# georgesterpu/avsr-tf1

Measured on AMD Instinct MI355X. Metric: utterances/sec (train step) at B=64 T_a=500 T_v=75, higher is better.
Workload: dtype f32; 1 GPU; c4: AV dual-attention (bimodal) video 1x256 + audio 3x256 uni-LSTM, scaled_luong, B=64 T_a=500x80 T_v=75 L=40; utterances_per_gpu=64, global_batch=64, T_a=500, F_a=80, T_v=75, F_v=128, T_dec=40, parallelism=dp1, video_frontend=resnet_cnn, launch=hipgraph, dropout=True

## Files before the change

avsr-tf1_amd/_lib.py:

```python
import ctypes as C
import os

import torch

from . import build as _build

MAX_LAYERS = 4
MAX_MECH = 4
MAX_STACKS = 4

_fp = C.POINTER(C.c_float)
_ip = C.POINTER(C.c_int32)


class AvsrError(RuntimeError):
    pass


class Mat(C.Structure):
    _fields_ = [("ptr", C.c_void_p), ("ld", C.c_int64), ("T", C.c_int32), ("pad_", C.c_int32), ("ldo", C.c_int64)]


class GemmDesc(C.Structure):
    _fields_ = [("A", Mat), ("B", Mat), ("C", Mat), ("bias", C.c_void_p),
                ("M", C.c_int32), ("N", C.c_int32), ("K", C.c_int32),
                ("trans_a", C.c_int32), ("trans_b", C.c_int32),
                ("alpha", C.c_float), ("beta", C.c_float), ("batch", C.c_int32),
                ("stride_a", C.c_int64), ("stride_b", C.c_int64), ("stride_c", C.c_int64),
                ("alpha_dev", C.c_void_p),
                ("splitk", C.c_int32), ("pad_", C.c_int32),
                ("workspace", C.c_void_p), ("workspace_floats", C.c_int64),
                ("colsum", C.c_void_p), ("colsum_beta", C.c_float), ("pad2_", C.c_int32)]


class RnnLayer(C.Structure):
    _fields_ = [("units", C.c_int32), ("in_dim", C.c_int32), ("hoisted", C.c_int32), ("out_col", C.c_int32),
                ("wt", C.c_void_p), ("w", C.c_void_p), ("bias", C.c_void_p),
                ("gates", C.c_void_p), ("cs", C.c_void_p), ("out", C.c_void_p), ("ld_out", C.c_int64),
                ("state", C.c_void_p), ("h_final", C.c_void_p), ("c_final", C.c_void_p),
                ("dgates", C.c_void_p), ("dstate", C.c_void_p), ("dout", C.c_void_p), ("ld_dout", C.c_int64),
                ("dout_col", C.c_int32), ("residual", C.c_int32), ("hs_seq", C.c_void_p), ("xt_seq", C.c_void_p),
                ("wt2", C.c_void_p), ("w2", C.c_void_p), ("bias2", C.c_void_p), ("rh_seq", C.c_void_p), ("dgates2", C.c_void_p)]


class RnnStack(C.Structure):
    _fields_ = [("B", C.c_int32), ("T", C.c_int32), ("reverse", C.c_int32), ("n_layers", C.c_int32),
                ("cell", C.c_int32), ("pad_", C.c_int32),
                ("len", C.c_void_p), ("dh_final", C.c_void_p), ("dc_final", C.c_void_p),
                ("seed", C.c_void_p), ("keep_in", C.c_float), ("keep_state", C.c_float), ("keep_out", C.c_float),
                ("consumer_keep", C.c_float), ("cell_id_base", C.c_int32), ("consumer_stream", C.c_int32),
                ("consumer_width", C.c_int32), ("pad2_", C.c_int32),
                ("layer", RnnLayer * MAX_LAYERS)]


class AttnMech(C.Structure):
    _fields_ = [("type", C.c_int32), ("T", C.c_int32), ("D", C.c_int32), ("chunk", C.c_int32),
                ("len", C.c_void_p), ("keys", C.c_void_p), ("values", C.c_void_p),
                ("values_sb", C.c_int64), ("values_st", C.c_int64),
                ("g", C.c_void_p), ("v", C.c_void_p), ("bq", C.c_void_p),
                ("wq_t", C.c_void_p), ("wq", C.c_void_p), ("watt_t", C.c_void_p), ("watt", C.c_void_p),
                ("scores", C.c_void_p), ("ctx", C.c_void_p), ("pq", C.c_void_p), ("pstat", C.c_void_p),
                ("pctx", C.c_void_p), ("dscores", C.c_void_p), ("dctx", C.c_void_p), ("dpq", C.c_void_p),
                ("pdq", C.c_void_p)]


class DecLayer(C.Structure):
    _fields_ = [("wt", C.c_void_p), ("w", C.c_void_p), ("bias", C.c_void_p), ("gates", C.c_void_p), ("cs", C.c_void_p),
                ("out", C.c_void_p), ("state", C.c_void_p), ("hs_seq", C.c_void_p), ("xin_seq", C.c_void_p),
                ("dgates", C.c_void_p), ("dstate", C.c_void_p), ("cell_id", C.c_int32), ("pad_", C.c_int32),
                ("wt2", C.c_void_p), ("w2", C.c_void_p), ("bias2", C.c_void_p), ("rh_seq", C.c_void_p), ("dgates2", C.c_void_p)]


MAX_DEC_EXTRA = 3


class AttnRnn(C.Structure):
    _fields_ = [("B", C.c_int32), ("L", C.c_int32), ("H", C.c_int32), ("E", C.c_int32),
                ("n_mech", C.c_int32), ("output_attention", C.c_int32), ("V", C.c_int32), ("mode", C.c_int32),
                ("go_id", C.c_int32), ("eos_id", C.c_int32),
                ("steplen", C.c_void_p), ("wt", C.c_void_p), ("w", C.c_void_p), ("bias", C.c_void_p),
                ("gates", C.c_void_p), ("cs", C.c_void_p), ("cell_out", C.c_void_p), ("att", C.c_void_p),
                ("h0", C.c_void_p), ("c0", C.c_void_p), ("state", C.c_void_p),
                ("h_final", C.c_void_p), ("c_final", C.c_void_p),
                ("mech", AttnMech * MAX_MECH),
                ("embedding", C.c_void_p), ("wout_t", C.c_void_p), ("bout", C.c_void_p),
                ("logits", C.c_void_p), ("ids", C.c_void_p), ("tok", C.c_void_p), ("n_unfinished", C.c_void_p),
                ("dgates", C.c_void_p), ("dstate", C.c_void_p), ("datt", C.c_void_p), ("dq", C.c_void_p),
                ("datt_ext", C.c_void_p), ("dcell_ext", C.c_void_p), ("dh0", C.c_void_p), ("dc0", C.c_void_p),
                ("dh_final", C.c_void_p), ("dc_final", C.c_void_p),
                ("seed", C.c_void_p), ("keep_in", C.c_float), ("keep_state", C.c_float), ("keep_out", C.c_float),
                ("sampling_prob", C.c_float), ("cell_id", C.c_int32), ("pad3_", C.c_int32),
                ("hs_seq", C.c_void_p), ("attd", C.c_void_p), ("xs", C.c_void_p), ("labels", C.c_void_p), ("fed", C.c_void_p),
                ("cell", C.c_int32), ("pad4_", C.c_int32), ("wt2", C.c_void_p), ("w2", C.c_void_p), ("bias2", C.c_void_p),
                ("rh_seq", C.c_void_p), ("dgates2", C.c_void_p),
                ("beam_width", C.c_int32), ("mem_shared", C.c_int32), ("length_penalty", C.c_float), ("pad6_", C.c_float),
                ("beam_logp", C.c_void_p), ("beam_fin", C.c_void_p), ("beam_len", C.c_void_p), ("step_ids", C.c_void_p),
                ("parent_ids", C.c_void_p), ("parent_rows", C.c_void_p),
                ("n_extra", C.c_int32), ("prof_tag", C.c_int32), ("out0", C.c_void_p), ("extra", DecLayer * MAX_DEC_EXTRA),
                ("fused_ws", C.c_void_p), ("fused_ws_floats", C.c_int64)]


MAX_LM_LAYERS = 4


class BeamLm(C.Structure):
    _fields_ = [("n_layers", C.c_int32), ("H", C.c_int32), ("E", C.c_int32), ("V", C.c_int32),
                ("one_hot", C.c_int32), ("n_rows", C.c_int32), ("lm_weight", C.c_float), ("pad_", C.c_int32),
                ("embedding", C.c_void_p), ("wt", C.c_void_p * MAX_LM_LAYERS), ("bias", C.c_void_p * MAX_LM_LAYERS),
                ("wout_t", C.c_void_p), ("bout", C.c_void_p), ("state_c", C.c_void_p), ("state_h", C.c_void_p), ("lm_logp", C.c_void_p)]


BEAM_CTC_MAX_T, BEAM_CTC_MAX_V = 2048, 256


class BeamCtc(C.Structure):
    _fields_ = [("n_utt", C.c_int32), ("beam_width", C.c_int32), ("T", C.c_int32), ("V", C.c_int32), ("eos_id", C.c_int32),
                ("weight", C.c_float), ("ld", C.c_int64)] + \
               [(n, C.c_void_p) for n in ("z", "in_len", "y", "state", "psi", "last", "term", "extra", "lm_logp")] + \
               [("lm_weight", C.c_float), ("pad_", C.c_int32)]


class ConvDesc(C.Structure):
    _fields_ = [(n, C.c_int32) for n in ("N", "H", "W", "Ci", "Co", "k", "stride", "pad_t", "pad_l", "Ho", "Wo", "pad_")] + \
               [("bn_scale", C.c_void_p), ("bn_shift", C.c_void_p)]


class ConvLaunch(C.Structure):
    _fields_ = [(n, C.c_int32) for n in ("kernel", "m", "ntc", "ch4", "rs", "fold", "ep", "nsp", "ntap", "t0", "F", "grid", "CsP", "lds_bytes",
                                         "slab", "pad_")]


class Conv3dDesc(C.Structure):
    _fields_ = [(n, C.c_int32) for n in ("B", "T", "H", "W", "Ci", "Co", "kt", "kh", "kw", "stride", "pad_f", "pad_t", "pad_l", "Ho", "Wo",
                                         "relu")] + [("scale", C.c_void_p), ("shift", C.c_void_p)]


class LogmelArgs(C.Structure):
    _fields_ = [(n, C.c_int32) for n in ("B", "N", "T_out", "F", "frame_length", "frame_step", "fft_length", "num_mel_bins", "window", "stride",
                                         "mel_nnz", "pad_")] + \
               [(n, C.c_void_p) for n in ("wav", "wav_len", "hann", "twiddle", "mel_lo", "mel_cnt", "mel_ptr", "mel_w", "out", "out_len")]


class CtcArgs(C.Structure):
    _fields_ = [("B", C.c_int32), ("T", C.c_int32), ("L", C.c_int32), ("C", C.c_int32), ("ld", C.c_int64)] + \
               [(n, C.c_void_p) for n in ("z", "labels", "labels_len", "in_len", "denom")] + [("weight", C.c_float), ("pad_", C.c_int32)] + \
               [(n, C.c_void_p) for n in ("nll", "status", "utt_loss", "dz", "ws")] + [("ws_floats", C.c_int64)]


class ColsumJob(C.Structure):
    _fields_ = [("a", Mat), ("b", Mat), ("out", C.c_void_p), ("rows", C.c_int32), ("F", C.c_int32), ("alpha", C.c_float), ("beta", C.c_float)]


class TransposeJob(C.Structure):
    _fields_ = [("src", C.c_void_p), ("dst", C.c_void_p), ("rows", C.c_int32), ("cols", C.c_int32)]


_STRUCTS = {"avsr_dec_layer": DecLayer, "avsr_mat": Mat, "avsr_gemm_desc": GemmDesc, "avsr_rnn_layer": RnnLayer, "avsr_rnn_stack": RnnStack,
            "avsr_conv_desc": ConvDesc, "avsr_conv_launch": ConvLaunch, "avsr_conv3d_desc": Conv3dDesc, "avsr_logmel_args": LogmelArgs, "avsr_ctc_args": CtcArgs, "avsr_attn_mech": AttnMech, "avsr_attn_rnn": AttnRnn, "avsr_transpose_job": TransposeJob,
            "avsr_colsum_job": ColsumJob, "avsr_beam_lm": BeamLm, "avsr_beam_ctc": BeamCtc}

_vp, _i32, _i64, _f32 = C.c_void_p, C.c_int32, C.c_int64, C.c_float
_SIGS = {
    "avsr_gemm": [C.POINTER(GemmDesc), _vp],
    "avsr_gemm_batch": [C.POINTER(GemmDesc), _i32, _vp],
    "avsr_rnn_fwd": [C.POINTER(RnnStack), _i32, _vp],
    "avsr_rnn_bwd": [C.POINTER(RnnStack), _i32, _vp],
    "avsr_rnn_set_persistent": [_vp, _i64],
    "avsr_rnn_set_persistent_mode": [_i32],
    "avsr_rnn_set_persistent_scratch": [_vp, _i64],
    "avsr_attn_rnn_fwd": [C.POINTER(AttnRnn), _i32, _i32, _vp],
    "avsr_attn_rnn_fused_eligible": [C.POINTER(AttnRnn)],
    "avsr_attn_rnn_fused_fwd_active": [C.POINTER(AttnRnn)],
    "avsr_attn_rnn_set_fused": [_i32],
    "avsr_attn_rnn_set_beam_kernel": [_i32],
    "avsr_conv_set_mfma": [_i32],
    "avsr_conv_supported": [C.POINTER(ConvDesc)],
    "avsr_conv_fwd": [C.POINTER(ConvDesc), _vp, _vp, _vp, _vp, _vp, _vp, _vp, _vp, C.POINTER(_i32), _vp],
    "avsr_conv_bwd_data": [C.POINTER(ConvDesc), _vp, _vp, _vp, _f32, _vp],
    "avsr_conv_bwd_weight": [C.POINTER(ConvDesc), _vp, _vp, _vp, _vp, _f32, _vp, _i64, _vp],
    "avsr_conv_bwd_data_bn": [C.POINTER(ConvDesc), _vp, _vp, _vp, _f32, _vp, _vp, _vp, _vp, _vp, C.POINTER(_i32), _vp],
    "avsr_conv_bwd_data_bn_supported": [C.POINTER(ConvDesc)],
    "avsr_conv_bwd_weight_bn": [C.POINTER(ConvDesc), _vp, _vp, _vp, _vp, _vp, _vp, _vp, _f32, _vp, _i64, _vp],
    "avsr_conv_bwd_weight_bn_supported": [C.POINTER(ConvDesc)],
    "avsr_conv_plan": [C.POINTER(ConvDesc), _i32, _i32, _i64, C.POINTER(ConvLaunch), _i32],
    "avsr_bn_bwd_finalize": [_vp, _i32, _i32, _i64, _vp, _vp, _vp, _vp, _vp, _f32, _vp, _vp],
    "avsr_bn_bwd_apply": [_vp, _vp, _vp, _vp, _i64, _i32, _f32, _vp],
    "avsr_bn_bwd_stage1": [_vp, _vp, _vp, _vp, _vp, _vp, _i64, _i32, _vp, C.POINTER(_i32), _vp],
    "avsr_bn_partials_f64": [_vp, _i32, _i32, _vp, _vp],
    "avsr_bn_finalize_f64": [_vp, _i32, _f32, _f32, _vp, _vp, _vp, _vp, _vp, _vp, _vp, _vp, _vp],
    "avsr_bn_bwd_finalize_f64": [_vp, _vp, _i32, _vp, _vp, _vp, _vp, _vp, _f32, _vp, _vp],
    "avsr_bn_eval_affine": [_vp, _vp, _vp, _vp, _f32, _vp, _vp, _i32, _vp],
    "avsr_bn_finalize": [_vp, _i32, _i32, _i64, _f32, _f32, _vp, _vp, _vp, _vp, _vp, _vp, _vp, _vp, _vp],
    "avsr_conv3d_supported": [C.POINTER(Conv3dDesc)],
    "avsr_conv3d_fwd": [C.POINTER(Conv3dDesc), _vp, _vp, _vp, _vp, _vp, _vp, _vp, C.POINTER(_i32), _vp],
    "avsr_conv3d_bwd_data": [C.POINTER(Conv3dDesc), _vp, _vp, _vp, _f32, _vp],
    "avsr_conv3d_bwd_weight": [C.POINTER(Conv3dDesc), _vp, _vp, _vp, _f32, _vp, _i64, _vp],
    "avsr_conv3d_bn_finalize": [_vp, _i32, _i32, _i64, _f32, _f32, _vp, _vp, _vp, _vp, _vp, _vp, _vp, _vp, _vp],
    "avsr_logmel_supported": [_i32, _i32, _i32, _i32, _i32],
    "avsr_logmel_fwd": [C.POINTER(LogmelArgs), _vp],
    "avsr_ctc_loss": [C.POINTER(CtcArgs), _vp],
    "avsr_ctc_best_path": [_vp, _i64, _vp, _i32, _i32, _i32, _vp, _vp],
    "avsr_batchnorm_apply": [_vp, _vp, _i32, _i32, _vp, _vp, _vp, _vp, _i32, _vp],
    "avsr_attn_rnn_bwd": [C.POINTER(AttnRnn), _vp],
    "avsr_beam_gather_tree": [_vp, _vp, _vp, _vp, _i32, _i32, _i32, _i32, _vp],
    "avsr_beam_search_step": [_vp, _i32, _i32, _i32, _i32, _i32, _f32, _vp, _vp, _vp, _vp, _vp, _vp, _vp, _vp, _vp, _vp, _vp, _vp, _i64, _i32, _vp, _vp, _vp],
    "avsr_beam_lm_supported": [C.POINTER(BeamLm)],
    "avsr_beam_lm_step": [C.POINTER(BeamLm), _vp, _vp, _i32, _i32, _vp],
    "avsr_beam_search_step_lm": [_vp, _i32, _i32, _i32, _i32, _i32, _f32, _vp, _vp, _vp, _vp, _vp, _vp, _vp, _vp, _vp, _vp, _vp, _vp, _i64, _i32, _vp, _vp,
                                 _vp, _f32, _vp],
    "avsr_attn_rnn_fwd_lm": [C.POINTER(AttnRnn), C.POINTER(BeamLm), _i32, _i32, _vp],
    "avsr_beam_ctc_supported": [C.POINTER(BeamCtc)],
    "avsr_beam_ctc_begin": [C.POINTER(BeamCtc), _vp],
    "avsr_beam_ctc_step": [C.POINTER(BeamCtc), _vp, _vp, _vp, _i32, _vp],
    "avsr_beam_search_step_ctc": [_vp, _i32, _i32, _i32, _i32, _i32, _f32, _vp, _vp, _vp, _vp, _vp, _vp, _vp, _vp, _vp, _vp, _vp, _vp, _i64, _i32, _vp, _vp,
                                  _vp, _f32, _vp, _f32, _vp, _vp],
    "avsr_attn_rnn_fwd_ctc": [C.POINTER(AttnRnn), C.POINTER(BeamLm), C.POINTER(BeamCtc), _i32, _i32, _vp],
    "avsr_attn_alpha_rows": [_vp, _vp, _vp, _vp, _vp, _vp, _i32, _i32, _i32, _vp],
    "avsr_bahdanau_dkeys": [_vp, _vp, _i64, _i64, _vp, _vp, _vp, _vp, _vp, _vp, _i32, _i32, _i32, _i32, _vp],
    "avsr_transpose": [C.POINTER(TransposeJob), _i32, _vp],
    "avsr_colsum": [C.POINTER(Mat), C.POINTER(Mat), _i32, _i32, _f32, _f32, _vp, _vp, _i64, _vp],
    "avsr_batchnorm_fwd": [_vp, _vp, _i32, _i32, _vp, _vp, _vp, _vp, _vp, _vp, _i32, _vp, _i64, _vp],
    "avsr_batchnorm_xhat": [_vp, _vp, _vp, _vp, _i32, _i32, _vp],
    "avsr_batchnorm_fwd_ex": [_vp, _vp, _i32, _i32, _vp, _vp, _vp, _vp, _vp, _vp, _i32, _f32, _f32, _i32, _i32, _vp, _i64, _vp],
    "avsr_batchnorm_bwd": [_vp, _vp, _vp, _vp, _vp, _vp, _vp, _vp, _vp, _i32, _i32, _i32, _f32, _vp, _i64, _vp],
    "avsr_im2col": [_vp, _vp, _i32, _i32, _i32, _i32, _i32, _i32, _i32, _i32, _i32, _i32, _i32, _vp],
    "avsr_col2im": [_vp, _vp, _i32, _i32, _i32, _i32, _i32, _i32, _i32, _i32, _i32, _i32, _i32, _f32, _vp],
    "avsr_relu": [_vp, _vp, _i64, _vp],
    "avsr_relu_bwd": [_vp, _vp, _vp, _i64, _vp],
    "avsr_add": [_vp, _vp, _vp, _i64, _vp],
    "avsr_selu": [_vp, _vp, _i64, _vp],
    "avsr_selu_bwd": [_vp, _vp, _vp, _i64, _vp],
    "avsr_conv3x3_supported": [_i32, _i32, _i32, _i32],
    "avsr_conv3x3": [_vp, _vp, _vp, _vp, _i32, _i32, _i32, _i32, _i32, _i32, _i32, _i32, _i32, _i32, _i32, _f32, _vp],
    "avsr_conv3x3_bwd_data_s2": [_vp, _vp, _vp, _i32, _i32, _i32, _i32, _i32, _i32, _i32, _i32, _i32, _f32, _vp],
    "avsr_conv3x3_bwd_weight": [_vp, _vp, _vp, _i32, _i32, _i32, _i32, _i32, _i32, _i32, _i32, _i32, _i32, _f32, _vp, _i64, _vp],
    "avsr_embed_labels": [_vp, _vp, _i32, _vp, _vp, _i32, _i32, _i32, _i32, _vp],
    "avsr_embed_grad": [_vp, _vp, _vp, _i32, _i32, _i32, _i32, _vp, _i64, _vp],
    "avsr_dropout_rows": [C.POINTER(Mat), C.POINTER(Mat), _i32, _i32, _vp, _i32, _f32, _i32, _i32, _i32, _vp],
    "avsr_seq_loss": [_vp, _vp, _vp, _vp, _i32, _vp, _vp, _i32, _i32, _i32, _vp],
    "avsr_seq_loss_fun": [_vp, _vp, _vp, _vp, _i32, _vp, _vp, _i32, _i32, _i32, _i32, _f32, _vp],
    "avsr_au_loss": [_vp, _vp, _vp, _vp, _vp, _i32, _i32, _f32, _vp],
    "avsr_au_loss_dp": [_vp, _vp, _vp, _vp, _vp, _i32, _i32, _f32, _vp, _vp],
    "avsr_normed_v": [_vp, _vp, _vp, _i32, _vp],
    "avsr_normed_v_bwd": [_vp, _vp, _vp, _vp, _vp, _i32, _vp],
    "avsr_reduce_scalar": [_vp, _i32, _vp, _i32, _i32, _f32, _vp],
    "avsr_l2_regularise": [C.POINTER(_i64), C.POINTER(_i64), _i32, _vp, _vp, _f32, _vp, _vp, _vp],
    "avsr_global_norm": [_vp, _i64, _f32, _vp, _vp, _vp],
    "avsr_adam_step": [_vp, _vp, _vp, _vp, _i64, _vp, _vp, _f32, _i32, _f32, _f32, _vp],
    "avsr_batchnorm_sync_sum": [_vp, _i32, _i32, _vp, _vp, _i64, _vp],
    "avsr_batchnorm_sync_sqsum": [_vp, _i32, _i32, _vp, _vp, _vp, _vp, _vp, _i64, _vp],
    "avsr_batchnorm_sync_apply": [_vp, _vp, _i32, _i32, _vp, _vp, _vp, _vp, _vp, _vp, _vp, _vp, _f32, _f32, _i32, _vp],
    "avsr_batchnorm_sync_moments": [_vp, _i32, _i32, _vp, _vp, _i64, _vp],
    "avsr_dp_sync_unpack": [_vp, _vp, _i32, C.POINTER(_i32), C.POINTER(_i32), C.POINTER(_vp), C.POINTER(_vp), C.POINTER(_vp), _vp],
    "avsr_seq_loss_per_utterance": [_vp, _vp, _vp, _vp, _i32, _i32, _vp],
    "avsr_instnorm_fwd": [_vp, _vp, _i32, _i32, _i32, _vp, _vp, _vp, _vp, _f32, _vp],
    "avsr_instnorm_bwd": [_vp, _vp, _vp, _vp, _vp, _vp, _vp, _vp, _i32, _i32, _i32, _vp],
    "avsr_optimiser_step": [_vp, _vp, _vp, _vp, _i64, _vp, _vp, _f32, _i32, _i32, _f32, _f32, _i32, _f32, _vp],
    "avsr_highway_fwd": [_vp, _vp, _vp, _vp, _vp, _i32, _i32, _i32, _vp],
    "avsr_highway_bwd": [_vp, _vp, _vp, _vp, _vp, _vp, _vp, _vp, _i32, _i32, _i32, _i32, _vp],
    "avsr_copy_words": [_vp, _vp, _i64, _vp],
    "avsr_zero_words": [_vp, _i64, _vp],
    "avsr_zero_multi": [C.POINTER(_vp), C.POINTER(_i64), _i32, _vp],
    "avsr_add_int": [_vp, _i32, _vp, _vp],
    "avsr_colsum_multi": [C.POINTER(ColsumJob), _i32, _vp, _i64, _vp],
    "avsr_slab_defer_begin": [], "avsr_slab_defer_end": [_vp],
    "avsr_adam_step_decay": [_vp, _vp, _vp, _vp, _i64, _vp, _vp, _f32, _i32, _i32, _f32, _f32, _vp],
    "avsr_prof_begin": [_i32],
    "avsr_prof_end": [C.POINTER(_i32), C.POINTER(_f32), C.POINTER(C.c_double)],
}
EXPORTS = ["avsr_abi_version", "avsr_sizeof", "avsr_attn_rnn_fused_ws_floats", "avsr_conv3d_wgrad_scratch_floats", "avsr_ctc_ws_floats"] + list(_SIGS)

_lib = None


def lib_path():
    return _build.LIB


def load():
    global _lib
    if _lib is not None:
        return _lib
    path = os.environ.get("AVSR_LIB") or _build.LIB
    if path == _build.LIB and _build.needs_build():
        try:
            _build.build()
        except Exception as e:
            if not os.path.exists(path):
                raise AvsrError("libavsr_hip.so is missing and could not be built: %s" % e)
    lib = C.CDLL(path)
    lib.avsr_abi_version.restype = C.c_int
    lib.avsr_sizeof.restype = C.c_int64
    lib.avsr_sizeof.argtypes = [C.c_char_p]
    for sym in EXPORTS:
        if not hasattr(lib, sym):
            raise AvsrError("libavsr_hip.so does not export %s" % sym)
    for name, at in _SIGS.items():
        fn = getattr(lib, name)
        fn.argtypes = at
        fn.restype = C.c_int
    lib.avsr_attn_rnn_fused_ws_floats.argtypes = [_i32, _i32, _i32]
    lib.avsr_attn_rnn_fused_ws_floats.restype = C.c_int64
    lib.avsr_conv3d_wgrad_scratch_floats.argtypes = [C.POINTER(Conv3dDesc)]
    lib.avsr_conv3d_wgrad_scratch_floats.restype = C.c_int64
    lib.avsr_ctc_ws_floats.argtypes = [_i32, _i32, _i32]
    lib.avsr_ctc_ws_floats.restype = C.c_int64
    for name, st in _STRUCTS.items():
        n = lib.avsr_sizeof(name.encode())
        if n != C.sizeof(st):
            raise AvsrError("ABI mismatch for %s: C %d vs ctypes %d" % (name, n, C.sizeof(st)))
    _lib = lib
    return lib


def check(rc, what):
    if rc != 0:
        raise AvsrError("%s failed with code %d" % (what, rc))


def ptr(t):
    return None if t is None else t.data_ptr()


def stream_ptr():
    return torch.cuda.current_stream().cuda_stream
```

avsr-tf1_amd/csrc/batchnorm.hip:

```cpp
#include "reduce.h"
#include "avsr_hip.h"

using namespace avsr;
#define S_(x) ((hipStream_t)(x))

namespace {

__global__ void bn_partial_sum_kernel(const float* x, float* part, int rows, int F, int rows_per_blk) {
  __shared__ float red[256];
  const int G = F < 256 ? 256 / F : 1;
  const int r0 = blockIdx.x * rows_per_blk, r1 = min(rows, r0 + rows_per_blk);
  for (int base = 0; base < (G > 1 ? 1 : F); base += blockDim.x) {
    const int idx = base + threadIdx.x;
    const int f = G > 1 ? idx % F : idx, g = G > 1 ? idx / F : 0;
    float s0 = 0.f, s1 = 0.f;
    if (G > 1 ? idx < G * F : idx < F) {
      int r = r0 + g;
      for (; r + G < r1; r += 2 * G) { s0 += x[(long)r * F + f]; s1 += x[(long)(r + G) * F + f]; }
      if (r < r1) s0 += x[(long)r * F + f];
    }
    if (G > 1) block_group_reduce(s0 + s1, idx, F, G, red, part + (long)blockIdx.x * F);
    else if (idx < F) part[(long)blockIdx.x * F + idx] = s0 + s1;
  }
}

__global__ __launch_bounds__(1024) void bn_mean_kernel(const float* part, int npart, float* mean, int rows, int F,
                                                       const float* total = nullptr) {
  if (total) rows = (int)total[0];
  __shared__ double red[32][33];
  const int fl = threadIdx.x & 31, g = threadIdx.x >> 5;
  const int f = blockIdx.x * 32 + fl;
  double s = 0.0;
  if (f < F)
    for (int i = g; i < npart; i += 32) s += (double)part[(long)i * F + f];
  red[g][fl] = s;
  __syncthreads();
  if (g == 0 && f < F) {
    double t = 0.0;
#pragma unroll
    for (int j = 0; j < 32; ++j) t += red[j][fl];
    mean[f] = (float)(t / rows);
  }
}

__global__ void bn_partial_sq_kernel(const float* x, const float* mean_v, float* part, int rows, int F, int rows_per_blk) {
  __shared__ float red[256];
  const int G = F < 256 ? 256 / F : 1;
  const int r0 = blockIdx.x * rows_per_blk, r1 = min(rows, r0 + rows_per_blk);
  for (int base = 0; base < (G > 1 ? 1 : F); base += blockDim.x) {
    const int idx = base + threadIdx.x;
    const int f = G > 1 ? idx % F : idx, g = G > 1 ? idx / F : 0;
    float s0 = 0.f, s1 = 0.f;
    if (G > 1 ? idx < G * F : idx < F) {
      const float mean = mean_v[f];
      int r = r0 + g;
      for (; r + G < r1; r += 2 * G) {
        const float d0 = x[(long)r * F + f] - mean, d1 = x[(long)(r + G) * F + f] - mean;
        s0 += d0 * d0; s1 += d1 * d1;
      }
      if (r < r1) { const float d0 = x[(long)r * F + f] - mean; s0 += d0 * d0; }
    }
    if (G > 1) block_group_reduce(s0 + s1, idx, F, G, red, part + (long)blockIdx.x * F);
    else if (idx < F) part[(long)blockIdx.x * F + idx] = s0 + s1;
  }
}

__global__ __launch_bounds__(1024) void bn_var_kernel(const float* part, int npart, const float* mean_v, float* invstd_v, float* mov_mean,
                                                      float* mov_var, int rows, int F, float eps, float momentum,
                                                      int bessel, const float* total = nullptr) {
  if (total) rows = (int)total[0];
  __shared__ double red[32][33];
  const int fl = threadIdx.x & 31, g = threadIdx.x >> 5;
  const int f = blockIdx.x * 32 + fl;
  double s = 0.0;
  if (f < F)
    for (int i = g; i < npart; i += 32) s += (double)part[(long)i * F + f];
  red[g][fl] = s;
  __syncthreads();
  if (g == 0 && f < F) {
    double t = 0.0;
#pragma unroll
    for (int j = 0; j < 32; ++j) t += red[j][fl];
    const float var = (float)(t / rows), mean = mean_v[f];
    invstd_v[f] = rsqrtf(var + eps);
    if (mov_mean) {
      const float unbiased = bessel ? var * ((float)rows / (float)max(1, rows - 1)) : var;
      mov_mean[f] = momentum * mov_mean[f] + (1.f - momentum) * mean;
      mov_var[f] = momentum * mov_var[f] + (1.f - momentum) * unbiased;
    }
  }
}

__global__ void bn_apply_kernel(const float* x, const float* mean_v, const float* invstd_v, const float* mov_mean, const float* mov_var,
                                const float* gamma, const float* beta, float* y, long n4, int F, int training, float eps, int relu) {
  for (long i = (long)blockIdx.x * blockDim.x + threadIdx.x; i < n4; i += (long)gridDim.x * blockDim.x) {
    const int f = (int)((i * 4) % F);
    const f32x4 xv = ld4(x + i * 4);
    f32x4 yv;
#pragma unroll
    for (int e = 0; e < 4; ++e) {
      const float mean = training ? mean_v[f + e] : mov_mean[f + e];
      const float istd = training ? invstd_v[f + e] : rsqrtf(mov_var[f + e] + eps);
      yv[e] = (xv[e] - mean) * (gamma[f + e] * istd) + beta[f + e];
      if (relu) yv[e] = fmaxf(yv[e], 0.f);
    }
    st4(y + i * 4, yv);
  }
}

__global__ void bn_xhat_kernel(const float* x, const float* mean, const float* invstd, float* xhat, long n, int F) {
  for (long i = (long)blockIdx.x * blockDim.x + threadIdx.x; i < n; i += (long)gridDim.x * blockDim.x) {
    const int f = (int)(i % F);
    xhat[i] = (x[i] - mean[f]) * invstd[f];
  }
}

int bn_blocks(int rows, int F, int64_t scratch_floats, int* rpb_out) {
  const int maxblk = 2048;
  int rpb = rows > 64 * maxblk ? (rows + maxblk - 1) / maxblk : 64;
  int nblk = (rows + rpb - 1) / rpb;
  if ((long)nblk * F > scratch_floats) {
    nblk = (int)(scratch_floats / F);
    if (nblk < 1) return 0;
    rpb = (rows + nblk - 1) / nblk;
    nblk = (rows + rpb - 1) / rpb;
  }
  *rpb_out = rpb;
  return nblk;
}

}

extern "C" int avsr_batchnorm_fwd_ex(const float* x, float* y, int32_t rows, int32_t F, const float* gamma, const float* beta,
                                     float* moving_mean, float* moving_var, float* save_mean, float* save_invstd, int32_t training,
                                     float eps, float momentum, int32_t relu, int32_t bessel, float* scratch, int64_t scratch_floats, void* stream) {
  if (!x || !y || !gamma || !beta || rows <= 0 || F <= 0 || !scratch) return AVSR_ERR_ARG;
  if (F % 4) return AVSR_ERR_ARG;
  int rpb;
  const int nblk = bn_blocks(rows, F, scratch_floats - 2 * F, &rpb);
  if (!nblk) return AVSR_ERR_ARG;
  float* part = scratch;
  float* mean_v = save_mean ? save_mean : scratch + (long)nblk * F;
  float* invstd_v = save_invstd ? save_invstd : scratch + (long)nblk * F + F;
  if (training) {
    hipLaunchKernelGGL(bn_partial_sum_kernel, dim3(nblk), dim3(256), 0, S_(stream), x, part, rows, F, rpb);
    AVSR_CHECK_LAUNCH();
    hipLaunchKernelGGL(bn_mean_kernel, dim3((F + 31) / 32), dim3(1024), 0, S_(stream), part, nblk, mean_v, rows, F);
    AVSR_CHECK_LAUNCH();
    hipLaunchKernelGGL(bn_partial_sq_kernel, dim3(nblk), dim3(256), 0, S_(stream), x, mean_v, part, rows, F, rpb);
    AVSR_CHECK_LAUNCH();
    hipLaunchKernelGGL(bn_var_kernel, dim3((F + 31) / 32), dim3(1024), 0, S_(stream), part, nblk, mean_v, invstd_v, moving_mean,
                       moving_var, rows, F, eps, momentum, bessel);
    AVSR_CHECK_LAUNCH();
  } else if (!moving_mean || !moving_var) {
    return AVSR_ERR_ARG;
  }
  const long n4 = (long)rows * F / 4;
  int blocks = (int)((n4 + 255) / 256);
  if (blocks > 4096) blocks = 4096;
  hipLaunchKernelGGL(bn_apply_kernel, dim3(blocks), dim3(256), 0, S_(stream), x, mean_v, invstd_v, moving_mean, moving_var, gamma, beta, y,
                     n4, F, training, eps, relu);
  AVSR_CHECK_LAUNCH();
  return AVSR_OK;
}

extern "C" int avsr_batchnorm_fwd(const float* x, float* y, int32_t rows, int32_t F, const float* gamma,
                                  const float* beta, float* moving_mean, float* moving_var, float* save_mean,
                                  float* save_invstd, int32_t training, float* scratch, int64_t scratch_floats,
                                  void* stream) {
  return avsr_batchnorm_fwd_ex(x, y, rows, F, gamma, beta, moving_mean, moving_var, save_mean, save_invstd, training, 1e-3f, 0.99f, 0,
                               0 , scratch, scratch_floats, stream);
}

extern "C" int avsr_batchnorm_apply(const float* x, float* y, int32_t rows, int32_t F, const float* gamma, const float* beta, const float* mean,
                                    const float* invstd, int32_t relu, void* stream) {
  if (!x || !y || !gamma || !beta || !mean || !invstd || rows <= 0 || F <= 0 || F % 4) return AVSR_ERR_ARG;
  const long n4 = (long)rows * F / 4;
  int blocks = (int)((n4 + 255) / 256);
  if (blocks > 4096) blocks = 4096;
  hipLaunchKernelGGL(bn_apply_kernel, dim3(blocks), dim3(256), 0, S_(stream), x, mean, invstd, nullptr, nullptr, gamma, beta, y, n4, F, 1, 0.f, relu);
  AVSR_CHECK_LAUNCH();
  return AVSR_OK;
}

extern "C" int avsr_batchnorm_xhat(const float* x, const float* mean, const float* invstd, float* xhat, int32_t rows,
                                   int32_t F, void* stream) {
  if (!x || !mean || !invstd || !xhat) return AVSR_ERR_ARG;
  const long n = (long)rows * F;
  hipLaunchKernelGGL(bn_xhat_kernel, dim3(blocks_for(n)), dim3(256), 0, S_(stream), x, mean, invstd, xhat, n, F);
  AVSR_CHECK_LAUNCH();
  return AVSR_OK;
}

namespace {

__global__ void bn_bwd_partial_kernel(const float* x, const float* dy, const float* gamma, const float* beta, const float* mean,
                                      const float* invstd, float* part, int rows, int F, int rows_per_blk, int relu) {
  __shared__ float red[512];
  const int G = F < 256 ? 256 / F : 1;
  const int r0 = blockIdx.x * rows_per_blk, r1 = min(rows, r0 + rows_per_blk);
  float* prow = part + (long)blockIdx.x * 2 * F;
  for (int base = 0; base < (G > 1 ? 1 : F); base += blockDim.x) {
    const int idx = base + threadIdx.x;
    const bool on = G > 1 ? idx < G * F : idx < F;
    const int f = G > 1 ? idx % F : idx, g = G > 1 ? idx / F : 0;
    float s1 = 0.f, s2 = 0.f;
    if (on) {
      const float m = mean[f], is = invstd[f], ga = gamma[f], be = beta[f];
      for (int r = r0 + g; r < r1; r += G) {
        const float xh = (x[(long)r * F + f] - m) * is;
        float d = dy[(long)r * F + f];
        if (relu && !(xh * ga + be > 0.f)) d = 0.f;
        s1 += d;
        s2 += d * xh;
      }
    }
    if (G > 1) {
      if (on) { red[idx] = s1; red[256 + idx] = s2; }
      __syncthreads();
      if (idx < F) {
        float t1 = 0.f, t2 = 0.f;
        for (int gg = 0; gg < G; ++gg) { t1 += red[gg * F + idx]; t2 += red[256 + gg * F + idx]; }
        prow[idx] = t1; prow[F + idx] = t2;
      }
    } else if (on) { prow[f] = s1; prow[F + f] = s2; }
  }
}

__global__ void bn_bwd_apply_kernel(const float* x, const float* dy, const float* gamma, const float* beta, const float* mean,
                                    const float* invstd, const float* sum1, const float* sum2, float* dx, long n, int rows, int F, int relu,
                                    float dx_beta) {
  const float inv_rows = 1.0f / (float)rows;
  for (long i = (long)blockIdx.x * blockDim.x + threadIdx.x; i < n; i += (long)gridDim.x * blockDim.x) {
    const int f = (int)(i % F);
    const float is = invstd[f], ga = gamma[f];
    const float xh = (x[i] - mean[f]) * is;
    float d = dy[i];
    if (relu && !(xh * ga + beta[f] > 0.f)) d = 0.f;
    const float v = ga * is * (d - (sum1[f] + xh * sum2[f]) * inv_rows);
    dx[i] = dx_beta != 0.f ? v + dx_beta * dx[i] : v;
  }
}

__global__ __launch_bounds__(256) void bn_bwd_partial4_kernel(const float* x, const float* dy, const float* gamma, const float* beta,
                                                               const float* mean, const float* invstd, float* part, long n4, int F, int relu) {
  __shared__ f32x4 red[2][256];
  const int f = (int)((threadIdx.x * 4) % F);
  const f32x4 m = ld4(mean + f), is = ld4(invstd + f), ga = ld4(gamma + f), be = ld4(beta + f);
  f32x4 s1 = {0.f, 0.f, 0.f, 0.f}, s2 = s1;
  for (long i = (long)blockIdx.x * 256 + threadIdx.x; i < n4; i += (long)gridDim.x * 256) {
    const f32x4 xv = ld4(x + i * 4), dv = ld4(dy + i * 4);
#pragma unroll
    for (int e = 0; e < 4; ++e) {
      const float xh = (xv[e] - m[e]) * is[e];
      float d = dv[e];
      if (relu && !(xh * ga[e] + be[e] > 0.f)) d = 0.f;
      s1[e] += d;
      s2[e] += d * xh;
    }
  }
  red[0][threadIdx.x] = s1; red[1][threadIdx.x] = s2;
  __syncthreads();
  const int tpf = F >> 2;
  if ((int)threadIdx.x < tpf) {
    f32x4 t1 = {0.f, 0.f, 0.f, 0.f}, t2 = t1;
    for (int k = threadIdx.x; k < 256; k += tpf) { t1 += red[0][k]; t2 += red[1][k]; }
    st4(part + (long)blockIdx.x * 2 * F + 4 * threadIdx.x, t1);
    st4(part + (long)blockIdx.x * 2 * F + F + 4 * threadIdx.x, t2);
  }
}

__global__ __launch_bounds__(256) void bn_bwd_apply4_kernel(const float* x, const float* dy, const float* gamma, const float* beta,
                                                             const float* mean, const float* invstd, const float* sum1, const float* sum2, float* dx,
                                                             long n4, int rows, int F, int relu, float dx_beta) {
  const int f = (int)((threadIdx.x * 4) % F);
  const float inv_rows = 1.0f / (float)rows;
  const f32x4 m = ld4(mean + f), is = ld4(invstd + f), ga = ld4(gamma + f), be = ld4(beta + f);
  f32x4 c1 = ld4(sum1 + f), c2 = ld4(sum2 + f);
#pragma unroll
  for (int e = 0; e < 4; ++e) { c1[e] *= inv_rows; c2[e] *= inv_rows; }
  for (long i = (long)blockIdx.x * 256 + threadIdx.x; i < n4; i += (long)gridDim.x * 256) {
    const f32x4 xv = ld4(x + i * 4), dv = ld4(dy + i * 4);
    f32x4 o;
    if (dx_beta != 0.f) o = ld4(dx + i * 4);
#pragma unroll
    for (int e = 0; e < 4; ++e) {
      const float xh = (xv[e] - m[e]) * is[e];
      float d = dv[e];
      if (relu && !(xh * ga[e] + be[e] > 0.f)) d = 0.f;
      const float v = ga[e] * is[e] * (d - (c1[e] + xh * c2[e]));
      o[e] = dx_beta != 0.f ? v + dx_beta * o[e] : v;
    }
    st4(dx + i * 4, o);
  }
}

}

extern "C" int avsr_batchnorm_bwd(const float* x, const float* dy, const float* gamma, const float* beta, const float* mean,
                                  const float* invstd, float* dx, float* dgamma, float* dbeta, int32_t rows, int32_t F, int32_t relu,
                                  float dx_beta, float* scratch, int64_t scratch_floats, void* stream) {
  if (!x || !dy || !gamma || !beta || !mean || !invstd || !scratch || rows <= 0 || F <= 0) return AVSR_ERR_ARG;
  const int maxblk = 2048;
  int rpb = rows > 64 * maxblk ? (rows + maxblk - 1) / maxblk : 64;
  int nblk = (rows + rpb - 1) / rpb;
  if ((long)nblk * 2 * F + 2 * F > scratch_floats) {
    nblk = (int)((scratch_floats - 2 * F) / (2L * F));
    if (nblk < 1) return AVSR_ERR_ARG;
    rpb = (rows + nblk - 1) / nblk;
    nblk = (rows + rpb - 1) / rpb;
  }
  float* part = scratch;
  const long n = (long)rows * F;
  auto al16 = [](const void* p) { return ((uintptr_t)p & 15) == 0; };
  const bool vec = F >= 4 && 1024 % F == 0 && al16(x) && al16(dy) && (!dx || al16(dx)) && al16(gamma) && al16(beta) && al16(mean) && al16(invstd) &&
                   al16(scratch) && rows >= 4096;
  if (vec) {
    int vb = (int)((n / 4 + 255) / 256);
    if (vb > 1024) vb = 1024;
    if ((long)vb * 2 * F + 2 * F > scratch_floats) vb = (int)((scratch_floats - 2 * F) / (2L * F));
    if (vb < 1) return AVSR_ERR_ARG;
    nblk = vb;
  }
  float* sums = scratch + (long)nblk * 2 * F;
  if (vec) hipLaunchKernelGGL(bn_bwd_partial4_kernel, dim3(nblk), dim3(256), 0, S_(stream), x, dy, gamma, beta, mean, invstd, part, n / 4, F, relu);
  else hipLaunchKernelGGL(bn_bwd_partial_kernel, dim3(nblk), dim3(256), 0, S_(stream), x, dy, gamma, beta, mean, invstd, part, rows, F, rpb, relu);
// ... 345 lines not shown
```

avsr-tf1_amd/csrc/capi.hip:

```cpp
#include <string.h>
#include "avsr_hip.h"

extern "C" int avsr_abi_version(void) { return 2; }

extern "C" int64_t avsr_sizeof(const char* name) {
  if (!name) return -1;
#define SZ(T) if (!strcmp(name, #T)) return (int64_t)sizeof(T);
  SZ(avsr_mat) SZ(avsr_gemm_desc) SZ(avsr_conv_desc) SZ(avsr_conv_launch) SZ(avsr_conv3d_desc) SZ(avsr_logmel_args) SZ(avsr_ctc_args) SZ(avsr_rnn_layer) SZ(avsr_rnn_stack) SZ(avsr_colsum_job)
#ifdef AVSR_HAVE_ATTN
  SZ(avsr_attn_mech) SZ(avsr_attn_rnn) SZ(avsr_transpose_job) SZ(avsr_dec_layer) SZ(avsr_beam_lm) SZ(avsr_beam_ctc)
#endif
#undef SZ
  return -1;
}

#include <vector>
#include "prof.h"
namespace avsr {
bool g_prof_enabled = false;
static std::vector<hipEvent_t> g_ev;
static std::vector<int> g_kind;
static size_t g_used = 0;
static double g_work[PROF_NKIND];
void prof_record(int kind, hipStream_t s, bool begin, double work) {
  if (begin) {
    if (g_used >= g_kind.size()) { g_prof_enabled = false; return; }
    g_kind[g_used] = kind;
    g_work[kind] += work;
    hipEventRecord(g_ev[2 * g_used], s);
  } else {
    hipEventRecord(g_ev[2 * g_used + 1], s);
    ++g_used;
  }
}
}

extern "C" int avsr_prof_begin(int32_t max_launches) {
  using namespace avsr;
  if (max_launches <= 0) return AVSR_ERR_ARG;
  while (g_ev.size() < (size_t)2 * max_launches) {
    hipEvent_t e;
    if (hipEventCreate(&e) != hipSuccess) return AVSR_ERR_HIP;
    g_ev.push_back(e);
  }
  g_kind.assign(max_launches, 0);
  g_used = 0;
  for (int k = 0; k < PROF_NKIND; ++k) g_work[k] = 0.0;
  g_prof_enabled = true;
  return AVSR_OK;
}

extern "C" int avsr_prof_end(int32_t* out_count, float* out_ms, double* out_flops) {
  using namespace avsr;
  g_prof_enabled = false;
  if (!out_count || !out_ms) return AVSR_ERR_ARG;
  if (hipDeviceSynchronize() != hipSuccess) return AVSR_ERR_HIP;
  for (int k = 0; k < PROF_NKIND; ++k) { out_count[k] = 0; out_ms[k] = 0.f; if (out_flops) out_flops[k] = g_work[k]; }
  for (size_t i = 0; i < g_used; ++i) {
    float ms = 0.f;
    if (hipEventElapsedTime(&ms, g_ev[2 * i], g_ev[2 * i + 1]) != hipSuccess) return AVSR_ERR_HIP;
    out_count[g_kind[i]] += 1;
    out_ms[g_kind[i]] += ms;
  }
  return AVSR_OK;
}
```

avsr-tf1_amd/csrc/elementwise.hip:

```cpp
#include "reduce.h"
#include "avsr_hip.h"

namespace avsr {

struct TJob { const float* src; float* dst; int rows, cols; };
struct TLaunch { int njob; TJob job[AVSR_MAX_TRANSPOSE]; };

__global__ void transpose_kernel(const TLaunch L) {
  __shared__ float tile[32][33];
  const TJob& J = L.job[blockIdx.z];
  const int tx = threadIdx.x & 31, ty = threadIdx.x >> 5;
  const int tiles_c = (J.cols + 31) / 32, tiles_r = (J.rows + 31) / 32;
  for (int tIdx = blockIdx.x; tIdx < tiles_c * tiles_r; tIdx += gridDim.x) {
    const int r0 = (tIdx / tiles_c) * 32, c0 = (tIdx % tiles_c) * 32;
    for (int j = ty; j < 32; j += 8) {
      const int r = r0 + j, c = c0 + tx;
      tile[j][tx] = (r < J.rows && c < J.cols) ? J.src[(long)r * J.cols + c] : 0.f;
    }
    __syncthreads();
    for (int j = ty; j < 32; j += 8) {
      const int c = c0 + j, r = r0 + tx;
      if (r < J.rows && c < J.cols) J.dst[(long)c * J.rows + r] = tile[tx][j];
    }
    __syncthreads();
  }
}

__global__ void embed_labels_kernel(const float* emb, const int32_t* labels, int go, float* out, int32_t* fed, int B, int L,
                                    int E, int nsteps) {
  const int b = blockIdx.x / nsteps, l = blockIdx.x % nsteps;
  const int tok = (l == 0) ? go : labels[(long)b * L + l - 1];
  if (fed && threadIdx.x == 0) fed[(long)b * L + l] = tok;
  for (int e = threadIdx.x; e < E; e += blockDim.x) out[((long)b * L + l) * E + e] = emb[(long)tok * E + e];
}

__global__ void dropout_rows_kernel(const float* x, long ldx, int Tx, long ldox, float* y, long ldy, int Ty, long ldoy,
                                    int rows, int cols, const int32_t* seed, uint32_t stream, float keep, int idx_w,
                                    int idx_coff, int accumulate) {
  const long total = (long)rows * cols;
  const bool on = seed && keep < 1.0f;
  const uint32_t sd = on ? (uint32_t)seed[0] : 0u;
  const float inv = 1.0f / keep;
  for (long i = (long)blockIdx.x * blockDim.x + threadIdx.x; i < total; i += (long)gridDim.x * blockDim.x) {
    const int r = (int)(i / cols), c = (int)(i % cols);
    float v = x[rowoff(r, ldx, Tx, ldox) + c];
    if (on) v = uniform01(sd, stream, (uint32_t)((long)r * idx_w + idx_coff + c)) < keep ? v * inv : 0.f;
    float* d = y + rowoff(r, ldy, Ty, ldoy) + c;
    *d = accumulate ? *d + v : v;
  }
}

#define EG_ROWS 256
__global__ void embed_grad_partial_kernel(const float* dx, const int32_t* fed, float* part, int rows, int E, int V) {
  __shared__ int toks[EG_ROWS];
  const int v = blockIdx.x, base = blockIdx.y * EG_ROWS;
  const int n = min(EG_ROWS, rows - base);
  for (int j = threadIdx.x; j < EG_ROWS; j += blockDim.x) toks[j] = j < n ? fed[base + j] : -1;
  __syncthreads();
  for (int e = threadIdx.x; e < E; e += blockDim.x) {
    float a = 0.f;
    for (int j = 0; j < n; j += 8) {
      float x[8];
#pragma unroll
      for (int k = 0; k < 8; ++k) x[k] = dx[(long)(base + min(j + k, n - 1)) * E + e];
#pragma unroll
      for (int k = 0; k < 8; ++k) a += (j + k < n && toks[j + k] == v) ? x[k] : 0.f;
    }
    part[((long)blockIdx.y * V + v) * E + e] = a;
  }
}

__global__ void seqlen_sum_kernel(const int32_t* len, int B, int L, float* denom) {
  __shared__ float red[4];
  float s = 0.f;
  for (int b = threadIdx.x; b < B; b += 256) s += (float)min(max(len[b], 0), L);
  s = block_sum_256(s, red);
  if (threadIdx.x == 0) denom[0] = s;
}

__global__ void set_scalar_kernel(float* p, float v) { p[0] = v; }

__global__ void seq_loss_kernel(float* logits, const int32_t* labels, const int32_t* len, const float* denom,
                                float* row_loss, float* dlogits, int B, int L, int V, int mode, float smooth) {
  const int row = blockIdx.x * blockDim.x + threadIdx.x;
  if (row >= B * L) return;
  const int b = row / L, l = row % L;
  float* lg = logits + (long)row * V;
  float* dl = dlogits ? dlogits + (long)row * V : nullptr;
  const bool valid = l < len[b];
  const float inv = 1.f / (denom[0] + 1e-12f);
  if (!valid) {
    row_loss[row] = mode == 1 ? logf((float)V) * inv : 0.f;
    for (int v = 0; v < V; ++v) lg[v] = 0.f;
    if (dl) for (int v = 0; v < V; ++v) dl[v] = 0.f;
    return;
  }
  float mx = lg[0];
  for (int v = 1; v < V; ++v) mx = fmaxf(mx, lg[v]);
  float s = 0.f;
  for (int v = 0; v < V; ++v) s += expf(lg[v] - mx);
  const float lse = mx + logf(s);
  const int y = labels[row];
  if (mode == 0) {
    row_loss[row] = (lse - lg[y]) * inv;
    if (dl) for (int v = 0; v < V; ++v) dl[v] = (expf(lg[v] - lse) - (v == y ? 1.f : 0.f)) * inv;
    return;
  }
  if (mode == 1) {
    const float off = smooth / (float)V, on = 1.f - smooth + off;
    float ce = 0.f;
    for (int v = 0; v < V; ++v) ce += (v == y ? on : off) * (lse - lg[v]);
    row_loss[row] = ce * inv;
    if (dl) for (int v = 0; v < V; ++v) dl[v] = (expf(lg[v] - lse) - (v == y ? on : off)) * inv;
    return;
  }
  float loss = 0.f, dot = 0.f;
  for (int v = 0; v < V; ++v) {
    const float p = expf(lg[v] - lse);
    const float q = fminf(fmaxf(p, 1e-7f), 1.f - 1e-7f);
    const bool inside = (p >= 1e-7f) && (p <= 1.f - 1e-7f);
    float f, a;
    if (mode == 3) {
      f = (v == y) ? -logf(q) : -logf(1.f - q);
      a = (v == y) ? -1.f / q : 1.f / (1.f - q);
    } else {
      if (v == y) { f = -(1.f - q) * (1.f - q) * logf(q); a = 2.f * (1.f - q) * logf(q) - (1.f - q) * (1.f - q) / q; }
      else        { f = -q * q * logf(1.f - q);           a = -2.f * q * logf(1.f - q) + q * q / (1.f - q); }
    }
    loss += f;
    dot += inside ? a * p : 0.f;
  }
  row_loss[row] = loss * inv;
  if (dl)
    for (int v = 0; v < V; ++v) {
      const float p = expf(lg[v] - lse);
      const float q = fminf(fmaxf(p, 1e-7f), 1.f - 1e-7f);
      const bool inside = (p >= 1e-7f) && (p <= 1.f - 1e-7f);
      float a;
      if (mode == 3) a = (v == y) ? -1.f / q : 1.f / (1.f - q);
      else a = (v == y) ? 2.f * (1.f - q) * logf(q) - (1.f - q) * (1.f - q) / q : -2.f * q * logf(1.f - q) + q * q / (1.f - q);
      dl[v] = p * ((inside ? a : 0.f) - dot) * inv;
    }
}

__global__ void seq_avg_kernel(const float* row_loss, const int32_t* len, const float* denom, float* out, int B, int L) {
  const int b = blockIdx.x * blockDim.x + threadIdx.x;
  if (b >= B) return;
  float s = 0.f;
  for (int l = 0; l < L; ++l) s += row_loss[(long)b * L + l];
  out[b] = s * (denom[0] + 1e-12f) / ((float)min(max(len[b], 0), L) + 1e-12f);
}

__global__ void au_loss_kernel(const float* z, const float* aus, const int32_t* len, float* row_loss, float* dz,
                               int B, int T, float weight, const float* total) {
  __shared__ float red[4];
  float cnt = 0.f;
  for (int b = threadIdx.x; b < B; b += 256) cnt += 2.f * (float)min(max(len[b], 0), T);
  cnt = block_sum_256(cnt, red);
  if (total) cnt = total[0];
  const float inv = cnt > 0.f ? 1.f / cnt : 0.f;
  for (int row = blockIdx.x * 256 + threadIdx.x; row < B * T; row += gridDim.x * 256) {
    const int b = row / T, t = row % T;
    float l = 0.f;
    for (int k = 0; k < 2; ++k) {
      float d = 0.f;
      if (t < len[b]) {
        const float p = sigmoidf_(z[(long)row * 2 + k]);
        const float tg = fminf(fmaxf(aus[(long)row * 2 + k], 0.f), 3.f) / 3.f;
        l += (p - tg) * (p - tg) * inv;
        d = weight * 2.f * (p - tg) * p * (1.f - p) * inv;
      }
      if (dz) dz[(long)row * 2 + k] = d;
    }
    row_loss[row] = l * weight;
  }
}

__global__ void normed_v_kernel(const float* v, const float* g, float* vn, int H) {
  __shared__ float red[4];
  float s = 0.f;
  for (int h = threadIdx.x; h < H; h += 256) s += v[h] * v[h];
  s = block_sum_256(s, red);
  const float sc = g[0] * rsqrtf(s);
  for (int h = threadIdx.x; h < H; h += 256) vn[h] = v[h] * sc;
}
__global__ void normed_v_bwd_kernel(const float* v, const float* g, const float* dvn, float* dv, float* dg, int H) {
  __shared__ float red[4];
  float s = 0.f, d = 0.f;
  for (int h = threadIdx.x; h < H; h += 256) { s += v[h] * v[h]; d += v[h] * dvn[h]; }
  s = block_sum_256(s, red);
  d = block_sum_256(d, red);
  const float nrm = sqrtf(s);
  for (int h = threadIdx.x; h < H; h += 256) dv[h] = g[0] / nrm * (dvn[h] - d * v[h] / s);
  if (threadIdx.x == 0) dg[0] = d / nrm;
}

struct Seg { long off, n; };
struct SegLaunch { int nseg; Seg seg[AVSR_MAX_SEGMENTS]; };

__global__ void l2_grad_kernel(const SegLaunch S, const float* w, float* g, float l2, float* part) {
  __shared__ float red[4];
  const Seg sg = S.seg[blockIdx.y];
  float s = 0.f;
  for (long i = (long)blockIdx.x * 256 + threadIdx.x; i < sg.n; i += (long)gridDim.x * 256) {
    const float x = w[sg.off + i];
    g[sg.off + i] += l2 * x;
    s += x * x;
  }
  s = block_sum_256(s, red);
  if (threadIdx.x == 0) part[blockIdx.y * gridDim.x + blockIdx.x] = 0.5f * l2 * s;
}

__global__ void sumsq_partial_kernel(const float* g, long n, float* part) {
  __shared__ float red[4];
  float s = 0.f;
  for (long i = (long)blockIdx.x * 256 + threadIdx.x; i < n; i += (long)gridDim.x * 256) s += g[i] * g[i];
  s = block_sum_256(s, red);
  if (threadIdx.x == 0) part[blockIdx.x] = s;
}

__global__ void reduce_scalar_kernel(const float* part, int n, float* out, int do_sqrt, int accumulate, float scale) {
  __shared__ double dred[256];
  double s = 0.0;
  for (int i = threadIdx.x; i < n; i += 256) s += (double)part[i];
  dred[threadIdx.x] = s;
  __syncthreads();
  for (int o = 128; o > 0; o >>= 1) {
    if (threadIdx.x < o) dred[threadIdx.x] += dred[threadIdx.x + o];
    __syncthreads();
  }
  if (threadIdx.x == 0) {
    double v = dred[0];
    if (do_sqrt) v = sqrt(v);
    v *= scale;
    out[0] = accumulate ? out[0] + (float)v : (float)v;
  }
}

__global__ void adam_kernel(float* p, float* g, float* m, float* v, long n, const float* gnorm, int32_t* step,
                            float lr, int warmup, float clip, float b1, float b2, float eps, float grad_scale,
                            int decay_steps, int opt, float weight_decay) {
  const int t = step[0] + 1;
  float lr_now = lr;
  if (decay_steps > 0) {
    const float frac = (float)(t - 1) / (float)decay_steps;
    const float i_restart = floorf(logf(1.0f + frac) / logf(2.0f));
    const float pw = exp2f(i_restart);
    const float within = (frac - (pw - 1.0f)) / pw;
    lr_now *= 0.5f * (1.0f + cosf(3.14159265358979323846f * within));
  }
  if (warmup > 0) lr_now *= fminf(1.0f, (float)t / (float)warmup);
  const double c1 = 1.0 - exp((double)t * log((double)b1));
  const double c2 = 1.0 - exp((double)t * log((double)b2));
  const float lr_t = (float)((double)lr_now * sqrt(c2) / c1);
  float scale = grad_scale;
  if (clip > 0.f) scale *= clip / fmaxf(gnorm[0], clip);
  for (long i = (long)blockIdx.x * blockDim.x + threadIdx.x; i < n; i += (long)gridDim.x * blockDim.x) {
    const float gi = g[i] * scale;
    if (opt == 3) {
      const float acc = 0.9f * m[i] + gi;
      m[i] = acc;
      p[i] -= lr_now * acc;
      continue;
    }
    const float mi = b1 * m[i] + (1.f - b1) * gi;
    const float vi = b2 * v[i] + (1.f - b2) * gi * gi;
    m[i] = mi;
    v[i] = vi;
    float pi = p[i];
    if (opt == 2) pi -= weight_decay * pi;
    const float num = opt == 1 ? b1 * mi + (1.f - b1) * gi : mi;
    p[i] = pi - lr_t * num / (sqrtf(vi) + eps);
  }
}
__global__ void step_inc_kernel(int32_t* step) { step[0] += 1; }

struct HwView { float* p; long ld; int T; long ldo; };
__device__ __forceinline__ long hw_off(const HwView& v, int r) { return rowoff(r, v.ld, v.T, v.ldo); }

__global__ void highway_fwd_kernel(HwView x, HwView h, HwView cpre, HwView y, const int32_t* len, int rows, int H, int T) {
  const long total = (long)rows * H;
  for (long i = (long)blockIdx.x * blockDim.x + threadIdx.x; i < total; i += (long)gridDim.x * blockDim.x) {
    const int r = (int)(i / H), c = (int)(i % H);
    float out = 0.f;
    if (!len || (r % T) < len[r / T]) {
      const float g = 1.f / (1.f + expf(-cpre.p[hw_off(cpre, r) + c]));
      out = x.p[hw_off(x, r) + c] * g + h.p[hw_off(h, r) + c] * (1.f - g);
    }
    y.p[hw_off(y, r) + c] = out;
  }
}

__global__ void highway_bwd_kernel(HwView x, HwView h, HwView cpre, HwView dy, HwView dh, HwView dcpre, HwView dx, const int32_t* len,
                                   int rows, int H, int T, int accumulate_dx) {
  const long total = (long)rows * H;
  for (long i = (long)blockIdx.x * blockDim.x + threadIdx.x; i < total; i += (long)gridDim.x * blockDim.x) {
    const int r = (int)(i / H), c = (int)(i % H);
    float vdh = 0.f, vdc = 0.f, vdx = 0.f;
    if (!len || (r % T) < len[r / T]) {
      const float g = 1.f / (1.f + expf(-cpre.p[hw_off(cpre, r) + c]));
      const float d = dy.p[hw_off(dy, r) + c];
      vdh = d * (1.f - g);
      vdc = d * (x.p[hw_off(x, r) + c] - h.p[hw_off(h, r) + c]) * g * (1.f - g);
      vdx = d * g;
    }
    dh.p[hw_off(dh, r) + c] = vdh;
    dcpre.p[hw_off(dcpre, r) + c] = vdc;
    float* px = dx.p + hw_off(dx, r) + c;
    *px = accumulate_dx ? *px + vdx : vdx;
  }
}

}

using namespace avsr;
#define S_(x) ((hipStream_t)(x))

extern "C" int avsr_transpose(const avsr_transpose_job* jobs, int32_t n, void* stream) {
  if (!jobs || n <= 0) return AVSR_ERR_ARG;
  for (int i0 = 0; i0 < n; i0 += AVSR_MAX_TRANSPOSE) {
    TLaunch L;
    L.njob = (n - i0) < AVSR_MAX_TRANSPOSE ? (n - i0) : AVSR_MAX_TRANSPOSE;
    int maxtiles = 1;
    for (int i = 0; i < L.njob; ++i) {
      const avsr_transpose_job& j = jobs[i0 + i];
      if (!j.src || !j.dst || j.rows <= 0 || j.cols <= 0) return AVSR_ERR_ARG;
      L.job[i] = TJob{j.src, j.dst, j.rows, j.cols};
      const int tiles = ((j.rows + 31) / 32) * ((j.cols + 31) / 32);
      if (tiles > maxtiles) maxtiles = tiles;
    }
    if (maxtiles > 1024) maxtiles = 1024;
    hipLaunchKernelGGL(transpose_kernel, dim3(maxtiles, 1, L.njob), dim3(256), 0, S_(stream), L);
    AVSR_CHECK_LAUNCH();
  }
  return AVSR_OK;
}

struct ZmLaunch { uint32_t* p[8]; long n[8]; int cnt; };
__global__ __launch_bounds__(256) void zero_multi_kernel(const ZmLaunch L) {
  const long stride = (long)gridDim.x * 256;
#pragma unroll 1
  for (int k = 0; k < L.cnt; ++k) {
    uint32_t* p = L.p[k];
    const long n = L.n[k], n4 = ((uintptr_t)p & 15) == 0 ? n >> 2 : 0;
    typedef unsigned int u32x4_ __attribute__((ext_vector_type(4)));
    for (long i = (long)blockIdx.x * 256 + threadIdx.x; i < n4; i += stride) reinterpret_cast<u32x4_*>(p)[i] = u32x4_{0u, 0u, 0u, 0u};
    for (long i = n4 * 4 + (long)blockIdx.x * 256 + threadIdx.x; i < n; i += stride) p[i] = 0u;
  }
}
extern "C" int avsr_zero_multi(void* const* ptrs, const int64_t* n_words, int32_t count, void* stream) {
  if (count <= 0) return AVSR_OK;
  if (!ptrs || !n_words) return AVSR_ERR_ARG;
  for (int c0 = 0; c0 < count; c0 += 8) {
    ZmLaunch L = {};
    long tot = 0;
    for (int k = 0; k < 8 && c0 + k < count; ++k) {
      if (!ptrs[c0 + k] || n_words[c0 + k] < 0) return AVSR_ERR_ARG;
      L.p[k] = (uint32_t*)ptrs[c0 + k]; L.n[k] = n_words[c0 + k]; L.cnt = k + 1; tot += n_words[c0 + k];
    }
    long blocks = (tot / 4 + 256 * 4 - 1) / (256 * 4);
    if (blocks > 2048) blocks = 2048;
    if (blocks < 1) blocks = 1;
    hipLaunchKernelGGL(zero_multi_kernel, dim3((int)blocks), dim3(256), 0, S_(stream), L);
    AVSR_CHECK_LAUNCH();
  }
  return AVSR_OK;
}
__global__ void add_int_kernel(const int32_t* a, int32_t b, int32_t* out) { out[0] = a[0] + b; }
extern "C" int avsr_add_int(const int32_t* a, int32_t b, int32_t* out, void* stream) {
  if (!a || !out) return AVSR_ERR_ARG;
  hipLaunchKernelGGL(add_int_kernel, dim3(1), dim3(1), 0, S_(stream), a, b, out);
  AVSR_CHECK_LAUNCH();
  return AVSR_OK;
}

struct DpUnpack { const double* buf; float* dp_norm; int nstream; int off[4]; int F[4]; float* mean[4]; float* sq[4]; float* rows[4]; };
__global__ void dp_sync_unpack_kernel(const DpUnpack U) {
  const int t = blockIdx.x * blockDim.x + threadIdx.x;
  if (t < 2 && U.dp_norm) U.dp_norm[t] = (float)U.buf[t];
  for (int s = 0; s < U.nstream; ++s) {
    const double* b = U.buf + U.off[s];
    const int F = U.F[s];
    const double n = b[2 * F];
    if (t == 0) U.rows[s][0] = (float)n;
    if (t < F) {
      const double m = n > 0.0 ? b[t] / n : 0.0;
      double c = b[F + t] - n * m * m;
      if (c < 0.0) c = 0.0;
      U.mean[s][t] = (float)m;
      U.sq[s][t] = (float)c;
    }
  }
}
extern "C" int avsr_dp_sync_unpack(const double* buf, float* dp_norm, int32_t nstream, const int32_t* off, const int32_t* F,
                                   float* const* mean, float* const* sq, float* const* rows, void* stream) {
  if (!buf || nstream < 0 || nstream > 4) return AVSR_ERR_ARG;
  DpUnpack U = {};
  U.buf = buf; U.dp_norm = dp_norm; U.nstream = nstream;
  int maxF = 2;
  for (int s = 0; s < nstream; ++s) {
    if (!off || !F || !mean || !sq || !rows || !mean[s] || !sq[s] || !rows[s] || F[s] <= 0) return AVSR_ERR_ARG;
    U.off[s] = off[s]; U.F[s] = F[s]; U.mean[s] = mean[s]; U.sq[s] = sq[s]; U.rows[s] = rows[s];
    if (F[s] > maxF) maxF = F[s];
  }
  hipLaunchKernelGGL(dp_sync_unpack_kernel, dim3((maxF + 255) / 256), dim3(256), 0, S_(stream), U);
  AVSR_CHECK_LAUNCH();
  return AVSR_OK;
}

extern "C" int avsr_embed_labels(const float* emb, const int32_t* labels, int32_t go_id, float* out, int32_t* fed,
                                 int32_t B, int32_t L, int32_t E, int32_t n_steps, void* stream) {
  if (!emb || !labels || !out || n_steps <= 0 || n_steps > L) return AVSR_ERR_ARG;
  hipLaunchKernelGGL(embed_labels_kernel, dim3(B * n_steps), dim3(E >= 256 ? 256 : ((E + 63) / 64) * 64), 0, S_(stream),
                     emb, labels, go_id, out, fed, B, L, E, n_steps);
  AVSR_CHECK_LAUNCH();
  return AVSR_OK;
}

extern "C" int avsr_embed_grad(const float* dx, const int32_t* fed, float* demb, int32_t B, int32_t L, int32_t E,
                               int32_t V, float* scratch, int64_t scratch_floats, void* stream) {
  if (!dx || !fed || !demb || !scratch || B <= 0 || L <= 0 || E <= 0 || V <= 0) return AVSR_ERR_ARG;
  const int rows = B * L;
  const int nchunk = (rows + EG_ROWS - 1) / EG_ROWS;
  if ((long)nchunk * V * E > scratch_floats || nchunk > 65535) return AVSR_ERR_ARG;
  hipLaunchKernelGGL(embed_grad_partial_kernel, dim3(V, nchunk), dim3(E >= 256 ? 256 : ((E + 63) / 64) * 64), 0, S_(stream), dx, fed,
                     scratch, rows, E, V);
  AVSR_CHECK_LAUNCH();
  return avsr_colsum_final_launch(scratch, nchunk, demb, V * E, 1.0f, 0.0f, stream);
}

extern "C" int avsr_dropout_rows(const avsr_mat* x, const avsr_mat* y, int32_t rows, int32_t cols, const int32_t* seed,
                                 int32_t stream_id, float keep, int32_t idx_width, int32_t idx_coff, int32_t accumulate,
                                 void* stream) {
  if (!x || !y || !x->ptr || !y->ptr || rows <= 0 || cols <= 0) return AVSR_ERR_ARG;
  hipLaunchKernelGGL(dropout_rows_kernel, dim3(blocks_for((long)rows * cols)), dim3(256), 0, S_(stream), x->ptr, (long)x->ld,
                     x->T, (long)x->ldo, y->ptr, (long)y->ld, y->T, (long)y->ldo, rows, cols, seed, (uint32_t)stream_id, keep,
                     idx_width, idx_coff, accumulate);
  AVSR_CHECK_LAUNCH();
  return AVSR_OK;
}

extern "C" int avsr_seq_loss(float* logits, const int32_t* labels, const int32_t* labels_len, float* denom,
                             int32_t compute_denom, float* row_loss, float* dlogits, int32_t B, int32_t L, int32_t V,
                             void* stream) {
  return avsr_seq_loss_fun(logits, labels, labels_len, denom, compute_denom, row_loss, dlogits, B, L, V, 0, 0.f, stream);
}

extern "C" int avsr_seq_loss_fun(float* logits, const int32_t* labels, const int32_t* labels_len, float* denom,
                                 int32_t compute_denom, float* row_loss, float* dlogits, int32_t B, int32_t L, int32_t V,
                                 int32_t loss_fun, float label_smoothing, void* stream) {
  if (!logits || !labels || !labels_len || !denom || !row_loss || loss_fun < 0 || loss_fun > 3) return AVSR_ERR_ARG;
  if (compute_denom) {
    if (loss_fun == 1) hipLaunchKernelGGL(set_scalar_kernel, dim3(1), dim3(1), 0, S_(stream), denom, (float)B * (float)L);
    else hipLaunchKernelGGL(seqlen_sum_kernel, dim3(1), dim3(256), 0, S_(stream), labels_len, B, L, denom);
    AVSR_CHECK_LAUNCH();
  }
  hipLaunchKernelGGL(seq_loss_kernel, dim3((B * L + 127) / 128), dim3(128), 0, S_(stream), logits, labels, labels_len,
                     denom, row_loss, dlogits, B, L, V, loss_fun, label_smoothing);
  AVSR_CHECK_LAUNCH();
  return AVSR_OK;
}

static inline avsr::HwView hwv(const avsr_mat* m) { return avsr::HwView{m->ptr, (long)m->ld, m->T, (long)m->ldo}; }

extern "C" int avsr_highway_fwd(const avsr_mat* x, const avsr_mat* h, const avsr_mat* carry_pre, const avsr_mat* y, const int32_t* len,
                                int32_t B, int32_t T, int32_t H, void* stream) {
  if (!x || !h || !carry_pre || !y || !x->ptr || !h->ptr || !carry_pre->ptr || !y->ptr || B <= 0 || T <= 0 || H <= 0) return AVSR_ERR_ARG;
  hipLaunchKernelGGL(highway_fwd_kernel, dim3(blocks_for((long)B * T * H)), dim3(256), 0, S_(stream), hwv(x), hwv(h), hwv(carry_pre), hwv(y),
                     len, B * T, H, T);
  AVSR_CHECK_LAUNCH();
  return AVSR_OK;
}

extern "C" int avsr_highway_bwd(const avsr_mat* x, const avsr_mat* h, const avsr_mat* carry_pre, const avsr_mat* dy, const avsr_mat* dh,
                                const avsr_mat* dcarry_pre, const avsr_mat* dx, const int32_t* len, int32_t B, int32_t T, int32_t H,
                                int32_t accumulate_dx, void* stream) {
  if (!x || !h || !carry_pre || !dy || !dh || !dcarry_pre || !dx || !x->ptr || !h->ptr || !carry_pre->ptr || !dy->ptr || !dh->ptr ||
      !dcarry_pre->ptr || !dx->ptr || B <= 0 || T <= 0 || H <= 0) return AVSR_ERR_ARG;
  hipLaunchKernelGGL(highway_bwd_kernel, dim3(blocks_for((long)B * T * H)), dim3(256), 0, S_(stream), hwv(x), hwv(h), hwv(carry_pre), hwv(dy),
                     hwv(dh), hwv(dcarry_pre), hwv(dx), len, B * T, H, T, accumulate_dx);
  AVSR_CHECK_LAUNCH();
  return AVSR_OK;
}

extern "C" int avsr_copy_words(void* dst, const void* src, int64_t n_words, void* stream) {
  if (!dst || !src || n_words < 0) return AVSR_ERR_ARG;
  return avsr::dev_copy(dst, src, (size_t)n_words * 4, S_(stream)) == hipSuccess ? AVSR_OK : AVSR_ERR_HIP;
}

extern "C" int avsr_zero_words(void* dst, int64_t n_words, void* stream) {
  if (!dst || n_words < 0) return AVSR_ERR_ARG;
  return avsr::dev_zero(dst, (size_t)n_words * 4, S_(stream)) == hipSuccess ? AVSR_OK : AVSR_ERR_HIP;
}

extern "C" int avsr_seq_loss_per_utterance(const float* row_loss, const int32_t* labels_len, const float* denom, float* out,
                                           int32_t B, int32_t L, void* stream) {
  if (!row_loss || !labels_len || !denom || !out || B <= 0 || L <= 0) return AVSR_ERR_ARG;
  hipLaunchKernelGGL(seq_avg_kernel, dim3((B + 63) / 64), dim3(64), 0, S_(stream), row_loss, labels_len, denom, out, B, L);
  AVSR_CHECK_LAUNCH();
  return AVSR_OK;
}

extern "C" int avsr_au_loss(const float* z, const float* aus, const int32_t* len, float* row_loss, float* dz, int32_t B,
                            int32_t T, float weight, void* stream) {
  return avsr_au_loss_dp(z, aus, len, row_loss, dz, B, T, weight, nullptr, stream);
}

extern "C" int avsr_au_loss_dp(const float* z, const float* aus, const int32_t* len, float* row_loss, float* dz, int32_t B,
                               int32_t T, float weight, const float* total_count, void* stream) {
  if (!z || !aus || !len || !row_loss) return AVSR_ERR_ARG;
  hipLaunchKernelGGL(au_loss_kernel, dim3(blocks_for((long)B * T, 256, 256)), dim3(256), 0, S_(stream), z, aus, len,
                     row_loss, dz, B, T, weight, total_count);
  AVSR_CHECK_LAUNCH();
  return AVSR_OK;
}

extern "C" int avsr_normed_v(const float* v, const float* g, float* vn, int32_t H, void* stream) {
  if (!v || !g || !vn) return AVSR_ERR_ARG;
  hipLaunchKernelGGL(normed_v_kernel, dim3(1), dim3(256), 0, S_(stream), v, g, vn, H);
  AVSR_CHECK_LAUNCH();
  return AVSR_OK;
}
extern "C" int avsr_normed_v_bwd(const float* v, const float* g, const float* dvn, float* dv, float* dg, int32_t H,
                                 void* stream) {
  if (!v || !g || !dvn || !dv || !dg) return AVSR_ERR_ARG;
  hipLaunchKernelGGL(normed_v_bwd_kernel, dim3(1), dim3(256), 0, S_(stream), v, g, dvn, dv, dg, H);
  AVSR_CHECK_LAUNCH();
  return AVSR_OK;
}

extern "C" int avsr_reduce_scalar(const float* part, int32_t n, float* out, int32_t do_sqrt, int32_t accumulate,
                                  float scale, void* stream) {
  if (!part || !out || n <= 0) return AVSR_ERR_ARG;
  hipLaunchKernelGGL(reduce_scalar_kernel, dim3(1), dim3(256), 0, S_(stream), part, n, out, do_sqrt, accumulate, scale);
  AVSR_CHECK_LAUNCH();
  return AVSR_OK;
}

extern "C" int avsr_l2_regularise(const int64_t* seg_off, const int64_t* seg_n, int32_t nseg, const float* params,
                                  float* grads, float l2, float* loss_accum, float* scratch, void* stream) {
  if (nseg <= 0) return AVSR_OK;
  if (!seg_off || !seg_n || !params || !grads || !scratch || nseg > AVSR_MAX_SEGMENTS) return AVSR_ERR_ARG;
  SegLaunch S;
  S.nseg = nseg;
  for (int i = 0; i < nseg; ++i) S.seg[i] = Seg{(long)seg_off[i], (long)seg_n[i]};
  const int gx = 64;
  hipLaunchKernelGGL(l2_grad_kernel, dim3(gx, nseg), dim3(256), 0, S_(stream), S, params, grads, l2, scratch);
  AVSR_CHECK_LAUNCH();
  if (loss_accum) {
    hipLaunchKernelGGL(reduce_scalar_kernel, dim3(1), dim3(256), 0, S_(stream), scratch, gx * nseg, loss_accum, 0, 1, 1.0f);
    AVSR_CHECK_LAUNCH();
  }
  return AVSR_OK;
}

extern "C" int avsr_global_norm(const float* grads, int64_t n, float grad_scale, float* norm_out, float* scratch,
                                void* stream) {
  if (!grads || !norm_out || !scratch || n <= 0) return AVSR_ERR_ARG;
  const int gx = blocks_for(n, 1024, 1024);
  hipLaunchKernelGGL(sumsq_partial_kernel, dim3(gx), dim3(256), 0, S_(stream), grads, (long)n, scratch);
  AVSR_CHECK_LAUNCH();
  hipLaunchKernelGGL(reduce_scalar_kernel, dim3(1), dim3(256), 0, S_(stream), scratch, gx, norm_out, 1, 0, grad_scale);
  AVSR_CHECK_LAUNCH();
  return AVSR_OK;
}

extern "C" int avsr_adam_step(float* params, float* grads, float* m, float* v, int64_t n, const float* global_norm,
                              int32_t* step, float lr, int32_t warmup_steps, float clip_norm, float grad_scale,
                              void* stream) {
  return avsr_adam_step_decay(params, grads, m, v, n, global_norm, step, lr, warmup_steps, 0, clip_norm, grad_scale, stream);
}

extern "C" int avsr_adam_step_decay(float* params, float* grads, float* m, float* v, int64_t n, const float* global_norm,
                                    int32_t* step, float lr, int32_t warmup_steps, int32_t first_decay_steps,
                                    float clip_norm, float grad_scale, void* stream) {
  return avsr_optimiser_step(params, grads, m, v, n, global_norm, step, lr, warmup_steps, first_decay_steps, clip_norm, grad_scale, 0, 0.f,
                             stream);
}

extern "C" int avsr_optimiser_step(float* params, float* grads, float* m, float* v, int64_t n, const float* global_norm,
                                   int32_t* step, float lr, int32_t warmup_steps, int32_t first_decay_steps, float clip_norm,
                                   float grad_scale, int32_t optimiser, float weight_decay, void* stream) {
  if (!params || !grads || !m || !v || !step || n <= 0 || first_decay_steps < 0 || optimiser < 0 || optimiser > 3) return AVSR_ERR_ARG;
  if (clip_norm > 0.f && !global_norm) return AVSR_ERR_ARG;
  hipLaunchKernelGGL(adam_kernel, dim3(blocks_for(n, 1024, 2048)), dim3(256), 0, S_(stream), params, grads, m, v, (long)n,
                     global_norm, step, lr, warmup_steps, clip_norm, 0.9f, 0.999f, 1e-8f, grad_scale, first_decay_steps, optimiser, weight_decay);
  AVSR_CHECK_LAUNCH();
  hipLaunchKernelGGL(step_inc_kernel, dim3(1), dim3(1), 0, S_(stream), step);
  AVSR_CHECK_LAUNCH();
  return AVSR_OK;
}
```

avsr-tf1_amd/model.py:

```python
from collections import OrderedDict
from dataclasses import dataclass
from typing import Dict, List, Optional

import os

import numpy as np
import torch

from . import ops, params as PR
from ._lib import AttnRnn, RnnStack
from .config import ATT_CODE, BAHDANAU_TYPES, CELL_ID_DECODER, LUONG_TYPES, ModelConfig, encoder_cell_id
from .model_base import Batch, Ref, SeqBuf, _FlagReader, _PtrView, _splitk, desc_steplen
from .model_decoder import DecoderMixin
from .model_encoder import EncoderMixin


class Seq2SeqModel(EncoderMixin, DecoderMixin):
    def __init__(self, cfg: ModelConfig, device="cuda", seed=0, weights: Optional[Dict[str, np.ndarray]] = None):
        cfg.validate()
        if not torch.cuda.is_available():
            raise RuntimeError("avsr_tf1_amd needs an MI355X GPU: the HIP engine has no CPU fallback")
        from . import _lib
        _lib.load()
        self.cfg_tf, self.dev = cfg, torch.device(device)
# ... 228 lines not shown
                                     ["dec/att%d" % i for i in range(len(cfg.decoder_memories()))], Tv=Tv, Ta=Ta, greedy=greedy)
        D = ws["dec"]
        V = cfg.vocab_size
        D["xemb"], D["dxemb"] = z(B * Ldec, cfg.embedding_size), z(B * Ldec, cfg.embedding_size)
        D["logits"], D["dlogits"], D["row_loss"] = z(B, Ldec, V), z(B, Ldec, V), z(B * Ldec)
        D["fed"] = torch.zeros(B, Ldec, dtype=torch.int32, device=dev)
        D["ids"] = torch.zeros(B, Ldec, dtype=torch.int32, device=dev)
        D["tok"] = torch.zeros(B, dtype=torch.int32, device=dev)
        D["nunf"] = torch.zeros(1, dtype=torch.int32, device=dev)
        D["nunf_prev"] = torch.zeros(1, dtype=torch.int32, device=dev)
        D["steplen"] = torch.zeros(B, dtype=torch.int32, device=dev)
        ws["B"], ws["L"] = B, L
        self._ws_cache[key] = ws
        return ws

    def prepare_workspace(self, batch):
        B, L = batch.labels.shape
        Ta = self._audio_rows(batch)
        Tv = batch.video.shape[1] if batch.video is not None else 0
        self._ensure_gemm_ws()
        return self._get_ws(B, Ta, Tv, L, False)

    def pin_workspace(self, ws):
        for k, v in self._ws_cache.items():
            if v is ws:
                self._ws_pinned.add(k)
                return k
        return None

    def unpin_workspace(self, key):
        self._ws_pinned.discard(key)

    def _make_block(self, ws, B, L, H, E, mems, cell_prefix, att_prefixes, Tv, Ta, greedy, mem_B=None):
        cfg, dev = self.cfg, self.dev
        z = lambda *s: torch.zeros(*s, device=dev)
        A = H * len(mems)
        mem_B = B if mem_B is None else mem_B
        blk = {"B": B, "L": L, "H": H, "E": E, "A": A, "cell": cell_prefix, "mems": [], "mem_B": mem_B}
        if cell_prefix.startswith("dec/"):
            blk["cell_id"], blk["keep"] = CELL_ID_DECODER, cfg.decoder_dropout
        else:
            blk["cell_id"], blk["keep"] = encoder_cell_id("audio", "fw", len(cfg.audio_units) - 1), cfg.audio_dropout
        if self.gru:
            blk["rh"], blk["dpc"] = z(B, L, H), z(B, L, H)
        if cfg.use_dropout:
            blk["hs_seq"] = SeqBuf(B, L, H, 1, 0, dev)
            if A:
                blk["attd"] = SeqBuf(B, L, A, 1, 0, dev)
        blk.update(gates=z(B, L, H, 4), cs=z(B, L, H), cell_out=SeqBuf(B, L, H, 1, 0, dev), state=z(4 * B * H),
                   dgates=z(B, L, H, 4), dstate=z(12 * B * H), dq=z(B, L, H), dh0=z(B, H), dc0=z(B, H),
                   hf=z(B, H), cf=z(B, H), dcell_ext=z(B, L, H))
        if A:
            blk.update(att=SeqBuf(B, L, A, 1, 0, dev), datt=z(B, L, A), datt_ext=z(B, L, A))
        if mems and len(mems) <= 2 and not self.gru:
            blk["fused_ws"] = z(ops.attn_rnn_fused_ws_floats(B, len(mems), 256))
        blk["extra"] = []
        if cell_prefix == "dec/l0":
            n_extra = len(cfg.decoder_units) - 1
            if n_extra:
                blk["out0"] = SeqBuf(B, L, H, 1, 0, dev)
            for j in range(1, n_extra + 1):
                X = dict(prefix="dec/l%d" % j, cell_id=CELL_ID_DECODER + j, gates=z(B, L, H, 4), cs=z(B, L, H), state=z(4 * B * H),
                         dgates=z(B, L, H, 4), dstate=z(12 * B * H), out=(blk["cell_out"] if j == n_extra else SeqBuf(B, L, H, 1, 0, dev)))
                if cfg.use_dropout:
                    X["hs_seq"], X["xin_seq"] = SeqBuf(B, L, H, 1, 0, dev), SeqBuf(B, L, H, 1, 0, dev)
                if self.gru:
                    X["rh"], X["dpc"] = z(B, L, H), z(B, L, H)
                blk["extra"].append(X)
        for (stream, att_type), pre in zip(mems, att_prefixes):
            T = Ta if stream == "audio" else Tv
            D = cfg.memory_depth(stream)
            chunk = 64 if T > 64 else max(16, (T + 1) // 2)
            while (T + chunk - 1) // chunk > 16:
                chunk *= 2
            nc = (T + chunk - 1) // chunk
            m = {"stream": stream, "type": att_type, "prefix": pre, "T": T, "D": D, "chunk": chunk, "nc": nc}
            m["proj"] = D > 256 and H <= 256
            Dv = H if m["proj"] else D
            m["Dv"] = Dv
            if m["proj"]:
                eye = torch.eye(H, device=dev)
                m.update(pvals=z(mem_B, T, H), dpvals=z(mem_B, T, H), eye=eye, watt_p=torch.cat([z(H, H), eye], 0).contiguous(),
                         watt_p_t=torch.cat([z(H, H), eye], 1).contiguous())
            m.update(keys=z(mem_B, T, H), dkeys=z(mem_B, T, H), scores=z(B, L, T), dscores=z(B, L, T), ctx=z(B, L, Dv), dctx=z(B, L, Dv),
                     pstat=z(L, 2, nc, B), pctx=z(nc, B, Dv), pdq=z(nc, B, H), rowdot=z(B * L))
            if att_type in BAHDANAU_TYPES:
                m.update(pq=z(B, L, H), dpq=z(B, L, H), vn=z(H), dvn=z(H), dv_part=z(((T + 15) // 16) * B, H))
            blk["mems"].append(m)
        return blk

    def _ensure_gemm_ws(self):
        if self.gemm_ws is None:
            self.gemm_ws = torch.empty(48 << 20, device=self.dev)
        ops.set_gemm_workspace(self.gemm_ws)

    def _gemm_tn(self, A, Bm, Cm, M, N, K, beta=1.0, colsum=None, group_tiles=None):
        sk = _splitk(M, N, K)
        if group_tiles and K >= 16384:
            sk = max(2, min(768 // int(group_tiles), K // 256))
        elif group_tiles and K >= 1024:
            sk = max(1, min(768 // int(group_tiles), K // 64))
        while sk > 1 and sk * (M * N + (N if colsum is not None else 0)) > self.gemm_ws.numel():
            sk //= 2
        ops.gemm(A, Bm, Cm, M, N, K, trans_a=1, beta=beta, splitk=sk, workspace=self.gemm_ws, colsum=colsum, colsum_beta=1.0)

    def forward_train(self, batch: Batch, compute_denom=True):
        cfg = self.cfg
        B, L = batch.labels.shape
        Ta = self._audio_rows(batch)
        Tv = batch.video.shape[1] if batch.video is not None else 0
        ws = self._get_ws(B, Ta, Tv, L, False)
        self._cur = (ws, batch)
        ops.colsum_batch_abort()
        self._refresh_derived()
        ops.add_int(self.step, int(self.seed_offset), self.seed)
        self._encode(ws, batch, True)
        D = ws["dec"]
        H, E, V = D["H"], D["E"], cfg.vocab_size
        self._decoder_init_state(ws)
        sampling = cfg.sampling_probability > 0
        A = D["A"]
        drop_in = self._dropping and cfg.decoder_dropout[0] < 1.0
        xm = ops.mat(D["xemb"], E)
        ops.embed_labels(self._emb_t(), batch.labels, cfg.go_id, D["xemb"], D["fed"], B, L, E, 1 if sampling else L)
        if drop_in:
            if sampling:
                ops.dropout_rows(ops.mat(D["xemb"], L * E), ops.mat(D["xemb"], L * E), B, E, self.seed, CELL_ID_DECODER * 4,
                                 cfg.decoder_dropout[0], L * (E + A))
            else:
                ops.dropout_rows(xm, xm, B * L, E, self.seed, CELL_ID_DECODER * 4, cfg.decoder_dropout[0], E + A)
        if not sampling:
            ops.gemm(xm, self.P[self._kn("dec/l0")[0]].mat(self.G * H), ops.mat(D["gates"], self.G * H), B * L, self.G * H, E)
            if self.gru:
                ops.gemm(xm, self.P["dec/l0/cand_kernel"].mat(H), ops.mat(D["cs"], H), B * L, H, E)
        self._block_prepare(ws, D)
        D["desc"] = d = self._block_desc(ws, D, batch.labels_len, 2 if sampling else 0, D["h0"], D["c0"], with_bwd=True)
        if sampling:
            d.output_attention = int(cfg.output_attention())
            d.seed = ops.fptr(self.seed)
            d.sampling_prob = cfg.sampling_probability
            if not self._bdrop(D):
                d.keep_in = d.keep_state = d.keep_out = 1.0
                d.cell_id = CELL_ID_DECODER
            d.embedding = ops.fptr(*self._emb())
            d.wout_t = ops.fptr(self.derived, self.Tr["dec/out/kernel"].off)
            d.bout = ops.fptr(self.params, self.P["dec/out/bias"].off)
            d.logits, d.xs, d.labels, d.fed = ops.fptr(D["logits"]), ops.fptr(D["xemb"]), ops.fptr(batch.labels), ops.fptr(D["fed"])
        ops.attn_rnn_fwd(d, 0, L)
        if not sampling:
            ov, O = self._out_vec(D)
            ops.gemm(ov, self.P["dec/out/kernel"].mat(V), ops.mat(D["logits"], V), B * L, V, O, bias=self._pp("dec/out/bias"))
        ops.seq_loss(D["logits"], batch.labels, batch.labels_len, self.denom, compute_denom, D["row_loss"], D["dlogits"], B, L, V,
                     loss_fun=cfg.loss_code(), label_smoothing=cfg.label_smoothing)
        ops.reduce_scalar(D["row_loss"], B * L, self.loss)
        if cfg.regress_aus and "video" in ws["enc"]:
            Ev = ws["enc"]["video"]
            ops.reduce_scalar(Ev["au_row"], B * Ev["T"], self.loss, accumulate=True)
        if cfg.use_ctc:
            self._ctc_forward(ws, batch)
        return D["logits"]

    def local_loss_denominator(self, batch: Batch):
        B, L = batch.labels.shape
        if self.cfg.loss_code() == 1:
            return torch.full((1,), float(B * L), device=self.dev)
        return batch.labels_len.clamp(0, L).sum().to(torch.float32).reshape(1)

    def local_au_count(self, batch: Batch):
        if not (self.cfg.regress_aus and batch.video is not None):
            return torch.zeros(1, device=self.dev)
        return (2.0 * batch.video_len.clamp(0, batch.video.shape[1]).sum()).to(torch.float32).reshape(1)

    def sequence_likelihoods(self, batch: Batch):
        self.forward_train(batch)
        ws, _ = self._cur
        D = ws["dec"]
        if "utt_loss" not in D:
            D["utt_loss"] = torch.zeros(ws["B"], device=self.dev)
        ops.seq_loss_per_utterance(D["row_loss"], batch.labels_len, self.denom, D["utt_loss"], ws["B"], ws["L"])
        return D["utt_loss"]

    def backward_decoder(self):
        cfg = self.cfg
        ws, batch = self._cur
        B, L = ws["B"], ws["L"]
        D = ws["dec"]
        H, E, A, V = D["H"], D["E"], D["A"], cfg.vocab_size
        self._ensure_gemm_ws()
        zs = [self.grads] + [ws["enc"][s]["dmem"].t for s in cfg.streams() if "dmem" in ws["enc"][s]]
        if cfg.architecture == "av_align":
            zs += [ws["enc"]["audio"]["blk"]["datt_ext"], ws["enc"]["audio"]["blk"]["dcell_ext"]]
        ops.zero_multi(zs)
        ops.colsum_batch_begin(self.grads)
        ov, O = self._out_vec(D)
        dl = ops.mat(D["dlogits"], V)
        oa = cfg.output_attention()
        dext = D["datt_ext"] if oa else D["dcell_ext"]
        with ops.gemm_group():
            self._gemm_tn(ov, dl, self.Gr["dec/out/kernel"].mat(V), O, V, B * L)
            ops.colsum(dl, B * L, V, self.grads, self.scratch, beta=1.0, out_offset=self.Gr["dec/out/bias"].off)
            ops.gemm(dl, self.P["dec/out/kernel"].mat(V), ops.mat(dext, O), B * L, O, V, trans_b=1)
        d = D["desc"]
        d.datt_ext = ops.fptr(dext) if oa else None
        d.dcell_ext = None if oa else ops.fptr(dext)
        self._block_backward(ws, D, d, ops.mat(D["xemb"], E), ops.mat(D["dxemb"], E), 0.0, oa)
        if self._dropping and cfg.decoder_dropout[0] < 1.0:
            dm = ops.mat(D["dxemb"], E)
            ops.dropout_rows(dm, dm, B * L, E, self.seed, CELL_ID_DECODER * 4, cfg.decoder_dropout[0], E + A)
        if self.onehot is None:
            ops.embed_grad(D["dxemb"], D["fed"], self._gp("dec/embedding"), B, L, E, V, self.scratch)
        self._decoder_init_state_bwd(ws)
        ops.colsum_batch_end(self.scratch)

    def backward_encoders(self):
        ws, batch = self._cur
        ops.colsum_batch_begin(self.grads)
        try:
            self._encode_backward(ws, batch)
        finally:
            ops.colsum_batch_end(self.scratch)
        self._dp_stats_pack()

    def backward(self):
        self.backward_decoder()
        self.backward_encoders()

    def _dp_stats_pack(self):
        if self.dp_world > 1 and self.n_stats > 0:
            ops.colsum(ops.mat(self.stats, self.n_stats), 1, self.n_stats, self.grads_and_loss, self.scratch, alpha=1.0 / self.dp_world,
                       out_offset=self._stats_mirror_off)

    def _dp_stats_unpack(self):
        if self.dp_world > 1 and self.n_stats > 0:
            ops.colsum(ops.mat(self.grads_and_loss, self.n_stats, offset=self._stats_mirror_off), 1, self.n_stats, self.stats, self.scratch)

    def decoder_grad_bucket(self):
        segs = [(g.off, g.off + g.n, n) for n, g in self.Gr.items()]
        dec = [(lo, hi) for lo, hi, n in segs if n.startswith("dec/")]
        if not dec:
            return None
        lo, hi = min(x[0] for x in dec), max(x[1] for x in dec)
        if any(lo <= a < hi and not n.startswith("dec/") for a, b, n in segs):
            return None
        return lo, hi

    def apply_update(self):
        cfg = self.cfg
        self._dp_stats_unpack()
        if cfg.recurrent_l2 is not None:
            ops.l2_regularise(self.l2_segments, self.params, self.grads, cfg.recurrent_l2, self.loss, self.scratch)
        if self.use_cnn:
            ops.l2_regularise(self.cnn_l2_segments, self.params, self.grads, 1e-3, self.loss, self.scratch)
            if self.dense_l2_segments:
                ops.l2_regularise(self.dense_l2_segments, self.params, self.grads, 1e-4, self.loss, self.scratch)
        ops.global_norm(self.grads, self.n_train, self.gnorm, self.scratch)
        ops.adam_step(self.params, self.grads, self.adam_m, self.adam_v, self.n_train, self.gnorm, self.step,
                      cfg.learning_rate, cfg.warmup_steps, cfg.max_gradient_norm if cfg.clip_gradients else 0.0,
                      first_decay_steps=cfg.lr_decay_steps, optimiser=cfg.optimiser, weight_decay=cfg.weight_decay)

    def train_step(self, batch: Batch):
        self.forward_train(batch)
        self.backward()
        self.apply_update()
        return self.loss, self.gnorm
```

avsr-tf1_amd/model_encoder.py:

```python
from collections import OrderedDict
from dataclasses import dataclass
from typing import Dict, List, Optional
import os
import numpy as np
import torch
from . import ops, params as PR
from ._lib import AttnRnn, RnnStack
from .config import ATT_CODE, BAHDANAU_TYPES, CELL_ID_DECODER, LUONG_TYPES, ModelConfig, encoder_cell_id
from .model_base import Batch, Ref, SeqBuf, _FlagReader, _PtrView, _splitk, desc_steplen


class EncoderMixin:
    def _kn(self, prefix):
        return (prefix + "/gates_kernel", prefix + "/gates_bias") if self.gru else (prefix + "/kernel", prefix + "/bias")

    def _keeps(self, s):
        return self.cfg.video_dropout if s == "video" else self.cfg.audio_dropout

    def _sdrop(self, s):
        return self._dropping and min(self._keeps(s)) < 1.0

    def _bdrop(self, blk):
        return self._dropping and min(blk["keep"]) < 1.0

# ... 140 lines not shown
                E = ws["enc"][s]
                if l >= E["nplain"]:
                    continue
                T, u = E["T"], E["units"][l]
                for d in cfg.directions():
                    Ld = E["layers"][(d, l)]
                    if l > 0:
                        Lo = E["layers"][(d, l - 1)]
                        x, pre = self._highway_x(E, d, l), f"{s}/enc/{d}/l{l}"
                        cp, dcp = ops.mat(Ld["cpre"], u, T=T, ldo=T * u), ops.mat(Ld["dcpre"], u, T=T, ldo=T * u)
                        dy_below = Lo["dy"].mat(0, Lo["col"])
                        ops.highway_bwd(x, Ld["hout"].mat(0), cp, Ld["dy"].mat(0, Ld["col"]), Ld["dhout"].mat(0), dcp, dy_below, E["len"], B, T, u,
                                        accumulate_dx=False)
                        self._gemm_tn(x, ops.mat(Ld["dcpre"], u), self.Gr[pre + "/carry_w"].mat(u), u, u, B * T)
                        ops.colsum(ops.mat(Ld["dcpre"], u), B * T, u, self.grads, self.scratch, beta=1.0, out_offset=self.Gr[pre + "/carry_b"].off)
                        ops.gemm(ops.mat(Ld["dcpre"], u), self.P[pre + "/carry_w"].mat(u), dy_below, B * T, u, u, trans_b=1, beta=1.0)
                    stacks.append(self._rnn_stack_single(ws, s, d, l, B, E["len"], backward=True))
            self._run_stacks(stacks, ops.rnn_bwd)
            for s in hw_streams:
                E = ws["enc"][s]
                if l >= E["nplain"]:
                    continue
                T, u, F0 = E["T"], E["units"][l], E["F0"]
                drop = self._sdrop(s)
                for d in cfg.directions():
                    Ld = E["layers"][(d, l)]
                    kname, bname = self._kn(f"{s}/enc/{d}/l{l}")
                    G = self.G
                    Gk, dg = self.Gr[kname], ops.mat(Ld["dgates"], G * u)
                    in_w = F0 if l == 0 else u
                    if l == 0:
                        a_x = ops.mat(E["xd"][d] if drop else E["xin0"], F0)
                    else:
                        a_x = ops.mat(Ld["xd"], u) if drop else self._highway_x(E, d, l)
                    self._gemm_tn(a_x, dg, Gk.mat(G * u), in_w, G * u, B * T)
                    sh = 1 if d == "bw" else -1
                    hrec = Ld["hs_seq"].mat(sh) if drop else (Ld["out"].mat(sh, Ld["col"]) if l == 0 else Ld["hout"].mat(sh))
                    self._gemm_tn(hrec, dg, Gk.mat(G * u, row0=in_w), u, G * u, B * T)
                    ops.colsum(dg, B * T, G * u, self.grads, self.scratch, beta=1.0, out_offset=self.Gr[bname].off)
                    if self.gru:
                        cpre = f"{s}/enc/{d}/l{l}"
                        Gc, dpc = self.Gr[cpre + "/cand_kernel"], ops.mat(Ld["dpc"], u)
                        self._gemm_tn(a_x, dpc, Gc.mat(u), in_w, u, B * T)
                        self._gemm_tn(ops.mat(Ld["rh"], u), dpc, Gc.mat(u, row0=in_w), u, u, B * T)
                        ops.colsum(dpc, B * T, u, self.grads, self.scratch, beta=1.0, out_offset=self.Gr[cpre + "/cand_bias"].off)
                    if l > 0:
                        Lo = E["layers"][(d, l - 1)]
                        dy_below = Lo["dy"].mat(0, Lo["col"])
                        tgt, beta = (ops.mat(Ld["dxtmp"], u), 0.0) if drop else (dy_below, 1.0)
                        ops.gemm(dg, self.P[kname].mat(G * u), tgt, B * T, u, G * u, trans_b=1, beta=beta)
                        if self.gru:
                            ops.gemm(ops.mat(Ld["dpc"], u), self.P[f"{s}/enc/{d}/l{l}/cand_kernel"].mat(u), tgt, B * T, u, u, trans_b=1, beta=1.0)
                        if drop:
                            ops.dropout_rows(ops.mat(Ld["dxtmp"], u), dy_below, B * T, u, self.seed, encoder_cell_id(s, d, l) * 4,
                                             self._keeps(s)[0], u, accumulate=True)

    def bn_sync_enable(self):
        cfg = self.cfg
        streams = [s for s in cfg.streams() if cfg.batch_normalisation and not (s == "video" and self.use_cnn)]
        if not streams:
            return None
        off, n = {}, 0
        for s in streams:
            off[s], n = n, n + cfg.feat(s)
        z = lambda k: torch.zeros(k, dtype=torch.float32, device=self.dev)
        buf = z(n + len(streams))
        self.bn_sync = dict(streams=streams, off=off, sum=buf, sq=z(n), mean=z(n), rows=[buf[n + i:n + i + 1] for i in range(len(streams))])
        return self.bn_sync

    def _fit_width(self, E, x, s):
        F = E["F"]
        if "xpad" in E and x.shape[-1] != F:
            Ft = self.cfg_tf.feat(s)
            assert x.shape == E["xpad"].shape[:2] + (Ft,) and x.is_contiguous() and x.dtype == torch.float32
            ops.dropout_rows(ops.mat(x, Ft), ops.mat(E["xpad"], F), x.shape[0] * x.shape[1], Ft, None, 0, 1.0, Ft)
            x = E["xpad"]
        return x

    def _audio_rows(self, batch):
        if batch.audio is None:
            return 0
        return batch.audio.shape[1] if self.audio_fe is None else self.audio_fe.spec.rows(batch.audio.shape[1])

    def _wav_features(self, E, batch):
        x = batch.audio
        assert x.dim() == 2 and x.shape[0] == E["wav_x"].shape[0] and self.audio_fe.spec.rows(x.shape[1]) == E["T"], \
            "audio_processing='wav' takes [B, N] waveforms"
        self.audio_fe.forward(x, batch.audio_len, E["wav_x"], E["wav_len"])
        return E["wav_x"], E["wav_len"]

    def _bn_sync_x(self, batch, s):
        x = batch.video if s == "video" else batch.audio
        F = self.cfg.feat(s)
        if (s == "audio" and self.audio_fe is not None) or x.shape[-1] != F:
            B, L = batch.labels.shape
            ws = self._get_ws(B, self._audio_rows(batch), batch.video.shape[1] if batch.video is not None else 0, L, False)
            if s == "audio" and self.audio_fe is not None:
                x, _ = self._wav_features(ws["enc"][s], batch)
            else:
                x = self._fit_width(ws["enc"][s], x, s)
        assert x.is_contiguous() and x.dtype == torch.float32 and x.shape[-1] == F
        return x, x.shape[0] * x.shape[1], F

    def dp_sync_pack(self, batch):
        bs = self.bn_sync
        streams = bs["streams"] if bs else []
        if getattr(self, "_dp_buf", None) is None:
            offs, n = [], 2
            for s in streams:
                offs.append(n)
                n += 2 * self.cfg.feat(s) + 1
            self._dp_buf, self._dp_offs = torch.zeros(n, dtype=torch.float64, device=self.dev), offs
        buf = self._dp_buf
        buf[0:1].copy_(self.local_loss_denominator(batch))
        buf[1:2].copy_(self.local_au_count(batch))
        for i, s in enumerate(streams):
            x, rows, F = self._bn_sync_x(batch, s)
            o = self._dp_offs[i]
            ops.batchnorm_sync_moments(x, rows, F, buf[o:o + 2 * F], self.scratch)
            buf[o + 2 * F:o + 2 * F + 1].fill_(float(rows))
        self.au_scale, self.au_external = 1.0, True
        return buf

    def dp_sync_unpack(self):
        bs = self.bn_sync
        streams = bs["streams"] if bs else []
        jobs = []
        for i, s in enumerate(streams):
            F, o = self.cfg.feat(s), bs["off"][s]
            jobs.append((self._dp_offs[i], F, bs["mean"][o:o + F], bs["sq"][o:o + F], bs["rows"][i]))
        ops.dp_sync_unpack(self._dp_buf, self.dp_norm, jobs)

    def bn_sync_sums(self, batch):
        bs = self.bn_sync
        for i, s in enumerate(bs["streams"]):
            x, rows, F = self._bn_sync_x(batch, s)
            o = bs["off"][s]
            ops.batchnorm_sync_sum(x, rows, F, bs["sum"][o:o + F], self.scratch)
            bs["rows"][i].fill_(float(rows))
        return bs["sum"]

    def bn_sync_squares(self, batch):
        bs = self.bn_sync
        for i, s in enumerate(bs["streams"]):
            x, rows, F = self._bn_sync_x(batch, s)
            o = bs["off"][s]
            ops.batchnorm_sync_sqsum(x, rows, F, bs["sum"][o:o + F], bs["rows"][i], bs["mean"][o:o + F], bs["sq"][o:o + F], self.scratch)
        return bs["sq"]

    def _encode(self, ws, batch: Batch, training: bool):
        cfg, B = self.cfg, ws["B"]
        self._dropping = bool(cfg.use_dropout and training)
        stacks = []
        for s in cfg.streams():
            E = ws["enc"][s]
            T, F = E["T"], E["F"]
            x = batch.video if s == "video" else batch.audio
            len_t = batch.video_len if s == "video" else batch.audio_len
            if s == "audio" and self.audio_fe is not None:
                x, len_t = self._wav_features(E, batch)
            if "cnn" in E:
                Hh, Ww, Cc = cfg.video_hw
                assert x.shape == (B, T, Hh, Ww, Cc) and x.is_contiguous() and x.dtype == torch.float32
                x = E["cnn"].forward(x.view(B * T, Hh, Ww, Cc), training).view(B, T, F)
            if "cnn" not in E:
                x = self._fit_width(E, x, s)
            assert x.shape == (B, T, F) and x.is_contiguous() and x.dtype == torch.float32
            E["x"], E["len"] = x, len_t
            if cfg.batch_normalisation:
                sync = getattr(self, "cnn_bn_sync", None) if (training and "cnn" in E) else None
                if sync is not None:
                    if "sync64" not in E:
                        E["sync64"] = torch.zeros(2 * F + 1, dtype=torch.float64, device=self.dev)
                        E["sync_mean"], E["sync_sq"], E["sync_rows"] = (torch.zeros(F, device=self.dev), torch.zeros(F, device=self.dev),
                                                                       torch.zeros(1, device=self.dev))
                    buf = E["sync64"]
                    ops.batchnorm_sync_moments(x, B * T, F, buf[:2 * F], self.scratch)
                    buf[2 * F:2 * F + 1].fill_(float(B * T))
                    sync(buf)
                    ops.dp_sync_unpack(buf, None, [(0, F, E["sync_mean"], E["sync_sq"], E["sync_rows"])])
                    ops.batchnorm_sync_apply(x, E["xn"], B * T, F, self._pp(f"{s}/bn/gamma"), self._pp(f"{s}/bn/beta"),
                                             self._sp(f"{s}/bn/moving_mean"), self._sp(f"{s}/bn/moving_variance"),
                                             E["sync_mean"], E["sync_sq"], E["sync_rows"], E["invstd"])
                    E["mean"] = E["sync_mean"]
                elif training and self.bn_sync is not None and s in self.bn_sync["streams"]:
                    o = self.bn_sync["off"][s]
                    ops.batchnorm_sync_apply(x, E["xn"], B * T, F, self._pp(f"{s}/bn/gamma"), self._pp(f"{s}/bn/beta"),
                                             self._sp(f"{s}/bn/moving_mean"), self._sp(f"{s}/bn/moving_variance"),
                                             self.bn_sync["mean"][o:o + F], self.bn_sync["sq"][o:o + F],
                                             self.bn_sync["rows"][self.bn_sync["streams"].index(s)], E["invstd"])
                    E["mean"] = self.bn_sync["mean"][o:o + F]
                else:
                    E["mean"] = E["mean_own"]
                    ops.batchnorm_fwd(x, E["xn"], B * T, F, self._pp(f"{s}/bn/gamma"), self._pp(f"{s}/bn/beta"),
                                      self._sp(f"{s}/bn/moving_mean"), self._sp(f"{s}/bn/moving_variance"),
                                      E["mean"], E["invstd"], training, self.scratch)
                E["xin"] = E["xn"]
            else:
                E["xin"] = x
            if cfg.instance_normalisation:
                E["in_x"] = E["xin"]
                ops.instnorm_fwd(E["xin"], E["xi"], B, T, F, self._pp(f"{s}/in/gamma"), self._pp(f"{s}/in/beta"), E["in_mean"], E["in_invstd"])
                E["xin"] = E["xi"]
            F0 = E["F0"]
            E["xin0"], E["dxin0"] = E["xin"], E["dxn"]
            if self.n_dense:
                a_prev, w_prev = E["xin"], F
                for k, Dn in enumerate(E["dense"]):
                    u = cfg.input_dense_layers[k]
                    ops.gemm(ops.mat(a_prev, w_prev), self.P[f"{s}/dense{k}/kernel"].mat(u), ops.mat(Dn["z"], u), B * T, u, w_prev)
                    ops.selu(Dn["z"], Dn["a"], B * T * u)
                    a_prev, w_prev = Dn["a"], u
                E["xin0"], E["dxin0"] = a_prev, E["dense"][-1]["da"]
            if E["nplain"] == 0 or cfg.highway(s):
                continue
            for d in cfg.directions():
                u0 = E["units"][0]
                W0 = self.P[self._kn(f"{s}/enc/{d}/l0")[0]]
                xin = E["xin0"]
                if self._sdrop(s):
                    xin = E["xd"][d]
                    ops.dropout_rows(ops.mat(E["xin0"], F0), ops.mat(xin, F0), B * T, F0, self.seed, encoder_cell_id(s, d, 0) * 4,
                                     self._keeps(s)[0], F0)
                G = self.G
                ops.gemm(ops.mat(xin, F0), W0.mat(G * u0), ops.mat(E["layers"][(d, 0)]["gates"], G * u0), B * T, G * u0, F0)
                if self.gru:
                    ops.gemm(ops.mat(xin, F0), self.P[f"{s}/enc/{d}/l0/cand_kernel"].mat(u0), ops.mat(E["layers"][(d, 0)]["cs"], u0), B * T, u0, F0)
                stacks.append(self._rnn_stack(ws, s, d, B, len_t))
        self._run_stacks(stacks, ops.rnn_fwd)
        if any(cfg.highway(s) for s in cfg.streams()):
            self._encode_highway(ws, B)
        for s in cfg.streams():
            E = ws["enc"][s]
            if E["attentive"]:
                self._av_align_forward(ws, batch, training)
                continue
            self._final_state_fwd(ws, s)
            if s == "video" and cfg.regress_aus and training:
                Wau = self.P["video/au/kernel"]
                ops.gemm(E["mem"].mat(), Wau.mat(2), ops.mat(E["au_z"], 2), B * E["T"], 2, E["mem"].D, bias=self._pp("video/au/bias"))
                ops.au_loss(E["au_z"], batch.aus, E["len"], E["au_row"], E["au_dz"], B, E["T"], cfg.au_loss_weight * self.au_scale,
                            total_count=self.au_total if self.au_external else None)

    def _ctc_head(self, ws):
        cfg, B = self.cfg, ws["B"]
        s = cfg.ctc_stream()
        E, Cc = ws["enc"][s], cfg.vocab_size + 1
        ops.gemm(self._mem_desc(ws, s)["vmat"], self.P[f"{s}/ctc/kernel"].mat(Cc), ops.mat(E["ctc_z"], Cc), B * E["T"], Cc,
                 cfg.memory_depth(s), bias=self._pp(f"{s}/ctc/bias"))
        return E, Cc

    def _ctc_forward(self, ws, batch):
        cfg, B = self.cfg, ws["B"]
        E, Cc = self._ctc_head(ws)
        ops.ctc_loss(E["ctc_z"], Cc, batch.labels, batch.labels_len, E["len"], self.denom, cfg.ctc_weight, E["ctc_nll"], E["ctc_status"],
                     E["ctc_utt"], E["ctc_dz"], E["ctc_ws"], B, E["T"], ws["L"], Cc)
        ops.reduce_scalar(E["ctc_utt"], B, self.loss, accumulate=True)

    def ctc_best_path(self, batch):
        out = self._ctc_best_path(batch)
        if self.check_persistent():
            out = self._ctc_best_path(batch)
        return out

    def _ctc_best_path(self, batch):
        cfg = self.cfg
        if not cfg.use_ctc:
            raise ValueError("ctc_best_path needs a model built with use_ctc=True")
        B = (batch.audio if batch.audio is not None else batch.video).shape[0]
        Ta = self._audio_rows(batch)
        Tv = batch.video.shape[1] if batch.video is not None else 0
        ws = self._get_ws(B, Ta, Tv, 1, True)
        self._refresh_derived()
        self._encode(ws, batch, False)
        E, Cc = self._ctc_head(ws)
        ops.ctc_best_path(E["ctc_z"], Cc, E["len"], B, E["T"], Cc, E["ctc_ids"])
        ids = E["ctc_ids"].view(B, E["T"]).cpu().numpy()
        out = []
        for row in ids:
            seq, prev = [], -1
            for k in row:
                k = int(k)
                if k < 0:
                    break
                if k != prev and k != Cc - 1:
                    seq.append(k)
                prev = k
            out.append(seq)
        return out

    def persistent_flagged(self):
        return bool(self.persistent_rnn and ops.rnn_persistent_error())

    def check_persistent(self, disable=True, force=False):
        if not self.persistent_rnn:
            return False
        if not force and not ops.rnn_persistent_error():
            return False
        if disable:
            import warnings
            warnings.warn("avsr_tf1_amd: persistent RNN kernel timed out; falling back to per-step launches")
            self.persistent_rnn = False
            self.fused_decode = False
            ops.rnn_set_persistent(False)
            ops.rnn_persistent_clear()
        return True

    @staticmethod
    def _run_stacks(stacks, fn):
        if not stacks:
            return
        if sum(s.n_layers for s in stacks) <= 8 and len(stacks) <= 4:
            fn(stacks)
            return
        for s in stacks:
            fn([s])

    def _pp(self, name):
        r = self.P[name]
        return r.t[r.off:r.off + r.n]

    def _gp(self, name):
        r = self.Gr[name]
        return r.t[r.off:r.off + r.n]

    def _sp(self, name):
        r = self.S[name]
        if self._redo_pass:
            if self._stats_sink is None:
                self._stats_sink = torch.empty_like(self.stats)
            ops.copy_(self._stats_sink[r.off:r.off + r.n], r.t[r.off:r.off + r.n])
            return self._stats_sink[r.off:r.off + r.n]
        return r.t[r.off:r.off + r.n]

    def redoing(self):
        import contextlib

        @contextlib.contextmanager
        def ctx():
            self._redo_pass = True
            try:
                yield
            finally:
                self._redo_pass = False
        return ctx()

    def _final_state_fwd(self, ws, s):
        cfg, B = self.cfg, ws["B"]
        E = ws["enc"][s]
        top = len(E["units"]) - 1
        u, H = E["units"][-1], cfg.decoder_units[0]
        if cfg.encoder_type == "unidirectional":
            Lt = E["layers"][("fw", top)]
            E["c_fin"], E["h_fin"] = (None if self.gru else Lt["cf"]), Lt["hf"]
            return
        for nm, key, dst in ((("proj", "hf", "h_dec"),) if self.gru else (("proj_c", "cf", "c_dec"), ("proj_h", "hf", "h_dec"))):
            Pm = self.P[f"{s}/enc/{nm}"]
            for di, d in enumerate(cfg.directions()):
                ops.gemm(ops.mat(E["layers"][(d, top)][key], u), Pm.mat(H, row0=di * u), ops.mat(E[dst], H), B, H, u,
                         beta=0.0 if di == 0 else 1.0)
        E["c_fin"], E["h_fin"] = (None if self.gru else E["c_dec"]), E["h_dec"]

    def _final_state_bwd(self, ws, s, dc, dh):
        cfg, B = self.cfg, ws["B"]
        E = ws["enc"][s]
        top = len(E["units"]) - 1
        u, H = E["units"][-1], cfg.decoder_units[0]
        if E["attentive"]:
            E["blk"]["dcf_in"], E["blk"]["dhf_in"] = dc, dh
            return
        if cfg.encoder_type == "unidirectional":
            Lt = E["layers"][("fw", top)]
            if not self.gru and dc.data_ptr() != Lt["dcf"].data_ptr():
                ops.copy_(Lt["dcf"], dc)
            if dh.data_ptr() != Lt["dhf"].data_ptr():
                ops.copy_(Lt["dhf"], dh)
# ... 124 lines not shown
```

avsr-tf1_amd/ops.py:

```python
import ctypes as C
import os

import torch

from . import _lib
from ._lib import (AttnMech, AttnRnn, GemmDesc, Mat, RnnLayer, RnnStack, TransposeJob, check, stream_ptr)


def fptr(t, offset=0):
    if t is None:
        return None
    assert t.is_cuda, "HIP engine buffers must live on the GPU"
    return t.data_ptr() + t.element_size() * int(offset)


def mat(t, ld, T=0, ldo=0, offset=0):
    assert t.dtype == torch.float32
    return Mat(fptr(t, offset), int(ld), int(T), 0, int(ldo))


def _L():
    return _lib.load()


# ... 102 lines not shown
        check(_L().avsr_gemm_batch(arr, n, _s()), "avsr_gemm_batch")
    grp["descs"], grp["cursor"], grp["keep"] = [], 0, []


def rnn_fwd(stacks):
    arr = (RnnStack * len(stacks))(*stacks)
    check(_L().avsr_rnn_fwd(arr, len(stacks), _s()), "avsr_rnn_fwd")


def rnn_bwd(stacks):
    arr = (RnnStack * len(stacks))(*stacks)
    check(_L().avsr_rnn_bwd(arr, len(stacks), _s()), "avsr_rnn_bwd")


def attn_rnn_fwd(desc, l_begin, l_end):
    check(_L().avsr_attn_rnn_fwd(C.byref(desc), int(l_begin), int(l_end), _s()), "avsr_attn_rnn_fwd")


def attn_rnn_bwd(desc):
    check(_L().avsr_attn_rnn_bwd(C.byref(desc), _s()), "avsr_attn_rnn_bwd")


def beam_search_step(logits, n_utt, beam_width, V, step, eos_id, length_penalty_weight, logp_in, fin_in, len_in, logp_out, fin_out, len_out,
                     tok, parent_rows, step_ids, parent_ids, n_unfinished, x=None, x_stride=0, O=0, wout_t=None, bout=None):
    check(_L().avsr_beam_search_step(fptr(logits), n_utt, beam_width, V, step, eos_id, float(length_penalty_weight), fptr(logp_in), fptr(fin_in),
                                     fptr(len_in), fptr(logp_out), fptr(fin_out), fptr(len_out), fptr(tok), fptr(parent_rows), fptr(step_ids),
                                     fptr(parent_ids), fptr(n_unfinished), fptr(x), x_stride, O, fptr(wout_t), fptr(bout), _s()),
          "avsr_beam_search_step")


def beam_search_step_lm(logits, n_utt, beam_width, V, step, eos_id, length_penalty_weight, logp_in, fin_in, len_in, logp_out, fin_out, len_out,
                        tok, parent_rows, step_ids, parent_ids, n_unfinished, lm_logp, lm_weight, x=None, x_stride=0, O=0, wout_t=None, bout=None):
    check(_L().avsr_beam_search_step_lm(fptr(logits), n_utt, beam_width, V, step, eos_id, float(length_penalty_weight), fptr(logp_in), fptr(fin_in),
                                        fptr(len_in), fptr(logp_out), fptr(fin_out), fptr(len_out), fptr(tok), fptr(parent_rows), fptr(step_ids),
                                        fptr(parent_ids), fptr(n_unfinished), fptr(x), x_stride, O, fptr(wout_t), fptr(bout), fptr(lm_logp),
                                        float(lm_weight), _s()), "avsr_beam_search_step_lm")


def beam_lm_supported(desc):
    return bool(_L().avsr_beam_lm_supported(C.byref(desc)))


def beam_lm_step(desc, tok, parent_rows, n_rows, step):
    check(_L().avsr_beam_lm_step(C.byref(desc), fptr(tok), fptr(parent_rows), int(n_rows), int(step), _s()), "avsr_beam_lm_step")


def beam_ctc_supported(desc):
    return bool(_L().avsr_beam_ctc_supported(C.byref(desc)))


def beam_ctc_begin(desc):
    check(_L().avsr_beam_ctc_begin(C.byref(desc), _s()), "avsr_beam_ctc_begin")


def beam_ctc_step(desc, tok, parent_rows, fin, step):
    check(_L().avsr_beam_ctc_step(C.byref(desc), fptr(tok), fptr(parent_rows), fptr(fin), int(step), _s()), "avsr_beam_ctc_step")


def beam_search_step_ctc(logits, n_utt, beam_width, V, step, eos_id, length_penalty_weight, logp_in, fin_in, len_in, logp_out, fin_out, len_out,
                         tok, parent_rows, step_ids, parent_ids, n_unfinished, lm_logp, lm_weight, ctc_term, ctc_weight, extra,
                         x=None, x_stride=0, O=0, wout_t=None, bout=None):
    check(_L().avsr_beam_search_step_ctc(fptr(logits), n_utt, beam_width, V, step, eos_id, float(length_penalty_weight), fptr(logp_in),
                                         fptr(fin_in), fptr(len_in), fptr(logp_out), fptr(fin_out), fptr(len_out), fptr(tok), fptr(parent_rows),
                                         fptr(step_ids), fptr(parent_ids), fptr(n_unfinished), fptr(x), x_stride, O, fptr(wout_t), fptr(bout),
                                         fptr(lm_logp), float(lm_weight), fptr(ctc_term), float(ctc_weight), fptr(extra), _s()),
          "avsr_beam_search_step_ctc")


def attn_rnn_fwd_ctc(desc, lm_desc, ctc_desc, l_begin, l_end):
    check(_L().avsr_attn_rnn_fwd_ctc(C.byref(desc), C.byref(lm_desc) if lm_desc is not None else None, C.byref(ctc_desc), int(l_begin),
                                     int(l_end), _s()), "avsr_attn_rnn_fwd_ctc")


def attn_rnn_fwd_lm(desc, lm_desc, l_begin, l_end):
    check(_L().avsr_attn_rnn_fwd_lm(C.byref(desc), C.byref(lm_desc), int(l_begin), int(l_end), _s()), "avsr_attn_rnn_fwd_lm")


def beam_gather_tree(step_ids, parent_ids, beam_len, out, n_utt, beam_width, T, eos_id):
    check(_L().avsr_beam_gather_tree(fptr(step_ids), fptr(parent_ids), fptr(beam_len), fptr(out), n_utt, beam_width, T, eos_id, _s()),
          "avsr_beam_gather_tree")


def attn_alpha_rows(scores, dscores, mem_len, steplen, g, rowdot, B, L, T):
    check(_L().avsr_attn_alpha_rows(fptr(scores), fptr(dscores), fptr(mem_len), fptr(steplen), fptr(g), fptr(rowdot),
                                    B, L, T, _s()), "avsr_attn_alpha_rows")


def bahdanau_dkeys(keys, pq, pq_sb, pq_sl, dscores, v, bq, mem_len, dkeys, dv_part, B, L, T, H):
    check(_L().avsr_bahdanau_dkeys(fptr(keys), fptr(pq), pq_sb, pq_sl, fptr(dscores), fptr(v), fptr(bq),
                                   fptr(mem_len), fptr(dkeys), fptr(dv_part), B, L, T, H, _s()), "avsr_bahdanau_dkeys")


def transpose(jobs):
    arr = (TransposeJob * len(jobs))()
    for i, (s, so, d, do, r, c) in enumerate(jobs):
        arr[i] = TransposeJob(fptr(s, so), fptr(d, do), int(r), int(c))
    check(_L().avsr_transpose(arr, len(jobs), _s()), "avsr_transpose")


_colsum_batch = None


def colsum_batch_begin(grads):
    global _colsum_batch
    _colsum_batch = (grads, [])


def colsum_batch_flush(scratch):
    global _colsum_batch
    if _colsum_batch is None:
        return
    grads, jobs = _colsum_batch
    _colsum_batch = (grads, [])
    if jobs:
        from ._lib import ColsumJob
        arr = (ColsumJob * len(jobs))(*jobs)
        check(_L().avsr_colsum_multi(arr, len(jobs), fptr(scratch), scratch.numel(), _s()), "avsr_colsum_multi")


def colsum_batch_abort():
    global _colsum_batch
    _colsum_batch = None


def colsum_batch_end(scratch):
    global _colsum_batch
    colsum_batch_flush(scratch)
    _colsum_batch = None


def colsum(a, rows, F, out, scratch, b=None, alpha=1.0, beta=0.0, out_offset=0):
    if _colsum_batch is not None and out is _colsum_batch[0]:
        from ._lib import ColsumJob, Mat
        dst = fptr(out, out_offset)
        dups = [j for j in _colsum_batch[1] if j.out == dst]
        dup = bool(dups)
        if dup and (beta != 1.0 or any(j.beta != 1.0 for j in dups)):
            colsum_batch_flush(scratch)
            dup = False
        if not dup:
            _colsum_batch[1].append(ColsumJob(a, b if b is not None else Mat(None, 0, 0, 0, 0), dst, int(rows), int(F),
                                              float(alpha), float(beta)))
            return
    check(_L().avsr_colsum(C.byref(a), C.byref(b) if b is not None else None, rows, F, alpha, beta,
                           fptr(out, out_offset), fptr(scratch), scratch.numel(), _s()), "avsr_colsum")


def batchnorm_fwd(x, y, rows, F, gamma, beta, mov_mean, mov_var, save_mean, save_invstd, training, scratch):
    check(_L().avsr_batchnorm_fwd(fptr(x), fptr(y), rows, F, fptr(gamma), fptr(beta), fptr(mov_mean), fptr(mov_var),
                                  fptr(save_mean), fptr(save_invstd), int(training), fptr(scratch), scratch.numel(),
                                  _s()), "avsr_batchnorm_fwd")


def batchnorm_sync_sum(x, rows, F, sum_out, scratch):
    check(_L().avsr_batchnorm_sync_sum(fptr(x), rows, F, fptr(sum_out), fptr(scratch), scratch.numel(), _s()), "avsr_batchnorm_sync_sum")


def batchnorm_sync_sqsum(x, rows, F, sum_global, total_rows, mean_out, sq_out, scratch):
    check(_L().avsr_batchnorm_sync_sqsum(fptr(x), rows, F, fptr(sum_global), fptr(total_rows), fptr(mean_out), fptr(sq_out),
                                         fptr(scratch), scratch.numel(), _s()), "avsr_batchnorm_sync_sqsum")


def batchnorm_sync_apply(x, y, rows, F, gamma, beta, mov_mean, mov_var, mean, sq_global, total_rows, invstd_out, eps=1e-3, momentum=0.99,
                         relu=0):
    check(_L().avsr_batchnorm_sync_apply(fptr(x), fptr(y), rows, F, fptr(gamma), fptr(beta), fptr(mov_mean), fptr(mov_var), fptr(mean),
                                         fptr(sq_global), fptr(total_rows), fptr(invstd_out), float(eps), float(momentum), int(relu), _s()),
          "avsr_batchnorm_sync_apply")


def batchnorm_sync_moments(x, rows, F, out64, scratch):
    assert out64.dtype == torch.float64
    check(_L().avsr_batchnorm_sync_moments(fptr(x), rows, F, out64.data_ptr(), fptr(scratch), scratch.numel(), _s()), "avsr_batchnorm_sync_moments")


def dp_sync_unpack(buf64, dp_norm, streams):
    n = len(streams)
    off = (C.c_int32 * max(n, 1))(*[int(s[0]) for s in streams])
    Fs = (C.c_int32 * max(n, 1))(*[int(s[1]) for s in streams])
    mk = lambda k: (C.c_void_p * max(n, 1))(*[s[k].data_ptr() for s in streams])
    check(_L().avsr_dp_sync_unpack(buf64.data_ptr(), fptr(dp_norm), n, off, Fs, mk(2), mk(3), mk(4), _s()), "avsr_dp_sync_unpack")


def batchnorm_xhat(x, mean, invstd, xhat, rows, F):
    check(_L().avsr_batchnorm_xhat(fptr(x), fptr(mean), fptr(invstd), fptr(xhat), rows, F, _s()), "avsr_batchnorm_xhat")


def embed_labels(emb, labels, go_id, out, fed, B, L, E, n_steps=None):
    check(_L().avsr_embed_labels(fptr(emb), fptr(labels), go_id, fptr(out), fptr(fed), B, L, E, L if n_steps is None else n_steps,
                                 _s()), "avsr_embed_labels")


def embed_grad(dx, fed, demb, B, L, E, V, scratch):
    check(_L().avsr_embed_grad(fptr(dx), fptr(fed), fptr(demb), B, L, E, V, fptr(scratch), scratch.numel(), _s()), "avsr_embed_grad")


def dropout_rows(x, y, rows, cols, seed, stream_id, keep, idx_width, idx_coff=0, accumulate=False):
    check(_L().avsr_dropout_rows(C.byref(x), C.byref(y), rows, cols, fptr(seed), int(stream_id), float(keep), int(idx_width),
                                 int(idx_coff), int(accumulate), _s()), "avsr_dropout_rows")


LOSS_FUN = {None: 0, "label_smoothing": 1, "focal_loss": 2, "mc_loss": 3}


def seq_loss(logits, labels, labels_len, denom, compute_denom, row_loss, dlogits, B, L, V, loss_fun=0, label_smoothing=0.0):
    check(_L().avsr_seq_loss_fun(fptr(logits), fptr(labels), fptr(labels_len), fptr(denom), int(compute_denom),
                                 fptr(row_loss), fptr(dlogits), B, L, V, int(loss_fun), float(label_smoothing), _s()), "avsr_seq_loss_fun")


def au_loss(z, aus, lens, row_loss, dz, B, T, weight, total_count=None):
    check(_L().avsr_au_loss_dp(fptr(z), fptr(aus), fptr(lens), fptr(row_loss), fptr(dz), B, T, float(weight), fptr(total_count), _s()),
          "avsr_au_loss_dp")


def ctc_ws_floats(B, T, L):
    return int(_L().avsr_ctc_ws_floats(int(B), int(T), int(L)))


def ctc_loss(z, ld, labels, labels_len, in_len, denom, weight, nll, status, utt_loss, dz, ws, B, T, L, n_classes):
    from ._lib import CtcArgs
    a = CtcArgs()
    a.B, a.T, a.L, a.C, a.ld = int(B), int(T), int(L), int(n_classes), int(ld)
    a.z, a.labels, a.labels_len, a.in_len, a.denom = fptr(z), fptr(labels), fptr(labels_len), fptr(in_len), fptr(denom)
    a.weight = float(weight)
    a.nll, a.status, a.utt_loss, a.dz, a.ws, a.ws_floats = fptr(nll), fptr(status), fptr(utt_loss), fptr(dz), fptr(ws), int(ws.numel())
    check(_L().avsr_ctc_loss(C.byref(a), _s()), "avsr_ctc_loss")


def ctc_best_path(z, ld, in_len, B, T, n_classes, ids):
    check(_L().avsr_ctc_best_path(fptr(z), int(ld), fptr(in_len), int(B), int(T), int(n_classes), fptr(ids), _s()), "avsr_ctc_best_path")


def normed_v(v, g, vn, H):
    check(_L().avsr_normed_v(fptr(v), fptr(g), fptr(vn), H, _s()), "avsr_normed_v")


def normed_v_bwd(v, g, dvn, dv, dg, H):
    check(_L().avsr_normed_v_bwd(fptr(v), fptr(g), fptr(dvn), fptr(dv), fptr(dg), H, _s()), "avsr_normed_v_bwd")


def reduce_scalar(part, n, out, do_sqrt=False, accumulate=False, scale=1.0, out_offset=0):
    check(_L().avsr_reduce_scalar(fptr(part), n, fptr(out, out_offset), int(do_sqrt), int(accumulate), float(scale),
                                  _s()), "avsr_reduce_scalar")


def l2_regularise(segments, params, grads, l2, loss_accum, scratch):
    n = len(segments)
    if n == 0:
        return
    off = (C.c_int64 * n)(*[int(o) for o, _ in segments])
    cnt = (C.c_int64 * n)(*[int(c) for _, c in segments])
    check(_L().avsr_l2_regularise(off, cnt, n, fptr(params), fptr(grads), float(l2), fptr(loss_accum), fptr(scratch),
                                  _s()), "avsr_l2_regularise")


def global_norm(grads, n, norm_out, scratch, grad_scale=1.0):
    check(_L().avsr_global_norm(fptr(grads), n, float(grad_scale), fptr(norm_out), fptr(scratch), _s()),
          "avsr_global_norm")


def seq_loss_per_utterance(row_loss, labels_len, denom, out, B, L):
    check(_L().avsr_seq_loss_per_utterance(fptr(row_loss), fptr(labels_len), fptr(denom), fptr(out), B, L, _s()),
          "avsr_seq_loss_per_utterance")


def highway_fwd(x, h, cpre, y, lens, B, T, H):
    check(_L().avsr_highway_fwd(C.byref(x), C.byref(h), C.byref(cpre), C.byref(y), fptr(lens), B, T, H, _s()), "avsr_highway_fwd")


def highway_bwd(x, h, cpre, dy, dh, dcpre, dx, lens, B, T, H, accumulate_dx=False):
    check(_L().avsr_highway_bwd(C.byref(x), C.byref(h), C.byref(cpre), C.byref(dy), C.byref(dh), C.byref(dcpre), C.byref(dx), fptr(lens),
                                B, T, H, int(accumulate_dx), _s()), "avsr_highway_bwd")


def copy_(dst, src):
    assert dst.is_cuda and src.is_cuda and dst.numel() == src.numel() and dst.element_size() == 4 and src.element_size() == 4
    assert dst.is_contiguous() and src.is_contiguous() and dst.dtype == src.dtype
    check(_L().avsr_copy_words(dst.data_ptr(), src.data_ptr(), dst.numel(), _s()), "avsr_copy_words")


def zero_(dst):
    assert dst.is_cuda and dst.element_size() == 4 and dst.is_contiguous()
    check(_L().avsr_zero_words(dst.data_ptr(), dst.numel(), _s()), "avsr_zero_words")


def zero_multi(tensors):
    ts = [t for t in tensors if t is not None and t.numel()]
    if not ts:
        return
    for t in ts:
        assert t.is_cuda and t.element_size() == 4 and t.is_contiguous()
    ptrs = (C.c_void_p * len(ts))(*[t.data_ptr() for t in ts])
    cnt = (C.c_int64 * len(ts))(*[t.numel() for t in ts])
    check(_L().avsr_zero_multi(ptrs, cnt, len(ts), _s()), "avsr_zero_multi")


def add_int(a, b, out):
    check(_L().avsr_add_int(fptr(a), int(b), fptr(out), _s()), "avsr_add_int")


def instnorm_fwd(x, y, B, T, F, gamma, beta, mean_out, invstd_out, eps=1e-6):
    check(_L().avsr_instnorm_fwd(fptr(x), fptr(y), B, T, F, fptr(gamma), fptr(beta), fptr(mean_out), fptr(invstd_out), float(eps), _s()),
          "avsr_instnorm_fwd")


def instnorm_bwd(x, dy, gamma, mean, invstd, dx, dgamma_part, dbeta_part, B, T, F):
    check(_L().avsr_instnorm_bwd(fptr(x), fptr(dy), fptr(gamma), fptr(mean), fptr(invstd), fptr(dx), fptr(dgamma_part), fptr(dbeta_part),
                                 B, T, F, _s()), "avsr_instnorm_bwd")


OPTIMISER = {"Adam": 0, "Nadam": 1, "AdamW": 2, "Momentum": 3}


def adam_step(params, grads, m, v, n, gnorm, step, lr, warmup_steps, clip_norm, grad_scale=1.0, first_decay_steps=0, optimiser="Adam",
              weight_decay=0.0):
    check(_L().avsr_optimiser_step(fptr(params), fptr(grads), fptr(m), fptr(v), n, fptr(gnorm), fptr(step), float(lr),
                                   int(warmup_steps), int(first_decay_steps), float(clip_norm), float(grad_scale), OPTIMISER[optimiser],
                                   float(weight_decay), _s()), "avsr_optimiser_step")


PROF_KINDS = ("gemm", "step_lstm_fwd", "step_lstm_bwd", "step_dense", "attn_fwd", "attn_bwd", "rnn_persist_fwd", "rnn_persist_bwd", "dec_persist_fwd", "dec_persist_bwd",
              "conv_fwd", "conv_bwd_data", "conv_bwd_weight", "align_persist_fwd", "align_persist_bwd")


def prof_begin(max_launches=65536):
    check(_L().avsr_prof_begin(int(max_launches)), "avsr_prof_begin")


def prof_end():
    cnt = (C.c_int32 * len(PROF_KINDS))()
    ms = (C.c_float * len(PROF_KINDS))()
    fl = (C.c_double * len(PROF_KINDS))()
    check(_L().avsr_prof_end(cnt, ms, fl), "avsr_prof_end")
    return {k: (int(cnt[i]), float(ms[i]), float(fl[i])) for i, k in enumerate(PROF_KINDS)}


_persist_sync = None
_persist_scratch = None


def rnn_set_persistent(on, device="cuda", ints=1 << 20, mode=3, scratch_floats=64 << 20):
    global _persist_sync, _persist_scratch
    check(_L().avsr_rnn_set_persistent_mode(int(mode)), "avsr_rnn_set_persistent_mode")
    if on:
        if _persist_sync is None:
            _persist_sync = torch.zeros(ints, dtype=torch.int32, device=device)
        if (mode & 6) == 2 and _persist_scratch is None:
            _persist_scratch = torch.zeros(scratch_floats, dtype=torch.float32, device=device)
        if _persist_scratch is not None:
            check(_L().avsr_rnn_set_persistent_scratch(_persist_scratch.data_ptr(), _persist_scratch.numel()), "avsr_rnn_set_persistent_scratch")
        _persist_sync[:1].zero_()
        check(_L().avsr_rnn_set_persistent(_persist_sync.data_ptr(), ints), "avsr_rnn_set_persistent")
    else:
        check(_L().avsr_rnn_set_persistent(None, 0), "avsr_rnn_set_persistent")


def rnn_persistent_clear():
    if _persist_sync is not None:
        _persist_sync[:1].zero_()


def attn_rnn_fused_ws_floats(B, n_mech, Dmax=256):
    return int(_L().avsr_attn_rnn_fused_ws_floats(int(B), int(n_mech), int(Dmax)))


def attn_rnn_fused_eligible(desc):
    return bool(_L().avsr_attn_rnn_fused_eligible(C.byref(desc)))


def attn_rnn_fused_fwd_active(desc):
    return bool(_L().avsr_attn_rnn_fused_fwd_active(C.byref(desc)))


def attn_rnn_set_fused(on):
    check(_L().avsr_attn_rnn_set_fused(int(on)), "avsr_attn_rnn_set_fused")


def attn_rnn_set_beam_kernel(on):
    check(_L().avsr_attn_rnn_set_beam_kernel(int(on)), "avsr_attn_rnn_set_beam_kernel")


def rnn_persistent_error():
    return bool(_persist_sync is not None and int(_persist_sync[:1].item()) != 0)


def batchnorm_fwd_ex(x, y, rows, F, gamma, beta, mov_mean, mov_var, save_mean, save_invstd, training, eps, momentum, relu, scratch, bessel=1):
    check(_L().avsr_batchnorm_fwd_ex(fptr(x), fptr(y), rows, F, fptr(gamma), fptr(beta), fptr(mov_mean), fptr(mov_var), fptr(save_mean),
                                     fptr(save_invstd), int(training), float(eps), float(momentum), int(relu), int(bessel), fptr(scratch),
                                     scratch.numel(), _s()), "avsr_batchnorm_fwd_ex")


def batchnorm_bwd(x, dy, gamma, beta, mean, invstd, dx, dgamma, dbeta, rows, F, relu, scratch, dx_beta=0.0):
    check(_L().avsr_batchnorm_bwd(fptr(x), fptr(dy), fptr(gamma), fptr(beta), fptr(mean), fptr(invstd), fptr(dx), fptr(dgamma), fptr(dbeta),
                                  rows, F, int(relu), float(dx_beta), fptr(scratch), scratch.numel(), _s()), "avsr_batchnorm_bwd")


def im2col(x, col, N, H, W, Cc, kh, kw, stride, pad_t, pad_l, Ho, Wo):
    check(_L().avsr_im2col(fptr(x), fptr(col), N, H, W, Cc, kh, kw, stride, pad_t, pad_l, Ho, Wo, _s()), "avsr_im2col")


def col2im(dcol, dx, N, H, W, Cc, kh, kw, stride, pad_t, pad_l, Ho, Wo, beta=0.0):
    check(_L().avsr_col2im(fptr(dcol), fptr(dx), N, H, W, Cc, kh, kw, stride, pad_t, pad_l, Ho, Wo, float(beta), _s()), "avsr_col2im")


def relu(x, y, n):
    check(_L().avsr_relu(fptr(x), fptr(y), int(n), _s()), "avsr_relu")


def relu_bwd(y, dy, dx, n):
    check(_L().avsr_relu_bwd(fptr(y), fptr(dy), fptr(dx), int(n), _s()), "avsr_relu_bwd")


def add(a, b, out, n):
    check(_L().avsr_add(fptr(a), fptr(b), fptr(out), int(n), _s()), "avsr_add")


def conv3x3_supported(Ci, Co, H, W):
    return bool(_L().avsr_conv3x3_supported(Ci, Co, H, W))


def conv3x3(x, w, bias, y, N, H, W, Ci, Co, stride, pad_t, pad_l, Ho, Wo, flip=0, beta=0.0):
    check(_L().avsr_conv3x3(fptr(x), fptr(w), fptr(bias), fptr(y), N, H, W, Ci, Co, stride, pad_t, pad_l, Ho, Wo, int(flip), float(beta), _s()),
          "avsr_conv3x3")


def conv_set_mfma(on):
    check(_L().avsr_conv_set_mfma(int(on)), "avsr_conv_set_mfma")


def conv_desc(N, H, W, Ci, Co, k, stride, pad_t, pad_l, Ho, Wo, bn=None):
    from ._lib import ConvDesc
    d = ConvDesc(N, H, W, Ci, Co, k, stride, pad_t, pad_l, Ho, Wo, 0, None, None)
    if bn is not None:
        d.bn_scale, d.bn_shift = fptr(bn[0]), fptr(bn[1])
    return d


def conv_supported(d):
    return bool(_L().avsr_conv_supported(C.byref(d)))


def conv_fwd(d, x, w, bias, y, res=None, res_bn=None, stats=None):
    n = C.c_int32(0)
    check(_L().avsr_conv_fwd(C.byref(d), fptr(x), fptr(w), fptr(bias), fptr(res), fptr(res_bn[0]) if res_bn else None,
                             fptr(res_bn[1]) if res_bn else None, fptr(y), fptr(stats), C.byref(n), _s()), "avsr_conv_fwd")
    return int(n.value)


def conv_bwd_data(d, dy, w, dx, beta=0.0):
    check(_L().avsr_conv_bwd_data(C.byref(d), fptr(dy), fptr(w), fptr(dx), float(beta), _s()), "avsr_conv_bwd_data")


def conv_bwd_data_bn_supported(d):
    return bool(_L().avsr_conv_bwd_data_bn_supported(C.byref(d)))


def conv_bwd_data_bn(d, dy, w, dx, beta=0.0, acc=None, bn_x=None, bn=None, stats=None):
    n = C.c_int32(0)
    check(_L().avsr_conv_bwd_data_bn(C.byref(d), fptr(dy), fptr(w), fptr(dx), float(beta), fptr(acc), fptr(bn_x),
                                     fptr(bn[0]) if bn else None, fptr(bn[1]) if bn else None, fptr(stats), C.byref(n), _s()), "avsr_conv_bwd_data_bn")
    return int(n.value)


def bn_bwd_finalize(part, nparts, Cn, count, mean, invstd, gamma, dgamma, dbeta, k, grad_beta=1.0):
    check(_L().avsr_bn_bwd_finalize(fptr(part), int(nparts), int(Cn), int(count), fptr(mean), fptr(invstd), fptr(gamma), fptr(dgamma), fptr(dbeta),
                                    float(grad_beta), fptr(k), _s()), "avsr_bn_bwd_finalize")


def bn_partials_f64(part, nparts, Cn, out64):
    check(_L().avsr_bn_partials_f64(fptr(part), int(nparts), int(Cn), out64.data_ptr(), _s()), "avsr_bn_partials_f64")

# ... 145 lines not shown
```

include/avsr_hip.h:

```cpp
#ifndef AVSR_HIP_H
#define AVSR_HIP_H
#include <stdint.h>

#ifdef __cplusplus
extern "C" {
#endif
#if defined(__GNUC__) || defined(__clang__)
#pragma GCC visibility push(default)
#endif

#define AVSR_OK 0
#define AVSR_ERR_ARG (-1)
#define AVSR_ERR_HIP (-2)
#define AVSR_ERR_UNSUPPORTED (-3)

#define AVSR_MAX_LAYERS 4
#define AVSR_MAX_MECH 4
#define AVSR_MAX_STACKS 4
#define AVSR_HAVE_ATTN 1
#define AVSR_MAX_TRANSPOSE 16
#define AVSR_MAX_SEGMENTS 32

int avsr_abi_version(void);
int64_t avsr_sizeof(const char* name);
// ... 120 lines not shown
#define AVSR_MAX_DEC_EXTRA 3

typedef struct avsr_attn_rnn {
  int32_t B, L, H, E, n_mech, output_attention, V, mode;
  int32_t go_id, eos_id;
  int32_t* steplen;
  const float* wt;
  const float* w;
  const float* bias;
  float* gates;
  float* cs;
  float* cell_out;
  float* att;
  const float* h0;
  const float* c0;
  float* state;
  float* h_final;
  float* c_final;
  avsr_attn_mech mech[AVSR_MAX_MECH];
  const float* embedding;
  const float* wout_t;
  const float* bout;
  float* logits;
  int32_t* ids;
  int32_t* tok;
  int32_t* n_unfinished;
  float* dgates;
  float* dstate;
  float* datt;
  float* dq;
  const float* datt_ext;
  const float* dcell_ext;
  float* dh0;
  float* dc0;
  const float* dh_final;
  const float* dc_final;
  const int32_t* seed;
  float keep_in, keep_state, keep_out, sampling_prob;
  int32_t cell_id, pad3_;
  float* hs_seq;
  float* attd;
  float* xs;
  const int32_t* labels;
  int32_t* fed;
  int32_t cell, pad4_;
  const float* wt2;
  const float* w2;
  const float* bias2;
  float* rh_seq;
  float* dgates2;
  int32_t beam_width, mem_shared;
  float length_penalty;
  float pad6_;
  float* beam_logp;
  int32_t* beam_fin;
  int32_t* beam_len;
  int32_t* step_ids;
  int32_t* parent_ids;
  int32_t* parent_rows;
  int32_t n_extra, prof_tag;
  float* out0;
  avsr_dec_layer extra[AVSR_MAX_DEC_EXTRA];
  float* fused_ws;
  int64_t fused_ws_floats;
} avsr_attn_rnn;
int64_t avsr_attn_rnn_fused_ws_floats(int32_t B, int32_t n_mech, int32_t Dmax);
int avsr_attn_rnn_fused_eligible(const avsr_attn_rnn* d);
int avsr_attn_rnn_fused_fwd_active(const avsr_attn_rnn* d);
int avsr_attn_rnn_set_fused(int32_t on);
int avsr_attn_rnn_set_beam_kernel(int32_t on);

int avsr_attn_rnn_fwd(const avsr_attn_rnn* d, int32_t l_begin, int32_t l_end, void* stream);
int avsr_attn_rnn_bwd(const avsr_attn_rnn* d, void* stream);
int avsr_beam_gather_tree(const int32_t* step_ids, const int32_t* parent_ids, const int32_t* beam_len, int32_t* out,
                          int32_t n_utt, int32_t beam_width, int32_t T, int32_t eos_id, void* stream);

int avsr_beam_search_step(float* logits, int32_t n_utt, int32_t beam_width, int32_t V, int32_t step, int32_t eos_id,
                          float length_penalty_weight, const float* logp_in, const int32_t* fin_in, const int32_t* len_in,
                          float* logp_out, int32_t* fin_out, int32_t* len_out, int32_t* tok, int32_t* parent_rows,
                          int32_t* step_ids, int32_t* parent_ids, int32_t* n_unfinished, const float* x, int64_t x_stride,
                          int32_t O, const float* wout_t, const float* bout, void* stream);

#define AVSR_MAX_LM_LAYERS 4
typedef struct avsr_beam_lm {
  int32_t n_layers, H, E, V;
  int32_t one_hot, n_rows;
  float lm_weight;
  int32_t pad_;
  const float* embedding;
  const float* wt[AVSR_MAX_LM_LAYERS];
  const float* bias[AVSR_MAX_LM_LAYERS];
  const float* wout_t;
  const float* bout;
  float* state_c;
  float* state_h;
  float* lm_logp;
} avsr_beam_lm;
int avsr_beam_lm_supported(const avsr_beam_lm* lm);
int avsr_beam_lm_step(const avsr_beam_lm* lm, const int32_t* tok, const int32_t* parent_rows, int32_t n_rows, int32_t step, void* stream);
int avsr_beam_search_step_lm(float* logits, int32_t n_utt, int32_t beam_width, int32_t V, int32_t step, int32_t eos_id,
                             float length_penalty_weight, const float* logp_in, const int32_t* fin_in, const int32_t* len_in,
                             float* logp_out, int32_t* fin_out, int32_t* len_out, int32_t* tok, int32_t* parent_rows,
                             int32_t* step_ids, int32_t* parent_ids, int32_t* n_unfinished, const float* x, int64_t x_stride,
                             int32_t O, const float* wout_t, const float* bout, const float* lm_logp, float lm_weight, void* stream);
int avsr_attn_rnn_fwd_lm(const avsr_attn_rnn* d, const avsr_beam_lm* lm, int32_t l_begin, int32_t l_end, void* stream);

#define AVSR_BEAM_CTC_MAX_T 2048
#define AVSR_BEAM_CTC_MAX_V 256
typedef struct avsr_beam_ctc {
  int32_t n_utt, beam_width, T, V;
  int32_t eos_id;
  float weight;
  int64_t ld;
  const float* z;
  const int32_t* in_len;
  float* y;
  float* state;
  float* psi;
  int32_t* last;
  float* term;
  float* extra;
  const float* lm_logp;
  float lm_weight;
  int32_t pad_;
} avsr_beam_ctc;
int avsr_beam_ctc_supported(const avsr_beam_ctc* ctc);
int avsr_beam_ctc_begin(const avsr_beam_ctc* ctc, void* stream);
int avsr_beam_ctc_step(const avsr_beam_ctc* ctc, const int32_t* tok, const int32_t* parent_rows, const int32_t* fin, int32_t step,
                       void* stream);
int avsr_beam_search_step_ctc(float* logits, int32_t n_utt, int32_t beam_width, int32_t V, int32_t step, int32_t eos_id,
                              float length_penalty_weight, const float* logp_in, const int32_t* fin_in, const int32_t* len_in,
                              float* logp_out, int32_t* fin_out, int32_t* len_out, int32_t* tok, int32_t* parent_rows,
                              int32_t* step_ids, int32_t* parent_ids, int32_t* n_unfinished, const float* x, int64_t x_stride,
                              int32_t O, const float* wout_t, const float* bout, const float* lm_logp, float lm_weight,
                              const float* ctc_term, float ctc_weight, float* extra, void* stream);
int avsr_attn_rnn_fwd_ctc(const avsr_attn_rnn* d, const avsr_beam_lm* lm, const avsr_beam_ctc* ctc, int32_t l_begin, int32_t l_end,
                          void* stream);

int avsr_attn_alpha_rows(float* scores, const float* dscores, const int32_t* len, const int32_t* steplen,
                         const float* g, float* rowdot, int32_t B, int32_t L, int32_t T, void* stream);
int avsr_bahdanau_dkeys(const float* keys, const float* pq, int64_t pq_sb, int64_t pq_sl, const float* dscores,
                        const float* v, const float* bq, const int32_t* len, float* dkeys, float* dv_part,
                        int32_t B, int32_t L, int32_t T, int32_t H, void* stream);

typedef struct avsr_transpose_job {
  const float* src;
  float* dst;
  int32_t rows, cols;
} avsr_transpose_job;
int avsr_transpose(const avsr_transpose_job* jobs, int32_t n, void* stream);

int avsr_colsum(const avsr_mat* a, const avsr_mat* b, int32_t rows, int32_t F, float alpha, float beta, float* out,
                float* scratch, int64_t scratch_floats, void* stream);

int avsr_batchnorm_fwd(const float* x, float* y, int32_t rows, int32_t F, const float* gamma, const float* beta,
                       float* moving_mean, float* moving_var, float* save_mean, float* save_invstd, int32_t training,
                       float* scratch, int64_t scratch_floats, void* stream);
int avsr_batchnorm_fwd_ex(const float* x, float* y, int32_t rows, int32_t F, const float* gamma, const float* beta,
                          float* moving_mean, float* moving_var, float* save_mean, float* save_invstd, int32_t training,
                          float eps, float momentum, int32_t relu, int32_t bessel, float* scratch, int64_t scratch_floats,
                          void* stream);
int avsr_batchnorm_sync_sum(const float* x, int32_t rows, int32_t F, float* sum_out, float* scratch, int64_t scratch_floats,
                            void* stream);
int avsr_batchnorm_sync_sqsum(const float* x, int32_t rows, int32_t F, const float* sum_global, const float* total_rows,
                              float* mean_out, float* sq_out, float* scratch, int64_t scratch_floats, void* stream);
int avsr_batchnorm_sync_moments(const float* x, int32_t rows, int32_t F, double* out64, float* scratch, int64_t scratch_floats, void* stream);
int avsr_dp_sync_unpack(const double* buf, float* dp_norm, int32_t nstream, const int32_t* off, const int32_t* F, float* const* mean,
                        float* const* sq, float* const* rows, void* stream);
int avsr_batchnorm_sync_apply(const float* x, float* y, int32_t rows, int32_t F, const float* gamma, const float* beta,
                              float* moving_mean, float* moving_var, const float* mean, const float* sq_global,
                              const float* total_rows, float* invstd_out, float eps, float momentum, int32_t relu, void* stream);
int avsr_batchnorm_bwd(const float* x, const float* dy, const float* gamma, const float* beta, const float* mean,
                       const float* invstd, float* dx, float* dgamma, float* dbeta, int32_t rows, int32_t F, int32_t relu,
                       float dx_beta, float* scratch, int64_t scratch_floats, void* stream);

int avsr_im2col(const float* x, float* col, int32_t N, int32_t H, int32_t W, int32_t C, int32_t kh, int32_t kw, int32_t stride,
                int32_t pad_t, int32_t pad_l, int32_t Ho, int32_t Wo, void* stream);
int avsr_col2im(const float* dcol, float* dx, int32_t N, int32_t H, int32_t W, int32_t C, int32_t kh, int32_t kw, int32_t stride,
                int32_t pad_t, int32_t pad_l, int32_t Ho, int32_t Wo, float beta, void* stream);
int avsr_conv3x3_supported(int32_t Ci, int32_t Co, int32_t H, int32_t W);
int avsr_conv_set_mfma(int32_t on);
typedef struct avsr_conv_desc {
  int32_t N, H, W, Ci, Co, k, stride, pad_t, pad_l, Ho, Wo, pad_;
  const float* bn_scale;
  const float* bn_shift;
} avsr_conv_desc;
int avsr_conv_supported(const avsr_conv_desc* c);
int avsr_conv_fwd(const avsr_conv_desc* c, const float* x, const float* w, const float* bias, const float* res, const float* res_scale,
                  const float* res_shift, float* y, float* stats, int32_t* nparts, void* stream);
int avsr_conv_bwd_data(const avsr_conv_desc* c, const float* dy, const float* w, float* dx, float beta, void* stream);
int avsr_conv_bwd_weight(const avsr_conv_desc* c, const float* x, const float* dy, float* dw, float* dbias, float beta, float* scratch,
                         int64_t scratch_floats, void* stream);
int avsr_conv_bwd_data_bn(const avsr_conv_desc* c, const float* dy, const float* w, float* dx, float beta, const float* acc,
                          const float* bn_x, const float* bn_scale, const float* bn_shift, float* stats, int32_t* nparts, void* stream);
int avsr_conv_bwd_data_bn_supported(const avsr_conv_desc* c);
int avsr_conv_bwd_weight_bn(const avsr_conv_desc* c, const float* x, const float* dz, const float* y, const float* k, float* dx_out,
                            float* dw, float* dbias, float beta, float* scratch, int64_t scratch_floats, void* stream);
int avsr_conv_bwd_weight_bn_supported(const avsr_conv_desc* c);
#define AVSR_CONV_PLAN_BIAS 1
#define AVSR_CONV_PLAN_RES 2
#define AVSR_CONV_PLAN_STATS 4
#define AVSR_CONV_PLAN_BETA 8
#define AVSR_CONV_PLAN_ACC 16
#define AVSR_CONV_PLAN_BNB 32
#define AVSR_CONV_PLAN_FOLD 64
#define AVSR_CONV_PLAN_FOLD_DX 128
#define AVSR_CONV_PLAN_DBIAS 256
typedef struct avsr_conv_launch {
  int32_t kernel, m, ntc, ch4, rs, fold, ep, nsp;
  int32_t ntap, t0, F, grid, CsP, lds_bytes, slab, pad_;
} avsr_conv_launch;
int avsr_conv_plan(const avsr_conv_desc* c, int32_t op, int32_t flags, int64_t scratch_floats, avsr_conv_launch* out, int32_t cap);
int avsr_bn_bwd_finalize(const float* part, int32_t nparts, int32_t C, int64_t count, const float* mean, const float* invstd,
                         const float* gamma, float* dgamma, float* dbeta, float grad_beta, float* k, void* stream);
int avsr_bn_bwd_apply(const float* dz, const float* x, const float* k, float* dx, int64_t rows, int32_t C, float beta, void* stream);
int avsr_bn_bwd_stage1(const float* dy, const float* x, const float* scale, const float* shift, const float* y, float* dz, int64_t rows,
                       int32_t C, float* part, int32_t* nparts, void* stream);
int avsr_bn_finalize(const float* part, int32_t nparts, int32_t C, int64_t count, float eps, float momentum, float* mean, float* invstd,
                     float* mov_mean, float* mov_var, const float* gamma, const float* beta, float* scale, float* shift, void* stream);
int avsr_bn_partials_f64(const float* part, int32_t nparts, int32_t C, double* out64, void* stream);
int avsr_bn_finalize_f64(const double* sums, int32_t C, float eps, float momentum, float* mean, float* invstd, float* mov_mean,
                         float* mov_var, const float* gamma, const float* beta, float* scale, float* shift, void* stream);
int avsr_bn_bwd_finalize_f64(const double* local, const double* global, int32_t C, const float* mean, const float* invstd,
                             const float* gamma, float* dgamma, float* dbeta, float grad_beta, float* k, void* stream);
int avsr_bn_eval_affine(const float* gamma, const float* beta, const float* mov_mean, const float* mov_var, float eps, float* scale,
                        float* shift, int32_t C, void* stream);
int avsr_batchnorm_apply(const float* x, float* y, int32_t rows, int32_t F, const float* gamma, const float* beta, const float* mean,
                         const float* invstd, int32_t relu, void* stream);
int avsr_conv3x3(const float* x, const float* w, const float* bias, float* y, int32_t N, int32_t H, int32_t W, int32_t Ci, int32_t Co,
                 int32_t stride, int32_t pad_t, int32_t pad_l, int32_t Ho, int32_t Wo, int32_t flip, float beta, void* stream);
int avsr_conv3x3_bwd_data_s2(const float* dy, const float* w, float* dx, int32_t N, int32_t H, int32_t W, int32_t Ci, int32_t Co,
                             int32_t pad_t, int32_t pad_l, int32_t Ho, int32_t Wo, float beta, void* stream);
int avsr_conv3x3_bwd_weight(const float* x, const float* dy, float* dw, int32_t N, int32_t H, int32_t W, int32_t Ci, int32_t Co,
                            int32_t stride, int32_t pad_t, int32_t pad_l, int32_t Ho, int32_t Wo, float beta, float* scratch,
                            int64_t scratch_floats, void* stream);
typedef struct avsr_conv3d_desc {
  int32_t B, T, H, W, Ci, Co;
  int32_t kt, kh, kw, stride;
  int32_t pad_f, pad_t, pad_l, Ho, Wo, relu;
  const float* scale;
  const float* shift;
} avsr_conv3d_desc;
int avsr_conv3d_supported(const avsr_conv3d_desc* c);
int64_t avsr_conv3d_wgrad_scratch_floats(const avsr_conv3d_desc* c);
int avsr_conv3d_fwd(const avsr_conv3d_desc* c, const float* x, const float* w, const float* res, const float* res_scale, const float* res_shift,
                    float* y, float* stats, int32_t* nparts, void* stream);
int avsr_conv3d_bwd_data(const avsr_conv3d_desc* c, const float* dy, const float* w, float* dx, float beta, void* stream);
int avsr_conv3d_bwd_weight(const avsr_conv3d_desc* c, const float* x, const float* dy, float* dw, float beta, float* scratch,
                           int64_t scratch_floats, void* stream);
int avsr_conv3d_bn_finalize(const float* part, int32_t nparts, int32_t C, int64_t count, float eps, float momentum, float* mean,
                            float* invstd, float* mov_mean, float* mov_var, const float* gamma, const float* beta, float* scale,
                            float* shift, void* stream);
typedef struct avsr_logmel_args {
  int32_t B, N, T_out, F;
  int32_t frame_length, frame_step, fft_length, num_mel_bins;
  int32_t window, stride, mel_nnz, pad_;
  const float* wav;
  const int32_t* wav_len;
  const float* hann;
  const float* twiddle;
  const int32_t* mel_lo;
  const int32_t* mel_cnt;
  const int32_t* mel_ptr;
  const float* mel_w;
  float* out;
  int32_t* out_len;
} avsr_logmel_args;
int avsr_logmel_supported(int32_t frame_length, int32_t fft_length, int32_t num_mel_bins, int32_t window, int32_t stride);
int avsr_logmel_fwd(const avsr_logmel_args* a, void* stream);
typedef struct avsr_ctc_args {
  int32_t B, T, L, C;
  int64_t ld;
  const float* z;
  const int32_t* labels;
  const int32_t* labels_len;
  const int32_t* in_len;
  const float* denom;
  float weight;
  int32_t pad_;
  float* nll;
  int32_t* status;
  float* utt_loss;
  float* dz;
  float* ws;
  int64_t ws_floats;
} avsr_ctc_args;
int avsr_ctc_loss(const avsr_ctc_args* a, void* stream);
int64_t avsr_ctc_ws_floats(int32_t B, int32_t T, int32_t L);
int avsr_ctc_best_path(const float* z, int64_t ld, const int32_t* in_len, int32_t B, int32_t T, int32_t C, int32_t* ids, void* stream);
int avsr_relu(const float* x, float* y, int64_t n, void* stream);
int avsr_relu_bwd(const float* y, const float* dy, float* dx, int64_t n, void* stream);
int avsr_add(const float* a, const float* b, float* out, int64_t n, void* stream);
int avsr_selu(const float* z, float* y, int64_t n, void* stream);
int avsr_selu_bwd(const float* z, const float* dy, float* dz, int64_t n, void* stream);

int avsr_batchnorm_xhat(const float* x, const float* mean, const float* invstd, float* xhat, int32_t rows, int32_t F,
                        void* stream);

int avsr_embed_labels(const float* emb, const int32_t* labels, int32_t go_id, float* out, int32_t* fed, int32_t B,
                      int32_t L, int32_t E, int32_t n_steps, void* stream);
int avsr_embed_grad(const float* dx, const int32_t* fed, float* demb, int32_t B, int32_t L, int32_t E, int32_t V,
                    float* scratch, int64_t scratch_floats, void* stream);

int avsr_dropout_rows(const avsr_mat* x, const avsr_mat* y, int32_t rows, int32_t cols, const int32_t* seed,
                      int32_t stream_id, float keep, int32_t idx_width, int32_t idx_coff, int32_t accumulate, void* stream);

int avsr_seq_loss(float* logits, const int32_t* labels, const int32_t* labels_len, float* denom,
                  int32_t compute_denom, float* row_loss, float* dlogits, int32_t B, int32_t L, int32_t V, void* stream);
int avsr_seq_loss_fun(float* logits, const int32_t* labels, const int32_t* labels_len, float* denom, int32_t compute_denom,
                      float* row_loss, float* dlogits, int32_t B, int32_t L, int32_t V, int32_t loss_fun,
                      float label_smoothing, void* stream);

int avsr_seq_loss_per_utterance(const float* row_loss, const int32_t* labels_len, const float* denom, float* out, int32_t B,
                                int32_t L, void* stream);
int avsr_instnorm_fwd(const float* x, float* y, int32_t B, int32_t T, int32_t F, const float* gamma, const float* beta,
                      float* mean_out, float* invstd_out, float eps, void* stream);
int avsr_instnorm_bwd(const float* x, const float* dy, const float* gamma, const float* mean, const float* invstd, float* dx,
                      float* dgamma_part, float* dbeta_part, int32_t B, int32_t T, int32_t F, void* stream);
int avsr_highway_fwd(const avsr_mat* x, const avsr_mat* h, const avsr_mat* carry_pre, const avsr_mat* y, const int32_t* len,
                     int32_t B, int32_t T, int32_t H, void* stream);
int avsr_highway_bwd(const avsr_mat* x, const avsr_mat* h, const avsr_mat* carry_pre, const avsr_mat* dy, const avsr_mat* dh,
                     const avsr_mat* dcarry_pre, const avsr_mat* dx, const int32_t* len, int32_t B, int32_t T, int32_t H,
                     int32_t accumulate_dx, void* stream);
int avsr_copy_words(void* dst, const void* src, int64_t n_words, void* stream);
int avsr_zero_words(void* dst, int64_t n_words, void* stream);
int avsr_zero_multi(void* const* ptrs, const int64_t* n_words, int32_t count, void* stream);
int avsr_add_int(const int32_t* a, int32_t b, int32_t* out, void* stream);
typedef struct avsr_colsum_job {
  avsr_mat a;
  avsr_mat b;
  float* out;
  int32_t rows, F;
  float alpha, beta;
} avsr_colsum_job;
int avsr_colsum_multi(const avsr_colsum_job* jobs, int32_t n, float* scratch, int64_t scratch_floats, void* stream);
int avsr_slab_defer_begin(void);
int avsr_slab_defer_end(void* stream);
int avsr_au_loss(const float* z, const float* aus, const int32_t* len, float* row_loss, float* dz, int32_t B, int32_t T,
                 float weight, void* stream);
int avsr_au_loss_dp(const float* z, const float* aus, const int32_t* len, float* row_loss, float* dz, int32_t B, int32_t T,
                    float weight, const float* total_count, void* stream);

int avsr_normed_v(const float* v, const float* g, float* vn, int32_t H, void* stream);
int avsr_normed_v_bwd(const float* v, const float* g, const float* dvn, float* dv, float* dg, int32_t H, void* stream);

int avsr_reduce_scalar(const float* part, int32_t n, float* out, int32_t do_sqrt, int32_t accumulate, float scale,
                       void* stream);

int avsr_l2_regularise(const int64_t* seg_off, const int64_t* seg_n, int32_t nseg, const float* params, float* grads,
                       float l2, float* loss_accum, float* scratch, void* stream);
int avsr_global_norm(const float* grads, int64_t n, float grad_scale, float* norm_out, float* scratch, void* stream);
int avsr_adam_step(float* params, float* grads, float* m, float* v, int64_t n, const float* global_norm, int32_t* step,
                   float lr, int32_t warmup_steps, float clip_norm, float grad_scale, void* stream);
int avsr_adam_step_decay(float* params, float* grads, float* m, float* v, int64_t n, const float* global_norm,
                         int32_t* step, float lr, int32_t warmup_steps, int32_t first_decay_steps, float clip_norm,
                         float grad_scale, void* stream);
int avsr_optimiser_step(float* params, float* grads, float* m, float* v, int64_t n, const float* global_norm, int32_t* step,
                        float lr, int32_t warmup_steps, int32_t first_decay_steps, float clip_norm, float grad_scale,
                        int32_t optimiser, float weight_decay, void* stream);

#define AVSR_PROF_NKIND 15
int avsr_prof_begin(int32_t max_launches);
int avsr_prof_end(int32_t* out_count, float* out_ms, double* out_flops);

#if defined(__GNUC__) || defined(__clang__)
#pragma GCC visibility pop
#endif
#ifdef __cplusplus
}
#endif
#endif
```

Before: 5713 utterances/sec.

## Batch encoder batchnorms with dropout, fuse loss assembly and optimiser step

Adds a multi-map batchnorm forward that computes statistics and applies normalisation for up to four encoder streams in one set of five launches, and folds the first-layer input dropout into the apply kernel. It also adds a loss-assembly kernel and a fused optimiser step that combines L2 regularisation, global-norm computation and the Adam update. The aim is fewer kernel launches and fewer passes over activations and parameters in the train step. The cost is extra code paths and a changed floating-point order in the moving-variance update, which uses fma.

```diff
diff --git a/avsr-tf1_amd/_lib.py b/avsr-tf1_amd/_lib.py
--- a/avsr-tf1_amd/_lib.py
+++ b/avsr-tf1_amd/_lib.py
@@ -151,13 +151,19 @@
     _fields_ = [("a", Mat), ("b", Mat), ("out", C.c_void_p), ("rows", C.c_int32), ("F", C.c_int32), ("alpha", C.c_float), ("beta", C.c_float)]
 
 
+class BnMap(C.Structure):
+    _fields_ = [("x", C.c_void_p), ("y", C.c_void_p), ("gamma", C.c_void_p), ("beta", C.c_void_p), ("moving_mean", C.c_void_p),
+                ("moving_var", C.c_void_p), ("save_mean", C.c_void_p), ("save_invstd", C.c_void_p), ("drop_out", C.c_void_p * 2),
+                ("drop_stream", C.c_int32 * 2), ("drop_keep", C.c_float * 2), ("rows", C.c_int32), ("F", C.c_int32)]
+
+
 class TransposeJob(C.Structure):
     _fields_ = [("src", C.c_void_p), ("dst", C.c_void_p), ("rows", C.c_int32), ("cols", C.c_int32)]
 
 
 _STRUCTS = {"avsr_dec_layer": DecLayer, "avsr_mat": Mat, "avsr_gemm_desc": GemmDesc, "avsr_rnn_layer": RnnLayer, "avsr_rnn_stack": RnnStack,
             "avsr_conv_desc": ConvDesc, "avsr_conv_launch": ConvLaunch, "avsr_conv3d_desc": Conv3dDesc, "avsr_logmel_args": LogmelArgs, "avsr_ctc_args": CtcArgs, "avsr_attn_mech": AttnMech, "avsr_attn_rnn": AttnRnn, "avsr_transpose_job": TransposeJob,
-            "avsr_colsum_job": ColsumJob, "avsr_beam_lm": BeamLm, "avsr_beam_ctc": BeamCtc}
+            "avsr_colsum_job": ColsumJob, "avsr_bn_map": BnMap, "avsr_beam_lm": BeamLm, "avsr_beam_ctc": BeamCtc}
 
 _vp, _i32, _i64, _f32 = C.c_void_p, C.c_int32, C.c_int64, C.c_float
 _SIGS = {
@@ -220,6 +226,7 @@
     "avsr_transpose": [C.POINTER(TransposeJob), _i32, _vp],
     "avsr_colsum": [C.POINTER(Mat), C.POINTER(Mat), _i32, _i32, _f32, _f32, _vp, _vp, _i64, _vp],
     "avsr_batchnorm_fwd": [_vp, _vp, _i32, _i32, _vp, _vp, _vp, _vp, _vp, _vp, _i32, _vp, _i64, _vp],
+    "avsr_batchnorm_fwd_multi": [C.POINTER(BnMap), _i32, _vp, _vp, _i64, _vp],
     "avsr_batchnorm_xhat": [_vp, _vp, _vp, _vp, _i32, _i32, _vp],
     "avsr_batchnorm_fwd_ex": [_vp, _vp, _i32, _i32, _vp, _vp, _vp, _vp, _vp, _vp, _i32, _f32, _f32, _i32, _i32, _vp, _i64, _vp],
     "avsr_batchnorm_bwd": [_vp, _vp, _vp, _vp, _vp, _vp, _vp, _vp, _vp, _i32, _i32, _i32, _f32, _vp, _i64, _vp],
@@ -244,6 +251,7 @@
     "avsr_normed_v": [_vp, _vp, _vp, _i32, _vp],
     "avsr_normed_v_bwd": [_vp, _vp, _vp, _vp, _vp, _i32, _vp],
     "avsr_reduce_scalar": [_vp, _i32, _vp, _i32, _i32, _f32, _vp],
+    "avsr_loss_assemble": [C.POINTER(_vp), C.POINTER(_i32), _i32, _vp, _vp],
     "avsr_l2_regularise": [C.POINTER(_i64), C.POINTER(_i64), _i32, _vp, _vp, _f32, _vp, _vp, _vp],
     "avsr_global_norm": [_vp, _i64, _f32, _vp, _vp, _vp],
     "avsr_adam_step": [_vp, _vp, _vp, _vp, _i64, _vp, _vp, _f32, _i32, _f32, _f32, _vp],
@@ -256,6 +264,8 @@
     "avsr_instnorm_fwd": [_vp, _vp, _i32, _i32, _i32, _vp, _vp, _vp, _vp, _f32, _vp],
     "avsr_instnorm_bwd": [_vp, _vp, _vp, _vp, _vp, _vp, _vp, _vp, _i32, _i32, _i32, _vp],
     "avsr_optimiser_step": [_vp, _vp, _vp, _vp, _i64, _vp, _vp, _f32, _i32, _i32, _f32, _f32, _i32, _f32, _vp],
+    "avsr_optimiser_step_fused": [_vp, _vp, _vp, _vp, _i64, C.POINTER(_i64), C.POINTER(_i64), C.POINTER(_i32), C.POINTER(_f32), _i32, _vp, _vp, _vp,
+                                  _f32, _i32, _i32, _f32, _f32, _i32, _f32, _vp, _i64, _vp],
     "avsr_highway_fwd": [_vp, _vp, _vp, _vp, _vp, _i32, _i32, _i32, _vp],
     "avsr_highway_bwd": [_vp, _vp, _vp, _vp, _vp, _vp, _vp, _vp, _i32, _i32, _i32, _i32, _vp],
     "avsr_copy_words": [_vp, _vp, _i64, _vp],
diff --git a/avsr-tf1_amd/csrc/batchnorm.hip b/avsr-tf1_amd/csrc/batchnorm.hip
--- a/avsr-tf1_amd/csrc/batchnorm.hip
+++ b/avsr-tf1_amd/csrc/batchnorm.hip
@@ -6,10 +6,9 @@
 
 namespace {
 
-__global__ void bn_partial_sum_kernel(const float* x, float* part, int rows, int F, int rows_per_blk) {
-  __shared__ float red[256];
+__device__ __forceinline__ void bn_partial_sum_block(const float* x, float* part, int rows, int F, int rows_per_blk, int blk, float* red) {
   const int G = F < 256 ? 256 / F : 1;
-  const int r0 = blockIdx.x * rows_per_blk, r1 = min(rows, r0 + rows_per_blk);
+  const int r0 = blk * rows_per_blk, r1 = min(rows, r0 + rows_per_blk);
   for (int base = 0; base < (G > 1 ? 1 : F); base += blockDim.x) {
     const int idx = base + threadIdx.x;
     const int f = G > 1 ? idx % F : idx, g = G > 1 ? idx / F : 0;
@@ -19,34 +18,43 @@
       for (; r + G < r1; r += 2 * G) { s0 += x[(long)r * F + f]; s1 += x[(long)(r + G) * F + f]; }
       if (r < r1) s0 += x[(long)r * F + f];
     }
-    if (G > 1) block_group_reduce(s0 + s1, idx, F, G, red, part + (long)blockIdx.x * F);
-    else if (idx < F) part[(long)blockIdx.x * F + idx] = s0 + s1;
-  }
-}
-
-__global__ __launch_bounds__(1024) void bn_mean_kernel(const float* part, int npart, float* mean, int rows, int F,
-                                                       const float* total = nullptr) {
-  if (total) rows = (int)total[0];
-  __shared__ double red[32][33];
+    if (G > 1) block_group_reduce(s0 + s1, idx, F, G, red, part + (long)blk * F);
+    else if (idx < F) part[(long)blk * F + idx] = s0 + s1;
+  }
+}
+__global__ void bn_partial_sum_kernel(const float* x, float* part, int rows, int F, int rows_per_blk) {
+  __shared__ float red[256];
+  bn_partial_sum_block(x, part, rows, F, rows_per_blk, blockIdx.x, red);
+}
+
+__device__ __forceinline__ bool bn_column_total(const float* part, int npart, int F, int fblk, double (*red)[33], double* t_out) {
   const int fl = threadIdx.x & 31, g = threadIdx.x >> 5;
-  const int f = blockIdx.x * 32 + fl;
+  const int f = fblk * 32 + fl;
   double s = 0.0;
   if (f < F)
     for (int i = g; i < npart; i += 32) s += (double)part[(long)i * F + f];
   red[g][fl] = s;
   __syncthreads();
-  if (g == 0 && f < F) {
-    double t = 0.0;
-#pragma unroll
-    for (int j = 0; j < 32; ++j) t += red[j][fl];
-    mean[f] = (float)(t / rows);
-  }
-}
-
-__global__ void bn_partial_sq_kernel(const float* x, const float* mean_v, float* part, int rows, int F, int rows_per_blk) {
-  __shared__ float red[256];
+  if (g != 0 || f >= F) return false;
+  double t = 0.0;
+#pragma unroll
+  for (int j = 0; j < 32; ++j) t += red[j][fl];
+  *t_out = t;
+  return true;
+}
+
+__global__ __launch_bounds__(1024) void bn_mean_kernel(const float* part, int npart, float* mean, int rows, int F,
+                                                       const float* total = nullptr) {
+  if (total) rows = (int)total[0];
+  __shared__ double red[32][33];
+  double t;
+  if (bn_column_total(part, npart, F, blockIdx.x, red, &t)) mean[blockIdx.x * 32 + (threadIdx.x & 31)] = (float)(t / rows);
+}
+
+__device__ __forceinline__ void bn_partial_sq_block(const float* x, const float* mean_v, float* part, int rows, int F, int rows_per_blk,
+                                                    int blk, float* red) {
   const int G = F < 256 ? 256 / F : 1;
-  const int r0 = blockIdx.x * rows_per_blk, r1 = min(rows, r0 + rows_per_blk);
+  const int r0 = blk * rows_per_blk, r1 = min(rows, r0 + rows_per_blk);
   for (int base = 0; base < (G > 1 ? 1 : F); base += blockDim.x) {
     const int idx = base + threadIdx.x;
     const int f = G > 1 ? idx % F : idx, g = G > 1 ? idx / F : 0;
@@ -60,8 +68,24 @@
       }
       if (r < r1) { const float d0 = x[(long)r * F + f] - mean; s0 += d0 * d0; }
     }
-    if (G > 1) block_group_reduce(s0 + s1, idx, F, G, red, part + (long)blockIdx.x * F);
-    else if (idx < F) part[(long)blockIdx.x * F + idx] = s0 + s1;
+    if (G > 1) block_group_reduce(s0 + s1, idx, F, G, red, part + (long)blk * F);
+    else if (idx < F) part[(long)blk * F + idx] = s0 + s1;
+  }
+}
+__global__ void bn_partial_sq_kernel(const float* x, const float* mean_v, float* part, int rows, int F, int rows_per_blk) {
+  __shared__ float red[256];
+  bn_partial_sq_block(x, mean_v, part, rows, F, rows_per_blk, blockIdx.x, red);
+}
+
+__device__ __forceinline__ void bn_var_finish(double t, int f, const float* mean_v, float* invstd_v, float* mov_mean, float* mov_var, int rows,
+                                              float eps, float momentum, int bessel) {
+#pragma clang fp contract(off)
+  const float var = (float)(t / rows), mean = mean_v[f];
+  invstd_v[f] = rsqrtf(var + eps);
+  if (mov_mean) {
+    const float unbiased = bessel ? var * ((float)rows / (float)max(1, rows - 1)) : var;
+    mov_mean[f] = momentum * mov_mean[f] + (1.f - momentum) * mean;
+    mov_var[f] = __builtin_fmaf(1.f - momentum, unbiased, momentum * mov_var[f]);
   }
 }
 
@@ -70,25 +94,9 @@
                                                       int bessel, const float* total = nullptr) {
   if (total) rows = (int)total[0];
   __shared__ double red[32][33];
-  const int fl = threadIdx.x & 31, g = threadIdx.x >> 5;
-  const int f = blockIdx.x * 32 + fl;
-  double s = 0.0;
-  if (f < F)
-    for (int i = g; i < npart; i += 32) s += (double)part[(long)i * F + f];
-  red[g][fl] = s;
-  __syncthreads();
-  if (g == 0 && f < F) {
-    double t = 0.0;
-#pragma unroll
-    for (int j = 0; j < 32; ++j) t += red[j][fl];
-    const float var = (float)(t / rows), mean = mean_v[f];
-    invstd_v[f] = rsqrtf(var + eps);
-    if (mov_mean) {
-      const float unbiased = bessel ? var * ((float)rows / (float)max(1, rows - 1)) : var;
-      mov_mean[f] = momentum * mov_mean[f] + (1.f - momentum) * mean;
-      mov_var[f] = momentum * mov_var[f] + (1.f - momentum) * unbiased;
-    }
-  }
+  double t;
+  if (bn_column_total(part, npart, F, blockIdx.x, red, &t))
+    bn_var_finish(t, blockIdx.x * 32 + (threadIdx.x & 31), mean_v, invstd_v, mov_mean, mov_var, rows, eps, momentum, bessel);
 }
 
 __global__ void bn_apply_kernel(const float* x, const float* mean_v, const float* invstd_v, const float* mov_mean, const float* mov_var,
@@ -127,6 +135,86 @@
   }
   *rpb_out = rpb;
   return nblk;
+}
+
+#define BNF_MAX 4
+struct BnfMap {
+  const float* x; float* y;
+  const float* gamma; const float* beta;
+  float* mov_mean; float* mov_var; float* mean; float* invstd;
+  float* part;
+  float* drop[2]; uint32_t drop_stream[2]; float drop_keep[2];
+  int rows, F, nblk, rpb, ablk;
+};
+struct BnfLaunch { int n; int blk0[BNF_MAX + 1]; int fblk0[BNF_MAX + 1]; int ablk0[BNF_MAX + 1]; const int32_t* seed; float eps, momentum; int bessel; BnfMap m[BNF_MAX]; };
+
+__device__ __forceinline__ int bnf_map_of_block(const int* blk0, int n) {
+  int j = 0;
+#pragma unroll 1
+  for (int k = 1; k < n; ++k) if ((int)blockIdx.x >= blk0[k]) j = k;
+  return __builtin_amdgcn_readfirstlane(j);
+}
+
+__global__ __launch_bounds__(256) void bnf_sum_kernel(const BnfLaunch L) {
+  __shared__ float red[256];
+  const int j = bnf_map_of_block(L.blk0, L.n);
+  const BnfMap& M = L.m[j];
+  bn_partial_sum_block(M.x, M.part, M.rows, M.F, M.rpb, (int)blockIdx.x - L.blk0[j], red);
+}
+__global__ __launch_bounds__(1024) void bnf_mean_kernel(const BnfLaunch L) {
+  __shared__ double red[32][33];
+  const int j = bnf_map_of_block(L.fblk0, L.n);
+  const BnfMap& M = L.m[j];
+  const int fblk = (int)blockIdx.x - L.fblk0[j];
+  double t;
+  if (bn_column_total(M.part, M.nblk, M.F, fblk, red, &t)) M.mean[fblk * 32 + (threadIdx.x & 31)] = (float)(t / M.rows);
+}
+__global__ __launch_bounds__(256) void bnf_sq_kernel(const BnfLaunch L) {
+  __shared__ float red[256];
+  const int j = bnf_map_of_block(L.blk0, L.n);
+  const BnfMap& M = L.m[j];
+  bn_partial_sq_block(M.x, M.mean, M.part, M.rows, M.F, M.rpb, (int)blockIdx.x - L.blk0[j], red);
+}
+__global__ __launch_bounds__(1024) void bnf_var_kernel(const BnfLaunch L) {
+  __shared__ double red[32][33];
+  const int j = bnf_map_of_block(L.fblk0, L.n);
+  const BnfMap& M = L.m[j];
+  const int fblk = (int)blockIdx.x - L.fblk0[j];
+  double t;
+  if (bn_column_total(M.part, M.nblk, M.F, fblk, red, &t))
+    bn_var_finish(t, fblk * 32 + (threadIdx.x & 31), M.mean, M.invstd, M.mov_mean, M.mov_var, M.rows, L.eps, L.momentum, L.bessel);
+}
+
+__global__ __launch_bounds__(256) void bnf_apply_kernel(const BnfLaunch L) {
+  const int j = bnf_map_of_block(L.ablk0, L.n);
+  const BnfMap& M = L.m[j];
+  const int F = M.F;
+  const long n4 = (long)M.rows * F / 4;
+  const uint32_t sd = L.seed ? (uint32_t)L.seed[0] : 0u;
+  const bool on0 = L.seed && M.drop_keep[0] < 1.0f, on1 = L.seed && M.drop_keep[1] < 1.0f;
+  const float inv0 = 1.0f / M.drop_keep[0], inv1 = 1.0f / M.drop_keep[1];
+  for (long i = (long)((int)blockIdx.x - L.ablk0[j]) * 256 + threadIdx.x; i < n4; i += (long)M.ablk * 256) {
+    const int f = (int)((i * 4) % F);
+    const f32x4 xv = ld4(M.x + i * 4);
+    f32x4 yv;
+#pragma unroll
+    for (int e = 0; e < 4; ++e) yv[e] = __builtin_fmaf(xv[e] - M.mean[f + e], M.gamma[f + e] * M.invstd[f + e], M.beta[f + e]);
+    if (M.y) st4(M.y + i * 4, yv);
+    if (M.drop[0]) {
+      f32x4 d;
+#pragma unroll
+      for (int e = 0; e < 4; ++e)
+        d[e] = !on0 ? yv[e] : (uniform01(sd, M.drop_stream[0], (uint32_t)(i * 4 + e)) < M.drop_keep[0] ? yv[e] * inv0 : 0.f);
+      st4(M.drop[0] + i * 4, d);
+    }
+    if (M.drop[1]) {
+      f32x4 d;
+#pragma unroll
+      for (int e = 0; e < 4; ++e)
+        d[e] = !on1 ? yv[e] : (uniform01(sd, M.drop_stream[1], (uint32_t)(i * 4 + e)) < M.drop_keep[1] ? yv[e] * inv1 : 0.f);
+      st4(M.drop[1] + i * 4, d);
+    }
+  }
 }
 
 }
@@ -172,6 +260,51 @@
                                0 , scratch, scratch_floats, stream);
 }
 
+extern "C" int avsr_batchnorm_fwd_multi(const avsr_bn_map* maps, int32_t n, const int32_t* seed, float* scratch, int64_t scratch_floats,
+                                        void* stream) {
+  if (n <= 0) return AVSR_OK;
+  if (!maps || !scratch || n > BNF_MAX) return AVSR_ERR_ARG;
+  BnfLaunch L = {};
+  L.seed = seed; L.eps = 1e-3f; L.momentum = 0.99f; L.bessel = 0;
+  long used = 0;
+  for (int k = 0; k < n; ++k) {
+    const avsr_bn_map& Q = maps[k];
+    if (Q.rows < 0 || Q.F <= 0 || Q.F % 4) return AVSR_ERR_ARG;
+    if (Q.rows == 0) continue;
+    if (!Q.x || !Q.gamma || !Q.beta || !Q.save_mean || !Q.save_invstd || (!Q.moving_mean) != (!Q.moving_var)) return AVSR_ERR_ARG;
+    for (int d = 0; d < 2; ++d)
+      if (Q.drop_out[d] && !(Q.drop_keep[d] > 0.f)) return AVSR_ERR_ARG;
+    BnfMap& M = L.m[L.n];
+    int rpb;
+    const int nblk = bn_blocks(Q.rows, Q.F, (int64_t)1 << 40, &rpb);
+    M.x = Q.x; M.y = Q.y; M.gamma = Q.gamma; M.beta = Q.beta; M.mov_mean = Q.moving_mean; M.mov_var = Q.moving_var;
+    M.mean = Q.save_mean; M.invstd = Q.save_invstd;
+    M.part = scratch + used;
+    used += (long)nblk * Q.F;
+    for (int d = 0; d < 2; ++d) { M.drop[d] = Q.drop_out[d]; M.drop_stream[d] = (uint32_t)Q.drop_stream[d]; M.drop_keep[d] = Q.drop_out[d] ? Q.drop_keep[d] : 1.f; }
+    M.rows = Q.rows; M.F = Q.F; M.nblk = nblk; M.rpb = rpb;
+    const long n4 = (long)Q.rows * Q.F / 4;
+    M.ablk = (int)((n4 + 255) / 256 > 1024 ? 1024 : (n4 + 255) / 256);
+    L.blk0[L.n + 1] = L.blk0[L.n] + nblk;
+    L.fblk0[L.n + 1] = L.fblk0[L.n] + (Q.F + 31) / 32;
+    L.ablk0[L.n + 1] = L.ablk0[L.n] + M.ablk;
+    ++L.n;
+  }
+  if (used > scratch_floats) return AVSR_ERR_ARG;
+  if (!L.n) return AVSR_OK;
+  hipLaunchKernelGGL(bnf_sum_kernel, dim3(L.blk0[L.n]), dim3(256), 0, S_(stream), L);
+  AVSR_CHECK_LAUNCH();
+  hipLaunchKernelGGL(bnf_mean_kernel, dim3(L.fblk0[L.n]), dim3(1024), 0, S_(stream), L);
+  AVSR_CHECK_LAUNCH();
+  hipLaunchKernelGGL(bnf_sq_kernel, dim3(L.blk0[L.n]), dim3(256), 0, S_(stream), L);
+  AVSR_CHECK_LAUNCH();
+  hipLaunchKernelGGL(bnf_var_kernel, dim3(L.fblk0[L.n]), dim3(1024), 0, S_(stream), L);
+  AVSR_CHECK_LAUNCH();
+  hipLaunchKernelGGL(bnf_apply_kernel, dim3(L.ablk0[L.n]), dim3(256), 0, S_(stream), L);
+  AVSR_CHECK_LAUNCH();
+  return AVSR_OK;
+}
+
 extern "C" int avsr_batchnorm_apply(const float* x, float* y, int32_t rows, int32_t F, const float* gamma, const float* beta, const float* mean,
                                     const float* invstd, int32_t relu, void* stream) {
   if (!x || !y || !gamma || !beta || !mean || !invstd || rows <= 0 || F <= 0 || F % 4) return AVSR_ERR_ARG;
diff --git a/avsr-tf1_amd/csrc/capi.hip b/avsr-tf1_amd/csrc/capi.hip
--- a/avsr-tf1_amd/csrc/capi.hip
+++ b/avsr-tf1_amd/csrc/capi.hip
@@ -6,7 +6,7 @@
 extern "C" int64_t avsr_sizeof(const char* name) {
   if (!name) return -1;
 #define SZ(T) if (!strcmp(name, #T)) return (int64_t)sizeof(T);
-  SZ(avsr_mat) SZ(avsr_gemm_desc) SZ(avsr_conv_desc) SZ(avsr_conv_launch) SZ(avsr_conv3d_desc) SZ(avsr_logmel_args) SZ(avsr_ctc_args) SZ(avsr_rnn_layer) SZ(avsr_rnn_stack) SZ(avsr_colsum_job)
+  SZ(avsr_mat) SZ(avsr_gemm_desc) SZ(avsr_conv_desc) SZ(avsr_conv_launch) SZ(avsr_conv3d_desc) SZ(avsr_logmel_args) SZ(avsr_ctc_args) SZ(avsr_rnn_layer) SZ(avsr_rnn_stack) SZ(avsr_colsum_job) SZ(avsr_bn_map)
 #ifdef AVSR_HAVE_ATTN
   SZ(avsr_attn_mech) SZ(avsr_attn_rnn) SZ(avsr_transpose_job) SZ(avsr_dec_layer) SZ(avsr_beam_lm) SZ(avsr_beam_ctc)
 #endif
diff --git a/avsr-tf1_amd/csrc/elementwise.hip b/avsr-tf1_amd/csrc/elementwise.hip
--- a/avsr-tf1_amd/csrc/elementwise.hip
+++ b/avsr-tf1_amd/csrc/elementwise.hip
@@ -80,15 +80,23 @@
 
 __global__ void set_scalar_kernel(float* p, float v) { p[0] = v; }
 
-__global__ void seq_loss_kernel(float* logits, const int32_t* labels, const int32_t* len, const float* denom,
-                                float* row_loss, float* dlogits, int B, int L, int V, int mode, float smooth) {
+__global__ void seq_loss_kernel(float* logits, const int32_t* labels, const int32_t* len, float* denom,
+                                float* row_loss, float* dlogits, int B, int L, int V, int mode, float smooth, int denom_mode) {
   const int row = blockIdx.x * blockDim.x + threadIdx.x;
+  float dn;
+  if (denom_mode == 0) dn = denom[0];
+  else if (denom_mode == 2) dn = (float)B * (float)L;
+  else {
+    dn = 0.f;
+    for (int b = 0; b < B; ++b) dn += (float)min(max(len[b], 0), L);
+  }
+  if (denom_mode != 0 && row == 0) denom[0] = dn;
   if (row >= B * L) return;
   const int b = row / L, l = row % L;
   float* lg = logits + (long)row * V;
   float* dl = dlogits ? dlogits + (long)row * V : nullptr;
   const bool valid = l < len[b];
-  const float inv = 1.f / (denom[0] + 1e-12f);
+  const float inv = 1.f / (dn + 1e-12f);
   if (!valid) {
     row_loss[row] = mode == 1 ? logf((float)V) * inv : 0.f;
     for (int v = 0; v < V; ++v) lg[v] = 0.f;
@@ -237,10 +245,9 @@
   }
 }
 
-__global__ void adam_kernel(float* p, float* g, float* m, float* v, long n, const float* gnorm, int32_t* step,
-                            float lr, int warmup, float clip, float b1, float b2, float eps, float grad_scale,
-                            int decay_steps, int opt, float weight_decay) {
-  const int t = step[0] + 1;
+struct AdamRates { float lr_now, lr_t, scale; };
+__device__ __forceinline__ AdamRates adam_rates(int t, float gnorm, float lr, int warmup, float clip, float b1, float b2, float grad_scale,
+                                                int decay_steps) {
   float lr_now = lr;
   if (decay_steps > 0) {
     const float frac = (float)(t - 1) / (float)decay_steps;
@@ -254,26 +261,140 @@
   const double c2 = 1.0 - exp((double)t * log((double)b2));
   const float lr_t = (float)((double)lr_now * sqrt(c2) / c1);
   float scale = grad_scale;
-  if (clip > 0.f) scale *= clip / fmaxf(gnorm[0], clip);
+  if (clip > 0.f) scale *= clip / fmaxf(gnorm, clip);
+  return AdamRates{lr_now, lr_t, scale};
+}
+
+__device__ __forceinline__ void adam_element(float* p, float* m, float* v, long i, float graw, const AdamRates& R, float b1, float b2,
+                                             float eps, int opt, float weight_decay) {
+  const float gi = graw * R.scale;
+  if (opt == 3) {
+    const float acc = 0.9f * m[i] + gi;
+    m[i] = acc;
+    p[i] -= R.lr_now * acc;
+    return;
+  }
+  const float mi = b1 * m[i] + (1.f - b1) * gi;
+  const float vi = b2 * v[i] + (1.f - b2) * gi * gi;
+  m[i] = mi;
+  v[i] = vi;
+  float pi = p[i];
+  if (opt == 2) pi -= weight_decay * pi;
+  const float num = opt == 1 ? b1 * mi + (1.f - b1) * gi : mi;
+  p[i] = pi - R.lr_t * num / (sqrtf(vi) + eps);
+}
+
+__global__ void adam_kernel(float* p, float* g, float* m, float* v, long n, const float* gnorm, int32_t* step,
+                            float lr, int warmup, float clip, float b1, float b2, float eps, float grad_scale,
+                            int decay_steps, int opt, float weight_decay) {
+  const AdamRates R = adam_rates(step[0] + 1, clip > 0.f ? gnorm[0] : 0.f, lr, warmup, clip, b1, b2, grad_scale, decay_steps);
+  for (long i = (long)blockIdx.x * blockDim.x + threadIdx.x; i < n; i += (long)gridDim.x * blockDim.x)
+    adam_element(p, m, v, i, g[i], R, b1, b2, eps, opt, weight_decay);
+}
+__global__ void step_inc_kernel(int32_t* step) { step[0] += 1; }
+
+#define FUSED_MAX_SEG (3 * AVSR_MAX_SEGMENTS)
+#define FUSED_MAX_GROUP 8
+#define L2_GX 64
+struct FSeg { long off, n; float l2; };
+struct FusedSegs {
+  int nseg, ngroup, nlook;
+  int group_first[FUSED_MAX_GROUP + 1];
+  FSeg seg[FUSED_MAX_SEG];
+  unsigned char by_off[FUSED_MAX_SEG];
+};
+
+__device__ __forceinline__ void fused_stage_segs(const FusedSegs& S, long* s_off, long* s_end, float* s_l2) {
+  for (int k = threadIdx.x; k < S.nlook; k += blockDim.x) {
+    const FSeg sg = S.seg[S.by_off[k]];
+    s_off[k] = sg.off; s_end[k] = sg.off + sg.n; s_l2[k] = sg.l2;
+  }
+  __syncthreads();
+}
+__device__ __forceinline__ bool fused_l2_of(long i, int nlook, const long* s_off, const long* s_end, const float* s_l2, float* l2) {
+  int lo = 0, hi = nlook;
+  while (lo < hi) {
+    const int mid = (lo + hi) >> 1;
+    if (s_off[mid] <= i) lo = mid + 1; else hi = mid;
+  }
+  if (lo == 0 || i >= s_end[lo - 1]) return false;
+  *l2 = s_l2[lo - 1];
+  return true;
+}
+
+__global__ __launch_bounds__(256) void optimiser_fused_partial_kernel(const FusedSegs S, const float* w, const float* g, long n, int gx,
+                                                                      float* part, float* reg, const int32_t* step, int32_t* step_copy) {
+  __shared__ float red[4];
+  __shared__ long s_off[FUSED_MAX_SEG], s_end[FUSED_MAX_SEG];
+  __shared__ float s_l2[FUSED_MAX_SEG];
+  if (blockIdx.x == 0 && threadIdx.x == 0) step_copy[0] = step[0];
+  if ((int)blockIdx.x >= gx) {
+    const int b = (int)blockIdx.x - gx, k = b / L2_GX, bx = b % L2_GX;
+    const FSeg sg = S.seg[k];
+    float s = 0.f;
+    for (long i = (long)bx * 256 + threadIdx.x; i < sg.n; i += (long)L2_GX * 256) {
+      const float x = w[sg.off + i];
+      s += x * x;
+    }
+    s = block_sum_256(s, red);
+    if (threadIdx.x == 0) reg[b] = 0.5f * sg.l2 * s;
+    return;
+  }
+  fused_stage_segs(S, s_off, s_end, s_l2);
+  float s = 0.f;
+  for (long i = (long)blockIdx.x * 256 + threadIdx.x; i < n; i += (long)gx * 256) {
+    float l2, gi = g[i];
+    if (fused_l2_of(i, S.nlook, s_off, s_end, s_l2, &l2)) gi += l2 * w[i];
+    s += gi * gi;
+  }
+  s = block_sum_256(s, red);
+  if (threadIdx.x == 0) part[blockIdx.x] = s;
+}
+
+__device__ __forceinline__ double reduce_partials_256(const float* part, int n, double* dred) {
+  double s = 0.0;
+  for (int i = threadIdx.x; i < n; i += 256) s += (double)part[i];
+  __syncthreads();
+  dred[threadIdx.x] = s;
+  __syncthreads();
+  for (int o = 128; o > 0; o >>= 1) {
+    if (threadIdx.x < o) dred[threadIdx.x] += dred[threadIdx.x + o];
+    __syncthreads();
+  }
+  return dred[0];
+}
+
+__global__ __launch_bounds__(256) void optimiser_fused_apply_kernel(const FusedSegs S, float* p, float* g, float* m, float* v, long n,
+                                                                    const float* part, int gx, const float* reg, float* loss_accum,
+                                                                    float* gnorm_out, int32_t* step, const int32_t* step_copy, float lr,
+                                                                    int warmup, float clip, float b1, float b2, float eps, float grad_scale,
+                                                                    int decay_steps, int opt, float weight_decay) {
+  __shared__ double dred[256];
+  __shared__ long s_off[FUSED_MAX_SEG], s_end[FUSED_MAX_SEG];
+  __shared__ float s_l2[FUSED_MAX_SEG];
+  fused_stage_segs(S, s_off, s_end, s_l2);
+  double nv = sqrt(reduce_partials_256(part, gx, dred));
+  nv *= grad_scale;
+  const float gn = (float)nv;
+  const int t0 = step_copy[0];
+  if (blockIdx.x == 0) {
+    if (loss_accum) {
+      float loss = loss_accum[0];
+      for (int k = 0; k < S.ngroup; ++k) {
+        const int f = S.group_first[k], cnt = S.group_first[k + 1] - f;
+        loss = loss + (float)reduce_partials_256(reg + (long)f * L2_GX, cnt * L2_GX, dred);
+      }
+      if (threadIdx.x == 0) loss_accum[0] = loss;
+    }
+    if (threadIdx.x == 0) { gnorm_out[0] = gn; step[0] = t0 + 1; }
+  }
+  const AdamRates R = adam_rates(t0 + 1, gn, lr, warmup, clip, b1, b2, grad_scale, decay_steps);
   for (long i = (long)blockIdx.x * blockDim.x + threadIdx.x; i < n; i += (long)gridDim.x * blockDim.x) {
-    const float gi = g[i] * scale;
-    if (opt == 3) {
-      const float acc = 0.9f * m[i] + gi;
-      m[i] = acc;
-      p[i] -= lr_now * acc;
-      continue;
-    }
-    const float mi = b1 * m[i] + (1.f - b1) * gi;
-    const float vi = b2 * v[i] + (1.f - b2) * gi * gi;
-    m[i] = mi;
-    v[i] = vi;
-    float pi = p[i];
-    if (opt == 2) pi -= weight_decay * pi;
-    const float num = opt == 1 ? b1 * mi + (1.f - b1) * gi : mi;
-    p[i] = pi - lr_t * num / (sqrtf(vi) + eps);
-  }
-}
-__global__ void step_inc_kernel(int32_t* step) { step[0] += 1; }
+    float l2, gi = g[i];
+    if (fused_l2_of(i, S.nlook, s_off, s_end, s_l2, &l2)) { gi += l2 * p[i]; g[i] = gi; }
+    adam_element(p, m, v, i, gi, R, b1, b2, eps, opt, weight_decay);
+  }
+}
 
 struct HwView { float* p; long ld; int T; long ldo; };
 __device__ __forceinline__ long hw_off(const HwView& v, int r) { return rowoff(r, v.ld, v.T, v.ldo); }
@@ -450,13 +571,14 @@
                                  int32_t compute_denom, float* row_loss, float* dlogits, int32_t B, int32_t L, int32_t V,
                                  int32_t loss_fun, float label_smoothing, void* stream) {
   if (!logits || !labels || !labels_len || !denom || !row_loss || loss_fun < 0 || loss_fun > 3) return AVSR_ERR_ARG;
-  if (compute_denom) {
+  const bool in_kernel = compute_denom && (long)B * L < (1L << 24) && B * L > 0;
+  if (compute_denom && !in_kernel) {
     if (loss_fun == 1) hipLaunchKernelGGL(set_scalar_kernel, dim3(1), dim3(1), 0, S_(stream), denom, (float)B * (float)L);
     else hipLaunchKernelGGL(seqlen_sum_kernel, dim3(1), dim3(256), 0, S_(stream), labels_len, B, L, denom);
     AVSR_CHECK_LAUNCH();
   }
   hipLaunchKernelGGL(seq_loss_kernel, dim3((B * L + 127) / 128), dim3(128), 0, S_(stream), logits, labels, labels_len,
-                     denom, row_loss, dlogits, B, L, V, loss_fun, label_smoothing);
+                     denom, row_loss, dlogits, B, L, V, loss_fun, label_smoothing, in_kernel ? (loss_fun == 1 ? 2 : 1) : 0);
   AVSR_CHECK_LAUNCH();
   return AVSR_OK;
 }
@@ -533,6 +655,29 @@
                                   float scale, void* stream) {
   if (!part || !out || n <= 0) return AVSR_ERR_ARG;
   hipLaunchKernelGGL(reduce_scalar_kernel, dim3(1), dim3(256), 0, S_(stream), part, n, out, do_sqrt, accumulate, scale);
+  AVSR_CHECK_LAUNCH();
+  return AVSR_OK;
+}
+
+struct LossTerms { int n; const float* part[8]; int cnt[8]; };
+__global__ __launch_bounds__(256) void loss_assemble_kernel(const LossTerms T, float* out) {
+  __shared__ double dred[256];
+  float loss = 0.f;
+  for (int k = 0; k < T.n; ++k) {
+    const float v = (float)avsr::reduce_partials_256(T.part[k], T.cnt[k], dred);
+    loss = k ? loss + v : v;
+  }
+  if (threadIdx.x == 0) out[0] = loss;
+}
+extern "C" int avsr_loss_assemble(const float* const* parts, const int32_t* n, int32_t count, float* out, void* stream) {
+  if (!parts || !n || !out || count <= 0 || count > 8) return AVSR_ERR_ARG;
+  LossTerms T = {};
+  T.n = count;
+  for (int k = 0; k < count; ++k) {
+    if (!parts[k] || n[k] <= 0) return AVSR_ERR_ARG;
+    T.part[k] = parts[k]; T.cnt[k] = n[k];
+  }
+  hipLaunchKernelGGL(loss_assemble_kernel, dim3(1), dim3(256), 0, S_(stream), T, out);
   AVSR_CHECK_LAUNCH();
   return AVSR_OK;
 }
@@ -590,3 +735,48 @@
   AVSR_CHECK_LAUNCH();
   return AVSR_OK;
 }
+
+extern "C" int avsr_optimiser_step_fused(float* params, float* grads, float* m, float* v, int64_t n, const int64_t* seg_off,
+                                         const int64_t* seg_n, const int32_t* group_nseg, const float* group_l2, int32_t ngroup,
+                                         float* loss_accum, float* gnorm_out, int32_t* step, float lr, int32_t warmup_steps,
+                                         int32_t first_decay_steps, float clip_norm, float grad_scale, int32_t optimiser, float weight_decay,
+                                         float* scratch, int64_t scratch_floats, void* stream) {
+  if (!params || !grads || !m || !v || !step || !gnorm_out || !scratch || n <= 0 || first_decay_steps < 0 || optimiser < 0 || optimiser > 3)
+    return AVSR_ERR_ARG;
+  if (ngroup < 0 || ngroup > FUSED_MAX_GROUP || (ngroup > 0 && (!seg_off || !seg_n || !group_nseg || !group_l2))) return AVSR_ERR_ARG;
+  FusedSegs S = {};
+  for (int k = 0; k < ngroup; ++k) {
+    if (group_nseg[k] < 0 || group_nseg[k] > AVSR_MAX_SEGMENTS || S.nseg + group_nseg[k] > FUSED_MAX_SEG) return AVSR_ERR_ARG;
+    if (group_nseg[k] == 0) continue;
+    S.group_first[S.ngroup] = S.nseg;
+    for (int i = 0; i < group_nseg[k]; ++i, ++S.nseg) {
+      const int64_t off = seg_off[S.nseg], cnt = seg_n[S.nseg];
+      if (off < 0 || cnt < 0 || off + cnt > n) return AVSR_ERR_ARG;
+      S.seg[S.nseg] = FSeg{(long)off, (long)cnt, group_l2[k]};
+    }
+    S.group_first[++S.ngroup] = S.nseg;
+  }
+  for (int i = 0; i < S.nseg; ++i)
+    if (S.seg[i].n > 0) S.by_off[S.nlook++] = (unsigned char)i;
+  for (int i = 1; i < S.nlook; ++i)
+    for (int j = i; j > 0 && S.seg[S.by_off[j - 1]].off > S.seg[S.by_off[j]].off; --j) {
+      const unsigned char t = S.by_off[j]; S.by_off[j] = S.by_off[j - 1]; S.by_off[j - 1] = t;
+    }
+  for (int i = 1; i < S.nlook; ++i) {
+    const FSeg& a = S.seg[S.by_off[i - 1]];
+    if (a.off + a.n > S.seg[S.by_off[i]].off) return AVSR_ERR_ARG;
+  }
+  const int gx = blocks_for(n, 1024, 1024);
+  if ((int64_t)gx + (int64_t)L2_GX * S.nseg + 1 > scratch_floats) return AVSR_ERR_ARG;
+  float* part = scratch;
+  float* reg = scratch + gx;
+  int32_t* step_copy = reinterpret_cast<int32_t*>(scratch + gx + L2_GX * S.nseg);
+  hipLaunchKernelGGL(optimiser_fused_partial_kernel, dim3(gx + L2_GX * S.nseg), dim3(256), 0, S_(stream), S, params, grads, (long)n, gx, part,
+                     reg, step, step_copy);
+  AVSR_CHECK_LAUNCH();
+  hipLaunchKernelGGL(optimiser_fused_apply_kernel, dim3(blocks_for(n, 1024, 2048)), dim3(256), 0, S_(stream), S, params, grads, m, v, (long)n,
+                     part, gx, reg, loss_accum, gnorm_out, step, step_copy, lr, warmup_steps, clip_norm, 0.9f, 0.999f, 1e-8f, grad_scale,
+                     first_decay_steps, optimiser, weight_decay);
+  AVSR_CHECK_LAUNCH();
+  return AVSR_OK;
+}
diff --git a/avsr-tf1_amd/model.py b/avsr-tf1_amd/model.py
--- a/avsr-tf1_amd/model.py
+++ b/avsr-tf1_amd/model.py
@@ -404,10 +404,11 @@
             ops.gemm(ov, self.P["dec/out/kernel"].mat(V), ops.mat(D["logits"], V), B * L, V, O, bias=self._pp("dec/out/bias"))
         ops.seq_loss(D["logits"], batch.labels, batch.labels_len, self.denom, compute_denom, D["row_loss"], D["dlogits"], B, L, V,
                      loss_fun=cfg.loss_code(), label_smoothing=cfg.label_smoothing)
-        ops.reduce_scalar(D["row_loss"], B * L, self.loss)
+        terms = [(D["row_loss"], B * L)]
         if cfg.regress_aus and "video" in ws["enc"]:
             Ev = ws["enc"]["video"]
-            ops.reduce_scalar(Ev["au_row"], B * Ev["T"], self.loss, accumulate=True)
+            terms.append((Ev["au_row"], B * Ev["T"]))
+        ops.loss_assemble(terms, self.loss)
         if cfg.use_ctc:
             self._ctc_forward(ws, batch)
         return D["logits"]
@@ -499,16 +500,16 @@
     def apply_update(self):
         cfg = self.cfg
         self._dp_stats_unpack()
+        groups = []
         if cfg.recurrent_l2 is not None:
-            ops.l2_regularise(self.l2_segments, self.params, self.grads, cfg.recurrent_l2, self.loss, self.scratch)
+            groups.append((self.l2_segments, cfg.recurrent_l2))
         if self.use_cnn:
-            ops.l2_regularise(self.cnn_l2_segments, self.params, self.grads, 1e-3, self.loss, self.scratch)
+            groups.append((self.cnn_l2_segments, 1e-3))
             if self.dense_l2_segments:
-                ops.l2_regularise(self.dense_l2_segments, self.params, self.grads, 1e-4, self.loss, self.scratch)
-        ops.global_norm(self.grads, self.n_train, self.gnorm, self.scratch)
-        ops.adam_step(self.params, self.grads, self.adam_m, self.adam_v, self.n_train, self.gnorm, self.step,
-                      cfg.learning_rate, cfg.warmup_steps, cfg.max_gradient_norm if cfg.clip_gradients else 0.0,
-                      first_decay_steps=cfg.lr_decay_steps, optimiser=cfg.optimiser, weight_decay=cfg.weight_decay)
+                groups.append((self.dense_l2_segments, 1e-4))
+        ops.optimiser_step_fused(self.params, self.grads, self.adam_m, self.adam_v, self.n_train, groups, self.loss, self.gnorm, self.step,
+                                 cfg.learning_rate, cfg.warmup_steps, cfg.max_gradient_norm if cfg.clip_gradients else 0.0, self.scratch,
+                                 first_decay_steps=cfg.lr_decay_steps, optimiser=cfg.optimiser, weight_decay=cfg.weight_decay)
 
     def train_step(self, batch: Batch):
         self.forward_train(batch)
diff --git a/avsr-tf1_amd/model_encoder.py b/avsr-tf1_amd/model_encoder.py
--- a/avsr-tf1_amd/model_encoder.py
+++ b/avsr-tf1_amd/model_encoder.py
@@ -316,6 +316,7 @@
         cfg, B = self.cfg, ws["B"]
         self._dropping = bool(cfg.use_dropout and training)
         stacks = []
+        bn_maps, bn_dropped = [], set()
         for s in cfg.streams():
             E = ws["enc"][s]
             T, F = E["T"], E["F"]
@@ -331,7 +332,30 @@
                 x = self._fit_width(E, x, s)
             assert x.shape == (B, T, F) and x.is_contiguous() and x.dtype == torch.float32
             E["x"], E["len"] = x, len_t
-            if cfg.batch_normalisation:
+            sync = getattr(self, "cnn_bn_sync", None) if (training and "cnn" in E) else None
+            if (cfg.batch_normalisation and training and sync is None and not (self.bn_sync is not None and s in self.bn_sync["streams"])
+                    and len(bn_maps) < 4):
+                m = dict(x=x, y=E["xn"], rows=B * T, F=F, gamma=self._pp(f"{s}/bn/gamma"), beta=self._pp(f"{s}/bn/beta"),
+                         mov_mean=self._sp(f"{s}/bn/moving_mean"), mov_var=self._sp(f"{s}/bn/moving_variance"),
+                         save_mean=E["mean_own"], save_invstd=E["invstd"], drops=[])
+                plain0 = not (cfg.instance_normalisation or self.n_dense or E["nplain"] == 0 or cfg.highway(s))
+                if plain0 and self._sdrop(s) and E["F0"] == F and len(cfg.directions()) <= 2:
+                    m["drops"] = [(E["xd"][d], encoder_cell_id(s, d, 0) * 4, self._keeps(s)[0]) for d in cfg.directions()]
+                    bn_dropped.add(s)
+                    if not E["attentive"] and cfg.architecture != "av_align":
+                        m["y"] = None
+                bn_maps.append((s, m))
+        if bn_maps:
+            ops.batchnorm_fwd_multi([m for _, m in bn_maps], self.seed, self.scratch)
+        bn_done = {s for s, _ in bn_maps}
+        for s in cfg.streams():
+            E = ws["enc"][s]
+            T, F = E["T"], E["F"]
+            x, len_t = E["x"], E["len"]
+            if s in bn_done:
+                E["mean"] = E["mean_own"]
+                E["xin"] = E["xn"]
+            elif cfg.batch_normalisation:
                 sync = getattr(self, "cnn_bn_sync", None) if (training and "cnn" in E) else None
                 if sync is not None:
                     if "sync64" not in E:
@@ -384,8 +408,9 @@
                 xin = E["xin0"]
                 if self._sdrop(s):
                     xin = E["xd"][d]
-                    ops.dropout_rows(ops.mat(E["xin0"], F0), ops.mat(xin, F0), B * T, F0, self.seed, encoder_cell_id(s, d, 0) * 4,
-                                     self._keeps(s)[0], F0)
+                    if s not in bn_dropped:
+                        ops.dropout_rows(ops.mat(E["xin0"], F0), ops.mat(xin, F0), B * T, F0, self.seed, encoder_cell_id(s, d, 0) * 4,
+                                         self._keeps(s)[0], F0)
                 G = self.G
                 ops.gemm(ops.mat(xin, F0), W0.mat(G * u0), ops.mat(E["layers"][(d, 0)]["gates"], G * u0), B * T, G * u0, F0)
                 if self.gru:
diff --git a/avsr-tf1_amd/ops.py b/avsr-tf1_amd/ops.py
--- a/avsr-tf1_amd/ops.py
+++ b/avsr-tf1_amd/ops.py
@@ -278,6 +278,18 @@
                                   _s()), "avsr_batchnorm_fwd")
 
 
+def batchnorm_fwd_multi(maps, seed, scratch):
+    from ._lib import BnMap
+    arr = (BnMap * len(maps))()
+    for q, m in zip(arr, maps):
+        q.x, q.y, q.gamma, q.beta = fptr(m["x"]), fptr(m["y"]), fptr(m["gamma"]), fptr(m["beta"])
+        q.moving_mean, q.moving_var, q.save_mean, q.save_invstd = fptr(m["mov_mean"]), fptr(m["mov_var"]), fptr(m["save_mean"]), fptr(m["save_invstd"])
+        q.rows, q.F = int(m["rows"]), int(m["F"])
+        for d, (out, stream_id, keep) in enumerate(m.get("drops", ())):
+            q.drop_out[d], q.drop_stream[d], q.drop_keep[d] = fptr(out), int(stream_id), float(keep)
+    check(_L().avsr_batchnorm_fwd_multi(arr, len(maps), fptr(seed), fptr(scratch), scratch.numel(), _s()), "avsr_batchnorm_fwd_multi")
+
+
 def batchnorm_sync_sum(x, rows, F, sum_out, scratch):
     check(_L().avsr_batchnorm_sync_sum(fptr(x), rows, F, fptr(sum_out), fptr(scratch), scratch.numel(), _s()), "avsr_batchnorm_sync_sum")
 
@@ -367,6 +379,12 @@
 def reduce_scalar(part, n, out, do_sqrt=False, accumulate=False, scale=1.0, out_offset=0):
     check(_L().avsr_reduce_scalar(fptr(part), n, fptr(out, out_offset), int(do_sqrt), int(accumulate), float(scale),
                                   _s()), "avsr_reduce_scalar")
+
+
+def loss_assemble(terms, out):
+    ptrs = (C.c_void_p * len(terms))(*[fptr(t) for t, _ in terms])
+    cnt = (C.c_int32 * len(terms))(*[int(n) for _, n in terms])
+    check(_L().avsr_loss_assemble(ptrs, cnt, len(terms), fptr(out), _s()), "avsr_loss_assemble")
 
 
 def l2_regularise(segments, params, grads, l2, loss_accum, scratch):
@@ -442,6 +460,19 @@
     check(_L().avsr_optimiser_step(fptr(params), fptr(grads), fptr(m), fptr(v), n, fptr(gnorm), fptr(step), float(lr),
                                    int(warmup_steps), int(first_decay_steps), float(clip_norm), float(grad_scale), OPTIMISER[optimiser],
                                    float(weight_decay), _s()), "avsr_optimiser_step")
+
+
+def optimiser_step_fused(params, grads, m, v, n, l2_groups, loss_accum, gnorm, step, lr, warmup_steps, clip_norm, scratch, grad_scale=1.0,
+                         first_decay_steps=0, optimiser="Adam", weight_decay=0.0):
+    segs = [sg for g, _ in l2_groups for sg in g]
+    off = (C.c_int64 * max(1, len(segs)))(*[int(o) for o, _ in segs])
+    cnt = (C.c_int64 * max(1, len(segs)))(*[int(c) for _, c in segs])
+    gn = (C.c_int32 * max(1, len(l2_groups)))(*[len(g) for g, _ in l2_groups])
+    gl = (C.c_float * max(1, len(l2_groups)))(*[float(l) for _, l in l2_groups])
+    check(_L().avsr_optimiser_step_fused(fptr(params), fptr(grads), fptr(m), fptr(v), n, off, cnt, gn, gl, len(l2_groups), fptr(loss_accum),
+                                         fptr(gnorm), fptr(step), float(lr), int(warmup_steps), int(first_decay_steps), float(clip_norm),
+                                         float(grad_scale), OPTIMISER[optimiser], float(weight_decay), fptr(scratch), scratch.numel(), _s()),
+          "avsr_optimiser_step_fused")
 
 
 PROF_KINDS = ("gemm", "step_lstm_fwd", "step_lstm_bwd", "step_dense", "attn_fwd", "attn_bwd", "rnn_persist_fwd", "rnn_persist_bwd", "dec_persist_fwd", "dec_persist_bwd",
diff --git a/include/avsr_hip.h b/include/avsr_hip.h
--- a/include/avsr_hip.h
+++ b/include/avsr_hip.h
@@ -296,6 +296,22 @@
 
 int avsr_colsum(const avsr_mat* a, const avsr_mat* b, int32_t rows, int32_t F, float alpha, float beta, float* out,
                 float* scratch, int64_t scratch_floats, void* stream);
+
+typedef struct avsr_bn_map {
+  const float* x;
+  float* y;
+  const float* gamma;
+  const float* beta;
+  float* moving_mean;
+  float* moving_var;
+  float* save_mean;
+  float* save_invstd;
+  float* drop_out[2];
+  int32_t drop_stream[2];
+  float drop_keep[2];
+  int32_t rows, F;
+} avsr_bn_map;
+int avsr_batchnorm_fwd_multi(const avsr_bn_map* maps, int32_t n, const int32_t* seed, float* scratch, int64_t scratch_floats, void* stream);
 
 int avsr_batchnorm_fwd(const float* x, float* y, int32_t rows, int32_t F, const float* gamma, const float* beta,
                        float* moving_mean, float* moving_var, float* save_mean, float* save_invstd, int32_t training,
@@ -491,6 +507,8 @@
 int avsr_reduce_scalar(const float* part, int32_t n, float* out, int32_t do_sqrt, int32_t accumulate, float scale,
                        void* stream);
 
+int avsr_loss_assemble(const float* const* parts, const int32_t* n, int32_t count, float* out, void* stream);
+
 int avsr_l2_regularise(const int64_t* seg_off, const int64_t* seg_n, int32_t nseg, const float* params, float* grads,
                        float l2, float* loss_accum, float* scratch, void* stream);
 int avsr_global_norm(const float* grads, int64_t n, float grad_scale, float* norm_out, float* scratch, void* stream);
@@ -502,6 +520,10 @@
 int avsr_optimiser_step(float* params, float* grads, float* m, float* v, int64_t n, const float* global_norm, int32_t* step,
                         float lr, int32_t warmup_steps, int32_t first_decay_steps, float clip_norm, float grad_scale,
                         int32_t optimiser, float weight_decay, void* stream);
+int avsr_optimiser_step_fused(float* params, float* grads, float* m, float* v, int64_t n, const int64_t* seg_off,
+                              const int64_t* seg_n, const int32_t* group_nseg, const float* group_l2, int32_t ngroup, float* loss_accum,
+                              float* gnorm_out, int32_t* step, float lr, int32_t warmup_steps, int32_t first_decay_steps, float clip_norm,
+                              float grad_scale, int32_t optimiser, float weight_decay, float* scratch, int64_t scratch_floats, void* stream);
 
 #define AVSR_PROF_NKIND 15
 int avsr_prof_begin(int32_t max_launches);
```

After: 5713 utterances/sec, median of 2. Within noise of the previous version (-0.0%).
